# V-DETR/V-DETR

Measured on AMD Instinct MI355X. Metric: scenes/sec (train fwd+bwd) 40k-pt ScanNet, higher is better.
Workload: dtype f32

## Files before the change

include/vdetr_hip.h:

```cpp
#ifndef VDETR_HIP_H
#define VDETR_HIP_H

#include <stddef.h>
#include <stdint.h>

#ifdef __cplusplus
extern "C" {
#endif

#define VDETR_OK 0
#define VDETR_ERR_ARG 1
#define VDETR_ERR_LAUNCH 2
#define VDETR_ERR_WORKSPACE 3

typedef void* vdetr_stream_t;

int vdetr_abi_version(void);
const char* vdetr_last_error(void);
int vdetr_ab_switches(void);


size_t vdetr_fps_workspace_bytes(int b, int n);
int vdetr_furthest_point_sampling_f32(const float* xyz, int b, int n, int m, int32_t* idx,
                                      void* workspace, size_t workspace_bytes, vdetr_stream_t stream);

size_t vdetr_fps_varlen_workspace_bytes(const int32_t* counts, int b);
int vdetr_furthest_point_sampling_varlen_f32(const float* const* xyz, const int32_t* counts, int b, int m, int32_t* idx,
                                             void* workspace, size_t workspace_bytes, vdetr_stream_t stream);

int vdetr_gather_rows_f32(const float* const* rows, const int32_t* idx, float* out, int b, int c, int m, vdetr_stream_t stream);
int vdetr_gather_rows_grad_f32(const float* grad_out, const int32_t* idx, float* const* grad_rows, int b, int c, int m,
                               vdetr_stream_t stream);

int vdetr_gather_points_f32(const float* points, const int32_t* idx, float* out, int b, int c, int n,
                            int m, vdetr_stream_t stream);
int vdetr_gather_points_grad_f32(const float* grad_out, const int32_t* idx, float* grad_points, int b,
                                 int c, int n, int m, vdetr_stream_t stream);
int vdetr_gather_points_grad_set_f32(const float* grad_out, const int32_t* idx, float* grad_points, int b,
                                     int c, int n, int m, vdetr_stream_t stream);

int vdetr_ball_query_f32(const float* new_xyz, const float* xyz, int32_t* idx, int b, int n, int m,
                         float radius, int nsample, vdetr_stream_t stream);

int vdetr_group_points_f32(const float* points, const int32_t* idx, float* out, int b, int c, int n,
                           int npoints, int nsample, vdetr_stream_t stream);
int vdetr_group_points_grad_f32(const float* grad_out, const int32_t* idx, float* grad_points, int b,
                                int c, int n, int npoints, int nsample, vdetr_stream_t stream);
int vdetr_group_points_grad_set_f32(const float* grad_out, const int32_t* idx, float* grad_points, int b,
                                    int c, int n, int npoints, int nsample, vdetr_stream_t stream);

int vdetr_three_nn_f32(const float* unknown, const float* known, float* dist2, int32_t* idx, int b,
                       int n, int m, vdetr_stream_t stream);
int vdetr_three_interpolate_f32(const float* points, const int32_t* idx, const float* weight,
                                float* out, int b, int c, int m, int n, vdetr_stream_t stream);
int vdetr_three_interpolate_grad_f32(const float* grad_out, const int32_t* idx, const float* weight,
                                     float* grad_points, int b, int c, int n, int m,
                                     vdetr_stream_t stream);

#define VDETR_ATTN_SHARED_KV 0
#define VDETR_ATTN_PER_HEAD 1

#define VDETR_MASK_NONE 0
#define VDETR_MASK_BOOL 1
#define VDETR_MASK_FLOAT 2

typedef struct vdetr_attn_desc {
  int32_t kind;
  int32_t B, H, nQ, nK;
  float scale;
  const float* table;
  int32_t table_size;
  float log_scale;
  float inv_log_norm;
  const float* vertices;
  const float* xyz;
  const float* cos_sin;
  const void* mask;
  int32_t mask_kind;
  float dropout_p;
  uint64_t seed, offset;
  const uint64_t* rng_state;
  int32_t k_row_stride, v_row_stride;
  uint32_t* bwd_aux;
  int32_t table_grid;
  int32_t kv_waves;
  int32_t fwd_kernel;
  int32_t bwd_kernel;
  int32_t kv_halves;
  const void* kv_img;
  uint32_t* fwd_sched;
} vdetr_attn_desc;

size_t vdetr_attn_fwd_workspace_bytes(const vdetr_attn_desc* d);
size_t vdetr_attn_kv_image_bytes(int B, int nK);
int vdetr_attn_pack_kv_f32(const float* k, const float* v, int B, int nK, int k_row_stride, int v_row_stride, int nlayers,
                           int64_t layer_stride, void* img, vdetr_stream_t stream);
size_t vdetr_attn_kv_image_parts_bytes(int B, int nK, int parts);
int vdetr_attn_pack_kv_parts_f32(const float* k, const float* v, int B, int nK, int k_row_stride, int v_row_stride, int nlayers,
                                 int64_t layer_stride, int parts, void* img, vdetr_stream_t stream);

int vdetr_attn_fwd_f32(const vdetr_attn_desc* d, const float* q, const float* k, const float* v,
                       float* out, float* lse, float* scores, void* workspace, size_t workspace_bytes,
                       vdetr_stream_t stream);

typedef struct vdetr_attn_parts {
  const float* part_o;
  const float* part_lse;
  int32_t ksplit;
  int32_t reserved;
  int64_t rows;
} vdetr_attn_parts;
int vdetr_attn_fwd_parts_f32(const vdetr_attn_desc* d, const float* q, const float* k, const float* v,
                             float* out, float* lse, float* scores, void* workspace, size_t workspace_bytes,
                             vdetr_attn_parts* parts, vdetr_stream_t stream);

int vdetr_attn_fwd_bf16(const vdetr_attn_desc* d, const void* q, const void* k, const void* v, float* out, float* lse,
                        float* scores, void* workspace, size_t workspace_bytes, vdetr_stream_t stream);
size_t vdetr_attn_bwd_workspace_bytes(const vdetr_attn_desc* d);
int vdetr_attn_bwd_scores_f32(const vdetr_attn_desc* d, const float* scores, const float* dprob, const float* lse,
                              const float* delta, float* probs_out, float* ds_out, float* dtable, void* workspace,
                              size_t workspace_bytes, vdetr_stream_t stream);

size_t vdetr_attn_bwd_kv_workspace_bytes(const vdetr_attn_desc* d);
int vdetr_attn_bwd_kv_f32(const vdetr_attn_desc* d, const float* q, const float* v, const float* dout, const float* scores,
                          const float* lse, const float* delta, float* ds_out, float* dk, float* dv, void* workspace,
                          size_t workspace_bytes, vdetr_stream_t stream);
int vdetr_attn_bwd_kv_delta_f32(const vdetr_attn_desc* d, const float* q, const float* v, const float* dout, const float* out,
                                const float* scores, const float* lse, float* delta, float* ds_out, float* dk, float* dv,
                                void* workspace, size_t workspace_bytes, vdetr_stream_t stream);
typedef struct vdetr_attn_kv_prep {
  int32_t kind, B, H, nQ, nK, v_row_stride;
  const float* q;
  const float* v;
  const float* vertices;
  const float* cos_sin;
  void* workspace;
  float *dk, *dv;
  uint32_t* bwd_aux;
} vdetr_attn_kv_prep;
int vdetr_attn_bwd_kv_prep_f32(const vdetr_attn_kv_prep* items, int n, vdetr_stream_t stream);
int vdetr_attn_bwd_kv_packed_f32(const vdetr_attn_desc* d, const float* q, const float* v, const float* dout, const float* scores,
                                 const float* lse, const float* delta, float* ds_out, float* dk, float* dv, void* workspace,
                                 size_t workspace_bytes, vdetr_stream_t stream);
typedef struct vdetr_rb_attn_emit {
  void* workspace;
  float* delta;
  const float* out;
  uint32_t* bwd_aux;
  int32_t per_head, nQ;
} vdetr_rb_attn_emit;
int vdetr_attn_bwd_dq_f32(const vdetr_attn_desc* d, const float* ds, const float* k, float* dq, vdetr_stream_t stream);
int vdetr_attn_bwd_table_f32(const vdetr_attn_desc* d, const float* ds, float* dtable, void* workspace,
                             size_t workspace_bytes, vdetr_stream_t stream);
int vdetr_attn_bwd_table_kernel_names(const vdetr_attn_desc* d, const char** box_kernel, const char** general_kernel);

int vdetr_attn_delta_f32(const vdetr_attn_desc* d, const float* dout, const float* out, const float* v, float* delta,
                         vdetr_stream_t stream);

int vdetr_attn_dropout_mask_u8(const vdetr_attn_desc* d, uint8_t* keep, vdetr_stream_t stream);

int vdetr_rpe_bias_f32(const vdetr_attn_desc* d, float* rpe, vdetr_stream_t stream);

#define VDETR_CLS_SOFTMAX 0
#define VDETR_CLS_SIGMOID 1

typedef struct vdetr_box_decode_desc {
  int32_t B, N;
  int32_t A;
  int32_t C1;
  int32_t num_angle_bin;
  int32_t cls_kind;
  const float *center, *size;
  const float *angle_cls, *angle_res;
  const float* cls;
  const float *pre_center_norm, *pre_size_norm;
  const float *dims_min, *dims_max;
  float *center_reg, *size_reg, *center_unnorm, *center_norm, *size_unnorm, *size_norm, *pre_center_unnorm, *pre_size_unnorm;
  float* angle_residual;
  float *angle_cont, *angle_prob;
  int32_t* angle_class;
  float* corners;
  float* corners_aa;
  float* cls_prob;
  float* objectness;
  int32_t in_batch_stride;
  float *cls_logits_t, *angle_logits_t, *angle_res_norm_t;
  float *corners_lidar, *center_size;
} vdetr_box_decode_desc;

typedef struct vdetr_box_decode_grads {
  const float *center_reg, *size_reg, *center_unnorm, *center_norm, *size_unnorm, *size_norm;
  const float* angle_residual;
  const float *angle_cont, *angle_prob;
  const float *corners, *corners_aa;
  float *d_center, *d_size;
  float *d_angle_cls, *d_angle_res;
  const float *cls_logits_t, *angle_logits_t, *angle_res_norm_t;
  float* d_cls;
  int32_t out_batch_stride, slab_rows;
} vdetr_box_decode_grads;

int vdetr_box_decode_fwd_f32(const vdetr_box_decode_desc* d, vdetr_stream_t stream);
int vdetr_box_decode_bwd_f32(const vdetr_box_decode_desc* d, const vdetr_box_decode_grads* g, vdetr_stream_t stream);
int vdetr_anchor_boxes_f32(const float* logits, const float* xyz, const float* dims_min, const float* dims_max, const float* anchors,
                           int B, int N, int ncls, float* size_unnorm, float* center_norm, float* size_norm, float* corners,
                           vdetr_stream_t stream);
int vdetr_gather_proposals_f32(const long long* topk, int B, int N, int nq, int corners_are_camera, const float* corners,
                               const float* center, const float* size, const float* angle, const float* center_norm,
                               const float* size_norm, float* o_corners_lidar, float* o_center, float* o_size, float* o_angle,
                               float* o_center_norm, float* o_size_norm, float* o_query_ref, vdetr_stream_t stream);
int vdetr_box_decode_bwd_batch_f32(const vdetr_box_decode_desc* d, const vdetr_box_decode_grads* g, int n, vdetr_stream_t stream);

typedef struct vdetr_addln_desc {
  int32_t rows, C;
  float eps;
  float dropout_p;
  uint64_t seed, offset;
  const uint64_t* rng_state;
  const float* x;
  const float* r;
  const float *gamma, *beta;
  const float *gamma2, *beta2;
  float* y;
  float *out, *out2;
  float *mean, *rstd;
} vdetr_addln_desc;

typedef struct vdetr_addln_grads {
  const float *d_out, *d_out2;
  const float* d_y;
  float* d_x;
  float* d_r;
  float *d_gamma, *d_beta, *d_gamma2, *d_beta2;
  float* partials;
} vdetr_addln_grads;

int vdetr_add_ln_fwd_f32(const vdetr_addln_desc* d, vdetr_stream_t stream);
size_t vdetr_add_ln_bwd_workspace_bytes(const vdetr_addln_desc* d);
int vdetr_add_ln_bwd_f32(const vdetr_addln_desc* d, const vdetr_addln_grads* g, vdetr_stream_t stream);
typedef struct vdetr_addln_reduce {
  const float* partials;
  int32_t nparts, C;
  float *d_gamma, *d_beta, *d_gamma2, *d_beta2;
} vdetr_addln_reduce;
int vdetr_add_ln_param_reduce_batch_f32(const vdetr_addln_reduce* items, int n, vdetr_stream_t stream);

typedef struct vdetr_rb_linear {
  const float* w;
  const float* b;
  const float* wt;
} vdetr_rb_linear;
typedef struct vdetr_rb_norm {
  const float *gamma, *beta;
  float eps;
} vdetr_rb_norm;
typedef struct vdetr_rb_drop {
  float p;
  uint64_t seed;
} vdetr_rb_drop;

typedef struct vdetr_rb_qkv_desc {
  int32_t rows, B;
  const float* t;
  const float* pos;
  const float* w;
  const float* b;
  const float* wt;
  float* x;
  float* out;
} vdetr_rb_qkv_desc;
int vdetr_rb_qkv_f32(const vdetr_rb_qkv_desc* d, vdetr_stream_t stream);
int vdetr_rb_transpose_f32(const float* const* src, float* dst, int n, vdetr_stream_t stream);

typedef struct vdetr_rb_projq_desc {
  int32_t rows, B;
  const uint64_t* rng_state;
  const float* a;
  const float* tgt;
  const float* pos;
  vdetr_rb_linear proj, q;
  vdetr_rb_drop drop1;
  vdetr_rb_norm norm2;
  float *y, *mean_y, *rstd_y, *t2;
  float* xq;
  float* qout;
} vdetr_rb_projq_desc;
int vdetr_rb_proj_q_f32(const vdetr_rb_projq_desc* d, vdetr_stream_t stream);

typedef struct vdetr_rb_ffn_desc {
  int32_t rows, B;
  const uint64_t* rng_state;
  const float* a;
  const float* tgt;
  vdetr_rb_linear proj, lin1, lin2;
  vdetr_rb_drop drop2, drop_act, drop3;
  vdetr_rb_norm norm3, post1, post2;
  float *y, *mean_y, *rstd_y, *t2;
  float* h;
  float *z, *mean_z, *rstd_z, *o1, *o2;
} vdetr_rb_ffn_desc;
int vdetr_rb_ffn_f32(const vdetr_rb_ffn_desc* d, vdetr_stream_t stream);
int vdetr_rb_ffn_parts_f32(const vdetr_rb_ffn_desc* d, const vdetr_attn_parts* parts, float* attn_out, float* attn_lse,
                           vdetr_stream_t stream);

typedef struct vdetr_rb_qkv_grads {
  const float *dq, *dk, *dv;
  float *dq_rows, *dk_rows, *dv_rows;
  float* d_x;
  const float* d_x_add;
  float* d_t;
} vdetr_rb_qkv_grads;
int vdetr_rb_qkv_bwd_f32(const vdetr_rb_qkv_desc* d, const vdetr_rb_qkv_grads* g, vdetr_stream_t stream);

typedef struct vdetr_rb_projq_grads {
  const float* d_y;
  const float* d_qout;
  float* d_tgt;
  float* d_a;
  float* d_t2;
  float* dq_rows;
  float* d_proj;
  float* part_n2;
} vdetr_rb_projq_grads;
int vdetr_rb_proj_q_bwd_f32(const vdetr_rb_projq_desc* d, const vdetr_rb_projq_grads* g, vdetr_stream_t stream);

typedef struct vdetr_rb_ffn_grads {
  const float *d_z, *d_o1, *d_o2;
  float* d_tgt;
  float* d_a;
  float *d_lin2, *d_lin1, *d_proj;
  float *part_post, *part_n3;
} vdetr_rb_ffn_grads;
int vdetr_rb_ffn_bwd_f32(const vdetr_rb_ffn_desc* d, const vdetr_rb_ffn_grads* g, vdetr_stream_t stream);
int vdetr_rb_ffn0_f32(const vdetr_rb_ffn_desc* d, vdetr_stream_t stream);
int vdetr_rb_ffn0_bwd_f32(const vdetr_rb_ffn_desc* d, const vdetr_rb_ffn_grads* g, vdetr_stream_t stream);
int vdetr_rb_ffn_bwd_emit_f32(const vdetr_rb_ffn_desc* d, const vdetr_rb_ffn_grads* g, const vdetr_rb_attn_emit* e, vdetr_stream_t stream);
int vdetr_rb_proj_q_bwd_emit_f32(const vdetr_rb_projq_desc* d, const vdetr_rb_projq_grads* g, const vdetr_rb_attn_emit* e,
                                 vdetr_stream_t stream);

typedef struct vdetr_bnact_desc {
  int32_t B, C, N;
  int32_t training;
  int32_t relu;
  float eps, momentum;
  float dropout_p;
  uint64_t seed, offset;
  const uint64_t* rng_state;
  const float* x;
  const float *gamma, *beta;
  float *running_mean, *running_var;
  float* y;
  float *save_mean, *save_invstd;
  const float* pre_bias;
  int64_t* counters[8];
  int32_t ncounters;
  int32_t stats_given;
} vdetr_bnact_desc;

typedef struct vdetr_bnact_grads {
  const float* dy;
  float* dx;
  float *d_gamma, *d_beta;
  const float *sum_dy_xhat, *sum_dy, *inv_count;
} vdetr_bnact_grads;

int vdetr_relu_dropout_fwd_f32(const float* x, float* y, long n, float dropout_p, uint64_t seed, uint64_t offset,
                               const uint64_t* rng_state, vdetr_stream_t stream);
int vdetr_relu_dropout_bwd_f32(const float* y, const float* dy, float* dx, long n, float dropout_p, vdetr_stream_t stream);
int vdetr_bn_act_fwd_f32(const vdetr_bnact_desc* d, vdetr_stream_t stream);
int vdetr_bn_stats_f32(const vdetr_bnact_desc* d, float* mean, float* m2, vdetr_stream_t stream);
int vdetr_bn_act_bwd_f32(const vdetr_bnact_desc* d, const vdetr_bnact_grads* g, vdetr_stream_t stream);
int vdetr_bn_act_bwd_batch_f32(const vdetr_bnact_desc* descs, const vdetr_bnact_grads* grads, int n, vdetr_stream_t stream);

typedef struct vdetr_pack_entry {
  const void* src;
  uint64_t dst_offset;
  uint64_t numel;
} vdetr_pack_entry;
int vdetr_colsum_f32(const float* x, float* out, int rows, int cols, long row_stride, vdetr_stream_t stream);
size_t vdetr_colsum_workspace_bytes(int n, int rows, int cols);
int vdetr_colsum_batched_f32(const float* x, float* out, int n, int rows, int cols, long row_stride, long item_stride,
                             void* workspace, size_t workspace_bytes, vdetr_stream_t stream);
int vdetr_colsum_ptrs_f32(const float* const* items, float* out, int n, int rows, int cols, long row_stride, void* workspace,
                          size_t workspace_bytes, vdetr_stream_t stream);
int vdetr_pack_chunk_floats(void);
int vdetr_pack_f32(const vdetr_pack_entry* entries, const uint32_t* block_entry, const uint32_t* block_chunk, int nblocks,
                   float* dst, vdetr_stream_t stream);
int vdetr_pack_sumsq_f32(const vdetr_pack_entry* entries, const uint32_t* block_entry, const uint32_t* block_chunk, int nblocks,
                         float* dst, float* sumsq, vdetr_stream_t stream);

int vdetr_cpb_tables_f32(const float* coords, const float* w1, const float* b1, const float* w2, int n, int P, int hidden, int H,
                         float* hid_out, float* tables, vdetr_stream_t stream);

typedef struct vdetr_adamw_desc {
  float* param;
  const float* grad;
  float* exp_avg;
  float* exp_avg_sq;
  int64_t n;
  float* step;
  uint32_t* ticket;
  const float* sumsq;
  int32_t nsumsq;
  float max_norm;
  float norm_eps;
  float* norm_out;
  double lr, beta1, beta2, eps, weight_decay;
} vdetr_adamw_desc;
int vdetr_adamw_clip_f32(const vdetr_adamw_desc* d, vdetr_stream_t stream);
int vdetr_sumsq_blocks(long n);
int vdetr_sumsq_f32(const float* g, long n, float* partial, int npartial, vdetr_stream_t stream);

int vdetr_morton_sort_max(void);
int vdetr_morton_order_f32(const float* xyz, int B, int n, int* codes, long long* order, vdetr_stream_t stream);
int vdetr_topk_order_f32(const float* values, int B, int n, int nq, long long* order, vdetr_stream_t stream);

#define VDETR_GT_CORNERS 0
#define VDETR_GT_CENTER 24
#define VDETR_GT_SIZE 27
#define VDETR_GT_ANGLE 30
#define VDETR_GT_LABEL 31
#define VDETR_GT_ANGLE_CLS 32
#define VDETR_GT_ANGLE_RES 33
#define VDETR_GT_PRESENT 34
#define VDETR_GT_FLOATS 36

int vdetr_gt_prepare_f32(const float* gt, int B, int G, int repeat, float* gt_rep, int64_t* nactual, int64_t* nactual_rep,
                         float* sums, vdetr_stream_t stream);

typedef struct vdetr_match_desc {
  int32_t B, P, G;
  int32_t C, A;
  int32_t cls_kind;
  int32_t label_override;
  float w_cls, w_objectness, w_center, w_giou, w_size, w_angle_cls, w_angle_reg;
  const float* cls;
  const float* objectness;
  const float *center_reg, *size_reg, *pre_center, *pre_size;
  const float* corners;
  const float *angle_logits, *angle_res_norm;
  const float* gt;
  const int64_t* nactual;
  float* cost_t;
  float* giou_t;
  const float* rotated;
} vdetr_match_desc;
int vdetr_match_cost_f32(const vdetr_match_desc* d, vdetr_stream_t stream);
int vdetr_match_cost_batch_f32(const vdetr_match_desc* descs, int n, vdetr_stream_t stream);

#define VDETR_LSA_MAX_PROBLEMS 16
typedef struct vdetr_lsa_problem {
  const float* cost_t;
  const int64_t* nactual;
  int64_t* inds;
  float* mask;
  int32_t B, P, G;
  int32_t row_repeat;
} vdetr_lsa_problem;
typedef struct vdetr_lsa_batch {
  int32_t nproblems;
  int32_t reserved;
  vdetr_lsa_problem p[VDETR_LSA_MAX_PROBLEMS];
} vdetr_lsa_batch;
int vdetr_lsa_f64(const vdetr_lsa_batch* batch, int32_t* status, vdetr_stream_t stream);

int vdetr_point_labels_f32(const float* seed_xyz, const float* gt, const int64_t* nactual, int B, int N, int G, int C,
                           int64_t* labels, float* matched_count, vdetr_stream_t stream);

typedef struct vdetr_setloss_desc {
  int32_t B, P, G, C, A;
  int32_t label_override;
  float focal_alpha;
  float w_cls, w_angle_cls, w_angle_reg, w_center, w_size, w_giou;
  int32_t cls_kind;
  float w_no_object;
  const float* cls_logits;
  const float *center_reg, *size_reg, *pre_center, *pre_size;
  const float* corners;
  const float *angle_logits, *angle_res_norm;
  const float* gt;
  const int64_t* nactual;
  const int64_t* inds;
  const float* mask;
  const int64_t* labels;
  const float* num_boxes;
  float* losses;
  unsigned long long* card_ws;
  float *d_cls_logits, *d_center_reg, *d_size_reg, *d_corners, *d_angle_logits, *d_angle_res_norm;
  const float* rotated;
  const float* ce_rows_matched;
} vdetr_setloss_desc;
int vdetr_set_loss_f32(const vdetr_setloss_desc* d, vdetr_stream_t stream);
int vdetr_set_loss_batch_f32(const vdetr_setloss_desc* descs, int n, vdetr_stream_t stream);

#define VDETR_IOU_GIOU 0
#define VDETR_IOU_DIOU 1
#define VDETR_IOU_IOU 2
typedef struct vdetr_iou_ext {
  int32_t iou_kind;
  int32_t reserved;
  const float *center, *size;
  const float* angle;
  float *d_center, *d_size;
  float* d_angle;
} vdetr_iou_ext;
int vdetr_match_cost_ext_batch_f32(const vdetr_match_desc* descs, const vdetr_iou_ext* exts, int n, vdetr_stream_t stream);
int vdetr_set_loss_ext_batch_f32(const vdetr_setloss_desc* descs, const vdetr_iou_ext* exts, int n, vdetr_stream_t stream);

size_t vdetr_nms3d_workspace_bytes(int B, int K);
int vdetr_nms3d_f32(const float* corners, const float* score, const int32_t* cls, const uint8_t* valid, const int64_t* order,
                    int B, int K, double iou_threshold, int old_type, uint8_t* keep, void* workspace, size_t workspace_bytes,
                    vdetr_stream_t stream);

size_t vdetr_nms3d_rot_workspace_bytes(int B, int K);
int vdetr_nms3d_rot_f32(const float* corners, const float* score, const int32_t* cls, const uint8_t* valid, const int64_t* order,
                        int B, int K, double iou_threshold, int old_type, uint8_t* keep, void* workspace,
                        size_t workspace_bytes, vdetr_stream_t stream);

int vdetr_box_point_count_f32(const float* points, const float* boxes, int B, int N, int K, int32_t* counts,
                              vdetr_stream_t stream);

int vdetr_box3d_iou_max_f64(const float* pred_corners, const int32_t* pred_img, const int32_t* pred_cls, int P,
                            const float* gt_corners, const int32_t* gt_cls, const int32_t* img_gt_begin, double* ovmax,
                            int32_t* jmax, vdetr_stream_t stream);

int vdetr_box3d_iou_pairs_f64(const float* corners_a, int Na, const float* corners_b, int Nb, double* out,
                              vdetr_stream_t stream);

int vdetr_sp_kernel_map_i32(const int64_t* in_keys, int nin, const int64_t* out_keys, int nout, const int32_t* offsets, int K,
                            int32_t* nbr, vdetr_stream_t stream);
int vdetr_sp_inverse_map_i32(const int32_t* nbr, int K, int nout, int nin, int32_t* inv, vdetr_stream_t stream);
int vdetr_sp_gather_cols_f32(const float* in, const int32_t* nbr, int K, int nout, int C, float* col, vdetr_stream_t stream);
int vdetr_sp_gather_sum_f32(const float* dcol, const int32_t* inv, int K, int nin, int C, int offset_major_rows, float* din,
                            vdetr_stream_t stream);

int vdetr_sp_pairs_gemm_f32(const float* x, const int32_t* arow, const float* w, const int32_t* tiles, int ntiles, int cin,
                            int cout, int transposed, float* y, vdetr_stream_t stream);
int vdetr_sp_pairs_wgrad_f32(const float* x, const float* dy, const int32_t* pin, const int32_t* pout, const int32_t* chunks,
                             int nchunks, int cin, int cout, float* partials, vdetr_stream_t stream);
int vdetr_sp_wgrad_reduce_f32(const float* partials, const int32_t* seg, int K, long elems, float* dw, vdetr_stream_t stream);
int vdetr_sp_pair_plan_workspace_ints(int K, int nout);
int vdetr_sp_pair_plan_i32(const int32_t* nbr, int K, int nout, int nin, int32_t* pin, int32_t* pout, int32_t* slot,
                           int32_t* islot, int32_t* counts, int32_t* workspace, vdetr_stream_t stream);

typedef struct vdetr_spbn_desc {
  int32_t N, C, act, training;
  float eps, momentum;
  const float *x, *gamma, *beta, *residual;
  float *running_mean, *running_var;
  int64_t* num_batches_tracked;
  float *y, *save_mean, *save_invstd;
  void* workspace;
} vdetr_spbn_desc;
size_t vdetr_sp_bn_workspace_bytes(int N, int C);
int vdetr_sp_bn_act_fwd_f32(const vdetr_spbn_desc* d, vdetr_stream_t stream);
int vdetr_sp_bn_act_bwd_f32(const vdetr_spbn_desc* d, const float* dy, float* dx, float* dresidual, float* dgamma, float* dbeta,
                            vdetr_stream_t stream);

int vdetr_pos_embed_fourier_f32(const float* xyz, int b, int n, const float* range_min, const float* range_max,
                                const float* gauss_b, int ldb, int d_out, float* out, vdetr_stream_t stream);
int vdetr_pos_embed_sine_f32(const float* xyz, int b, int n, const float* range_min, const float* range_max,
                             int num_channels, float temperature, float scale, float* out, vdetr_stream_t stream);

typedef struct vdetr_heads_desc {
  int32_t B, N;
  int32_t G, rows;
  const float* x;
  const float* w1t;
  const float* w2t;
  const float* w3;
  const float* b3;
  const float *gamma1, *beta1, *gamma2, *beta2;
  float *running_mean1, *running_var1, *running_mean2, *running_var2;
  int64_t* counters1[8];
  int64_t* counters2[8];
  float eps, momentum;
  float p1, p2;
  uint64_t salt1, salt2;
  const uint64_t* rng_state;
  float *pre1, *h1, *pre2, *h2;
  float *save_mean1, *save_invstd1, *save_mean2, *save_invstd2;
  float* y;
  void* workspace;
} vdetr_heads_desc;
size_t vdetr_heads_workspace_bytes(int B, int N, int G);
int vdetr_heads_fwd_f32(const vdetr_heads_desc* d, vdetr_stream_t stream);

typedef struct vdetr_heads_infer_desc {
  int32_t B, N;
  int32_t G, rows;
  int32_t tile;
  float eps;
  const float* x;
  const float* w1t;
  const float* w2t;
  const float* w3;
  const float* b3;
  const float *mean1, *var1, *gamma1, *beta1;
  const float *mean2, *var2, *gamma2, *beta2;
  float* y;
} vdetr_heads_infer_desc;
int vdetr_heads_infer_f32(const vdetr_heads_infer_desc* d, vdetr_stream_t stream);

typedef struct vdetr_posmlp_desc {
  int32_t B, N, cin;
  const float* x;
  const float* w1;
  const float* b1;
  const float *gamma, *beta;
  float *running_mean, *running_var;
  int64_t* counter;
  float eps, momentum;
  const float* w2t;
  const float* b2;
  float *hpre, *hact;
  float *save_mean, *save_invstd;
  float* out;
} vdetr_posmlp_desc;
int vdetr_pos_mlp_fwd_f32(const vdetr_posmlp_desc* d, vdetr_stream_t stream);
int vdetr_rb_qkv_pos_f32(const vdetr_rb_qkv_desc* d, const vdetr_posmlp_desc* m, vdetr_stream_t stream);
int vdetr_pos_mlp_infer_f32(const vdetr_posmlp_desc* d, vdetr_stream_t stream);
int vdetr_rb_qkv_pos_infer_f32(const vdetr_rb_qkv_desc* d, const vdetr_posmlp_desc* m, vdetr_stream_t stream);

int vdetr_selftest_lds_atomics(int mode, int iters, float* sink, vdetr_stream_t stream);

int vdetr_probe_timestamp(uint64_t* slot, vdetr_stream_t stream);

int vdetr_selftest_mfma_f32(const float* a, const float* b, float* c, vdetr_stream_t stream);

#ifdef __cplusplus
}
#endif
#endif
```

v-detr_amd/_lib.py:

```python
import ctypes
import os

import torch

_HERE = os.path.dirname(os.path.abspath(__file__))
LIB_PATH = os.path.join(_HERE, "lib", "libvdetr_hip.so")

c_int, c_float, c_void_p, c_size_t = ctypes.c_int, ctypes.c_float, ctypes.c_void_p, ctypes.c_size_t

VDETR_ATTN_SHARED_KV, VDETR_ATTN_PER_HEAD = 0, 1
VDETR_MASK_NONE, VDETR_MASK_BOOL, VDETR_MASK_FLOAT = 0, 1, 2


class AttnDesc(ctypes.Structure):

    _fields_ = [
        ("kind", ctypes.c_int32), ("B", ctypes.c_int32), ("H", ctypes.c_int32), ("nQ", ctypes.c_int32),
        ("nK", ctypes.c_int32), ("scale", c_float),
        ("table", c_void_p), ("table_size", ctypes.c_int32), ("log_scale", c_float), ("inv_log_norm", c_float),
        ("vertices", c_void_p), ("xyz", c_void_p), ("cos_sin", c_void_p),
        ("mask", c_void_p), ("mask_kind", ctypes.c_int32),
        ("dropout_p", c_float), ("seed", ctypes.c_uint64), ("offset", ctypes.c_uint64),
        ("rng_state", c_void_p),
        ("k_row_stride", ctypes.c_int32), ("v_row_stride", ctypes.c_int32),
        ("bwd_aux", c_void_p),
        ("table_grid", ctypes.c_int32), ("kv_waves", ctypes.c_int32), ("fwd_kernel", ctypes.c_int32), ("bwd_kernel", ctypes.c_int32), ("kv_halves", ctypes.c_int32), ("kv_img", c_void_p),
        ("fwd_sched", c_void_p),
    ]


VDETR_CLS_SOFTMAX, VDETR_CLS_SIGMOID = 0, 1

_BOX_IN = ("center", "size", "angle_cls", "angle_res", "cls", "pre_center_norm", "pre_size_norm", "dims_min", "dims_max")
_BOX_OUT = ("center_reg", "size_reg", "center_unnorm", "center_norm", "size_unnorm", "size_norm", "pre_center_unnorm",
            "pre_size_unnorm", "angle_residual", "angle_cont", "angle_prob", "angle_class", "corners", "corners_aa",
            "cls_prob", "objectness")


class BoxDecodeDesc(ctypes.Structure):

    _fields_ = ([(n, ctypes.c_int32) for n in ("B", "N", "A", "C1", "num_angle_bin", "cls_kind")] +
                [(n, c_void_p) for n in _BOX_IN + _BOX_OUT] + [("in_batch_stride", ctypes.c_int32)] +
                [(n, c_void_p) for n in ("cls_logits_t", "angle_logits_t", "angle_res_norm_t", "corners_lidar", "center_size")])


_BOX_GRAD_IN = ("center_reg", "size_reg", "center_unnorm", "center_norm", "size_unnorm", "size_norm", "angle_residual",
                "angle_cont", "angle_prob", "corners", "corners_aa")
_BOX_GRAD_OUT = ("d_center", "d_size", "d_angle_cls", "d_angle_res")


class BoxDecodeGrads(ctypes.Structure):

    _fields_ = ([(n, c_void_p) for n in _BOX_GRAD_IN + _BOX_GRAD_OUT] +
                [(n, c_void_p) for n in ("cls_logits_t", "angle_logits_t", "angle_res_norm_t", "d_cls")] +
                [("out_batch_stride", ctypes.c_int32), ("slab_rows", ctypes.c_int32)])


class AddLnDesc(ctypes.Structure):

    _fields_ = [("rows", ctypes.c_int32), ("C", ctypes.c_int32), ("eps", c_float), ("dropout_p", c_float),
                ("seed", ctypes.c_uint64), ("offset", ctypes.c_uint64), ("rng_state", c_void_p)] + [
        (n, c_void_p) for n in ("x", "r", "gamma", "beta", "gamma2", "beta2", "y", "out", "out2", "mean", "rstd")]


class AddLnGrads(ctypes.Structure):

    _fields_ = [(n, c_void_p) for n in ("d_out", "d_out2", "d_y", "d_x", "d_r", "d_gamma", "d_beta", "d_gamma2", "d_beta2",
                                        "partials")]


class AddLnReduce(ctypes.Structure):

    _fields_ = [("partials", c_void_p), ("nparts", ctypes.c_int32), ("C", ctypes.c_int32), ("d_gamma", c_void_p), ("d_beta", c_void_p),
                ("d_gamma2", c_void_p), ("d_beta2", c_void_p)]


class RbLinear(ctypes.Structure):

    _fields_ = [("w", c_void_p), ("b", c_void_p), ("wt", c_void_p)]


class RbNorm(ctypes.Structure):

    _fields_ = [("gamma", c_void_p), ("beta", c_void_p), ("eps", c_float)]


class RbDrop(ctypes.Structure):

    _fields_ = [("p", c_float), ("seed", ctypes.c_uint64)]


class RbQkvDesc(ctypes.Structure):

    _fields_ = [("rows", ctypes.c_int32), ("B", ctypes.c_int32)] + [(n, c_void_p) for n in ("t", "pos", "w", "b", "wt", "x", "out")]


class RbProjQDesc(ctypes.Structure):

    _fields_ = ([("rows", ctypes.c_int32), ("B", ctypes.c_int32)] + [(n, c_void_p) for n in ("rng_state", "a", "tgt", "pos")] +
                [("proj", RbLinear), ("q", RbLinear), ("drop1", RbDrop), ("norm2", RbNorm)] +
                [(n, c_void_p) for n in ("y", "mean_y", "rstd_y", "t2", "xq", "qout")])


class RbFfnDesc(ctypes.Structure):

    _fields_ = ([("rows", ctypes.c_int32), ("B", ctypes.c_int32)] + [(n, c_void_p) for n in ("rng_state", "a", "tgt")] +
                [("proj", RbLinear), ("lin1", RbLinear), ("lin2", RbLinear), ("drop2", RbDrop), ("drop_act", RbDrop), ("drop3", RbDrop),
                 ("norm3", RbNorm), ("post1", RbNorm), ("post2", RbNorm)] +
                [(n, c_void_p) for n in ("y", "mean_y", "rstd_y", "t2", "h", "z", "mean_z", "rstd_z", "o1", "o2")])


class RbQkvGrads(ctypes.Structure):

    _fields_ = [(n, c_void_p) for n in ("dq", "dk", "dv", "dq_rows", "dk_rows", "dv_rows", "d_x", "d_x_add", "d_t")]


class RbProjQGrads(ctypes.Structure):

    _fields_ = [(n, c_void_p) for n in ("d_y", "d_qout", "d_tgt", "d_a", "d_t2", "dq_rows", "d_proj", "part_n2")]


class RbFfnGrads(ctypes.Structure):

    _fields_ = [(n, c_void_p) for n in ("d_z", "d_o1", "d_o2", "d_tgt", "d_a", "d_lin2", "d_lin1", "d_proj", "part_post", "part_n3")]


class BnActDesc(ctypes.Structure):

    _fields_ = [(n, ctypes.c_int32) for n in ("B", "C", "N", "training", "relu")] + [
        ("eps", c_float), ("momentum", c_float), ("dropout_p", c_float), ("seed", ctypes.c_uint64),
        ("offset", ctypes.c_uint64), ("rng_state", c_void_p)] + [
        (n, c_void_p) for n in ("x", "gamma", "beta", "running_mean", "running_var", "y", "save_mean", "save_invstd",
                                "pre_bias")] + [("counters", c_void_p * 8), ("ncounters", ctypes.c_int32),
                                                ("stats_given", ctypes.c_int32)]


class HeadsDesc(ctypes.Structure):

    _fields_ = [(n, ctypes.c_int32) for n in ("B", "N", "G", "rows")] + [
        (n, c_void_p) for n in ("x", "w1t", "w2t", "w3", "b3", "gamma1", "beta1", "gamma2", "beta2", "running_mean1", "running_var1",
                                "running_mean2", "running_var2")] + [
        ("counters1", c_void_p * 8), ("counters2", c_void_p * 8), ("eps", c_float), ("momentum", c_float), ("p1", c_float),
        ("p2", c_float), ("salt1", ctypes.c_uint64), ("salt2", ctypes.c_uint64), ("rng_state", c_void_p)] + [
        (n, c_void_p) for n in ("pre1", "h1", "pre2", "h2", "save_mean1", "save_invstd1", "save_mean2", "save_invstd2", "y",
                                "workspace")]


class HeadsInferDesc(ctypes.Structure):

    _fields_ = [(n, ctypes.c_int32) for n in ("B", "N", "G", "rows", "tile")] + [("eps", c_float)] + [
        (n, c_void_p) for n in ("x", "w1t", "w2t", "w3", "b3", "mean1", "var1", "gamma1", "beta1", "mean2", "var2", "gamma2", "beta2",
                                "y")]


class AttnParts(ctypes.Structure):

    _fields_ = [("part_o", c_void_p), ("part_lse", c_void_p), ("ksplit", ctypes.c_int32), ("reserved", ctypes.c_int32),
                ("rows", ctypes.c_int64)]


class AttnKvPrep(ctypes.Structure):

    _fields_ = [(n, ctypes.c_int32) for n in ("kind", "B", "H", "nQ", "nK", "v_row_stride")] + [
        (n, c_void_p) for n in ("q", "v", "vertices", "cos_sin", "workspace", "dk", "dv", "bwd_aux")]


class RbAttnEmit(ctypes.Structure):

    _fields_ = [(n, c_void_p) for n in ("workspace", "delta", "out", "bwd_aux")] + [("per_head", ctypes.c_int32), ("nQ", ctypes.c_int32)]


class AdamWDesc(ctypes.Structure):

    _fields_ = [(n, c_void_p) for n in ("param", "grad", "exp_avg", "exp_avg_sq")] + [("n", ctypes.c_int64)] + [
        (n, c_void_p) for n in ("step", "ticket", "sumsq")] + [("nsumsq", ctypes.c_int32), ("max_norm", c_float), ("norm_eps", c_float),
                                                                ("norm_out", c_void_p)] + [
        (n, ctypes.c_double) for n in ("lr", "beta1", "beta2", "eps", "weight_decay")]


class PosMlpDesc(ctypes.Structure):

    _fields_ = [(n, ctypes.c_int32) for n in ("B", "N", "cin")] + [
        (n, c_void_p) for n in ("x", "w1", "b1", "gamma", "beta", "running_mean", "running_var", "counter")] + [
        ("eps", c_float), ("momentum", c_float)] + [
        (n, c_void_p) for n in ("w2t", "b2", "hpre", "hact", "save_mean", "save_invstd", "out")]


class BnActGrads(ctypes.Structure):

    _fields_ = [(n, c_void_p) for n in ("dy", "dx", "d_gamma", "d_beta", "sum_dy_xhat", "sum_dy", "inv_count")]


VDETR_GT_CORNERS, VDETR_GT_CENTER, VDETR_GT_SIZE, VDETR_GT_ANGLE, VDETR_GT_LABEL = 0, 24, 27, 30, 31
VDETR_GT_ANGLE_CLS, VDETR_GT_ANGLE_RES, VDETR_GT_PRESENT, VDETR_GT_FLOATS = 32, 33, 34, 36
VDETR_LSA_MAX_PROBLEMS = 16

_MATCH_W = ("w_cls", "w_objectness", "w_center", "w_giou", "w_size", "w_angle_cls", "w_angle_reg")
_MATCH_PTR = ("cls", "objectness", "center_reg", "size_reg", "pre_center", "pre_size", "corners", "angle_logits",
              "angle_res_norm", "gt", "nactual", "cost_t", "giou_t", "rotated")


class MatchDesc(ctypes.Structure):

    _fields_ = ([(n, ctypes.c_int32) for n in ("B", "P", "G", "C", "A", "cls_kind", "label_override")] +
                [(n, c_float) for n in _MATCH_W] + [(n, c_void_p) for n in _MATCH_PTR])


class LsaProblem(ctypes.Structure):

    _fields_ = [(n, c_void_p) for n in ("cost_t", "nactual", "inds", "mask")] + [
        (n, ctypes.c_int32) for n in ("B", "P", "G", "row_repeat")]


class LsaBatch(ctypes.Structure):

    _fields_ = [("nproblems", ctypes.c_int32), ("reserved", ctypes.c_int32), ("p", LsaProblem * VDETR_LSA_MAX_PROBLEMS)]


_LOSS_W = ("w_cls", "w_angle_cls", "w_angle_reg", "w_center", "w_size", "w_giou")
_LOSS_PTR = ("cls_logits", "center_reg", "size_reg", "pre_center", "pre_size", "corners", "angle_logits", "angle_res_norm",
             "gt", "nactual", "inds", "mask", "labels", "num_boxes", "losses", "card_ws", "d_cls_logits", "d_center_reg", "d_size_reg",
             "d_corners", "d_angle_logits", "d_angle_res_norm", "rotated", "ce_rows_matched")


class SetLossDesc(ctypes.Structure):

    _fields_ = ([(n, ctypes.c_int32) for n in ("B", "P", "G", "C", "A", "label_override")] + [("focal_alpha", c_float)] +
                [(n, c_float) for n in _LOSS_W] + [("cls_kind", ctypes.c_int32), ("w_no_object", c_float)] +
                [(n, c_void_p) for n in _LOSS_PTR])


VDETR_IOU_GIOU, VDETR_IOU_DIOU, VDETR_IOU_IOU = 0, 1, 2
IOU_KINDS = {"giou": VDETR_IOU_GIOU, "diou": VDETR_IOU_DIOU, "iou": VDETR_IOU_IOU}


class IouExt(ctypes.Structure):

    _fields_ = [("iou_kind", ctypes.c_int32), ("reserved", ctypes.c_int32)] + [
        (n, c_void_p) for n in ("center", "size", "angle", "d_center", "d_size", "d_angle")]


class SpBnDesc(ctypes.Structure):

    _fields_ = ([(n, ctypes.c_int32) for n in ("N", "C", "act", "training")] + [("eps", c_float), ("momentum", c_float)] +
                [(n, c_void_p) for n in ("x", "gamma", "beta", "residual", "running_mean", "running_var", "num_batches_tracked",
                                         "y", "save_mean", "save_invstd", "workspace")])


_SIGNATURES = {
    "vdetr_abi_version": (c_int, []),
    "vdetr_ab_switches": (c_int, []),
    "vdetr_last_error": (ctypes.c_char_p, []),
    "vdetr_fps_workspace_bytes": (c_size_t, [c_int, c_int]),
    "vdetr_furthest_point_sampling_f32": (c_int, [c_void_p, c_int, c_int, c_int, c_void_p, c_void_p, c_size_t, c_void_p]),
    "vdetr_fps_varlen_workspace_bytes": (c_size_t, [c_void_p, c_int]),
    "vdetr_furthest_point_sampling_varlen_f32": (c_int, [c_void_p, c_void_p, c_int, c_int, c_void_p, c_void_p, c_size_t, c_void_p]),
    "vdetr_pos_embed_fourier_f32": (c_int, [c_void_p, c_int, c_int, c_void_p, c_void_p, c_void_p, c_int, c_int, c_void_p, c_void_p]),
    "vdetr_pos_embed_sine_f32": (c_int, [c_void_p, c_int, c_int, c_void_p, c_void_p, c_int, c_float, c_float, c_void_p, c_void_p]),
    "vdetr_gather_rows_f32": (c_int, [c_void_p, c_void_p, c_void_p, c_int, c_int, c_int, c_void_p]),
    "vdetr_gather_rows_grad_f32": (c_int, [c_void_p, c_void_p, c_void_p, c_int, c_int, c_int, c_void_p]),
    "vdetr_gather_points_f32": (c_int, [c_void_p, c_void_p, c_void_p, c_int, c_int, c_int, c_int, c_void_p]),
    "vdetr_gather_points_grad_f32": (c_int, [c_void_p, c_void_p, c_void_p, c_int, c_int, c_int, c_int, c_void_p]),
    "vdetr_gather_points_grad_set_f32": (c_int, [c_void_p, c_void_p, c_void_p, c_int, c_int, c_int, c_int, c_void_p]),
    "vdetr_group_points_grad_set_f32": (c_int, [c_void_p, c_void_p, c_void_p, c_int, c_int, c_int, c_int, c_int, c_void_p]),
    "vdetr_ball_query_f32": (c_int, [c_void_p, c_void_p, c_void_p, c_int, c_int, c_int, c_float, c_int, c_void_p]),
    "vdetr_group_points_f32": (c_int, [c_void_p, c_void_p, c_void_p, c_int, c_int, c_int, c_int, c_int, c_void_p]),
    "vdetr_group_points_grad_f32": (c_int, [c_void_p, c_void_p, c_void_p, c_int, c_int, c_int, c_int, c_int, c_void_p]),
    "vdetr_three_nn_f32": (c_int, [c_void_p, c_void_p, c_void_p, c_void_p, c_int, c_int, c_int, c_void_p]),
    "vdetr_three_interpolate_f32": (c_int, [c_void_p, c_void_p, c_void_p, c_void_p, c_int, c_int, c_int, c_int, c_void_p]),
    "vdetr_three_interpolate_grad_f32": (c_int, [c_void_p, c_void_p, c_void_p, c_void_p, c_int, c_int, c_int, c_int, c_void_p]),
    "vdetr_attn_fwd_workspace_bytes": (c_size_t, [ctypes.POINTER(AttnDesc)]),
    "vdetr_attn_kv_image_bytes": (c_size_t, [c_int, c_int]),
    "vdetr_attn_pack_kv_f32": (c_int, [c_void_p, c_void_p, c_int, c_int, c_int, c_int, c_int, ctypes.c_int64, c_void_p, c_void_p]),
    "vdetr_attn_kv_image_parts_bytes": (c_size_t, [c_int, c_int, c_int]),
    "vdetr_attn_pack_kv_parts_f32": (c_int, [c_void_p, c_void_p, c_int, c_int, c_int, c_int, c_int, ctypes.c_int64, c_int, c_void_p, c_void_p]),
    "vdetr_attn_fwd_f32": (c_int, [ctypes.POINTER(AttnDesc), c_void_p, c_void_p, c_void_p, c_void_p, c_void_p, c_void_p, c_void_p, c_size_t, c_void_p]),
    "vdetr_attn_fwd_bf16": (c_int, [ctypes.POINTER(AttnDesc), c_void_p, c_void_p, c_void_p, c_void_p, c_void_p, c_void_p, c_void_p, c_size_t, c_void_p]),
    "vdetr_attn_fwd_parts_f32": (c_int, [ctypes.POINTER(AttnDesc), c_void_p, c_void_p, c_void_p, c_void_p, c_void_p, c_void_p, c_void_p, c_size_t,
                                         ctypes.POINTER(AttnParts), c_void_p]),
    "vdetr_attn_bwd_workspace_bytes": (c_size_t, [ctypes.POINTER(AttnDesc)]),
    "vdetr_attn_bwd_scores_f32": (c_int, [ctypes.POINTER(AttnDesc), c_void_p, c_void_p, c_void_p, c_void_p, c_void_p, c_void_p, c_void_p, c_void_p, c_size_t, c_void_p]),
    "vdetr_attn_bwd_kv_workspace_bytes": (c_size_t, [ctypes.POINTER(AttnDesc)]),
    "vdetr_attn_bwd_kv_f32": (c_int, [ctypes.POINTER(AttnDesc)] + [c_void_p] * 10 + [c_size_t, c_void_p]),
    "vdetr_attn_bwd_kv_delta_f32": (c_int, [ctypes.POINTER(AttnDesc)] + [c_void_p] * 11 + [c_size_t, c_void_p]),
    "vdetr_attn_bwd_dq_f32": (c_int, [ctypes.POINTER(AttnDesc), c_void_p, c_void_p, c_void_p, c_void_p]),
    "vdetr_attn_bwd_table_f32": (c_int, [ctypes.POINTER(AttnDesc), c_void_p, c_void_p, c_void_p, c_size_t, c_void_p]),
    "vdetr_attn_bwd_table_kernel_names": (c_int, [ctypes.POINTER(AttnDesc), ctypes.POINTER(ctypes.c_char_p), ctypes.POINTER(ctypes.c_char_p)]),
    "vdetr_attn_delta_f32": (c_int, [ctypes.POINTER(AttnDesc), c_void_p, c_void_p, c_void_p, c_void_p, c_void_p]),
    "vdetr_attn_dropout_mask_u8": (c_int, [ctypes.POINTER(AttnDesc), c_void_p, c_void_p]),
    "vdetr_rpe_bias_f32": (c_int, [ctypes.POINTER(AttnDesc), c_void_p, c_void_p]),
    "vdetr_box_decode_fwd_f32": (c_int, [ctypes.POINTER(BoxDecodeDesc), c_void_p]),
    "vdetr_box_decode_bwd_f32": (c_int, [ctypes.POINTER(BoxDecodeDesc), ctypes.POINTER(BoxDecodeGrads), c_void_p]),
    "vdetr_box_decode_bwd_batch_f32": (c_int, [ctypes.POINTER(BoxDecodeDesc), ctypes.POINTER(BoxDecodeGrads), c_int, c_void_p]),
    "vdetr_add_ln_fwd_f32": (c_int, [ctypes.POINTER(AddLnDesc), c_void_p]),
    "vdetr_add_ln_bwd_workspace_bytes": (c_size_t, [ctypes.POINTER(AddLnDesc)]),
    "vdetr_add_ln_bwd_f32": (c_int, [ctypes.POINTER(AddLnDesc), ctypes.POINTER(AddLnGrads), c_void_p]),
    "vdetr_add_ln_param_reduce_batch_f32": (c_int, [ctypes.POINTER(AddLnReduce), c_int, c_void_p]),
    "vdetr_relu_dropout_fwd_f32": (c_int, [c_void_p, c_void_p, ctypes.c_long, c_float, ctypes.c_uint64, ctypes.c_uint64, c_void_p,
                                           c_void_p]),
    "vdetr_relu_dropout_bwd_f32": (c_int, [c_void_p, c_void_p, c_void_p, ctypes.c_long, c_float, c_void_p]),
    "vdetr_bn_act_fwd_f32": (c_int, [ctypes.POINTER(BnActDesc), c_void_p]),
    "vdetr_bn_stats_f32": (c_int, [ctypes.POINTER(BnActDesc), c_void_p, c_void_p, c_void_p]),
    "vdetr_heads_workspace_bytes": (c_size_t, [c_int, c_int, c_int]),
    "vdetr_heads_fwd_f32": (c_int, [ctypes.POINTER(HeadsDesc), c_void_p]),
    "vdetr_pos_mlp_fwd_f32": (c_int, [ctypes.POINTER(PosMlpDesc), c_void_p]),
    "vdetr_heads_infer_f32": (c_int, [ctypes.POINTER(HeadsInferDesc), c_void_p]),
    "vdetr_pos_mlp_infer_f32": (c_int, [ctypes.POINTER(PosMlpDesc), c_void_p]),
    "vdetr_bn_act_bwd_f32": (c_int, [ctypes.POINTER(BnActDesc), ctypes.POINTER(BnActGrads), c_void_p]),
    "vdetr_bn_act_bwd_batch_f32": (c_int, [ctypes.POINTER(BnActDesc), ctypes.POINTER(BnActGrads), c_int, c_void_p]),
    "vdetr_colsum_f32": (c_int, [c_void_p, c_void_p, c_int, c_int, ctypes.c_long, c_void_p]),
    "vdetr_colsum_workspace_bytes": (c_size_t, [c_int, c_int, c_int]),
    "vdetr_colsum_batched_f32": (c_int, [c_void_p, c_void_p, c_int, c_int, c_int, ctypes.c_long, ctypes.c_long, c_void_p, c_size_t, c_void_p]),
    "vdetr_colsum_ptrs_f32": (c_int, [c_void_p, c_void_p, c_int, c_int, c_int, ctypes.c_long, c_void_p, c_size_t, c_void_p]),
    "vdetr_nms3d_workspace_bytes": (c_size_t, [c_int, c_int]),
    "vdetr_nms3d_f32": (c_int, [c_void_p, c_void_p, c_void_p, c_void_p, c_void_p, c_int, c_int, ctypes.c_double, c_int, c_void_p,
                        c_void_p, c_size_t, c_void_p]),
    "vdetr_nms3d_rot_workspace_bytes": (c_size_t, [c_int, c_int]),
    "vdetr_nms3d_rot_f32": (c_int, [c_void_p, c_void_p, c_void_p, c_void_p, c_void_p, c_int, c_int, ctypes.c_double, c_int, c_void_p,
                            c_void_p, c_size_t, c_void_p]),
    "vdetr_box_point_count_f32": (c_int, [c_void_p, c_void_p, c_int, c_int, c_int, c_void_p, c_void_p]),
    "vdetr_box3d_iou_max_f64": (c_int, [c_void_p, c_void_p, c_void_p, c_int, c_void_p, c_void_p, c_void_p, c_void_p, c_void_p,
                                c_void_p]),
    "vdetr_box3d_iou_pairs_f64": (c_int, [c_void_p, c_int, c_void_p, c_int, c_void_p, c_void_p]),
    "vdetr_morton_sort_max": (c_int, []),
    "vdetr_morton_order_f32": (c_int, [c_void_p, c_int, c_int, c_void_p, c_void_p, c_void_p]),
    "vdetr_pack_chunk_floats": (c_int, []),
    "vdetr_pack_f32": (c_int, [c_void_p, c_void_p, c_void_p, c_int, c_void_p, c_void_p]),
    "vdetr_pack_sumsq_f32": (c_int, [c_void_p, c_void_p, c_void_p, c_int, c_void_p, c_void_p, c_void_p]),
    "vdetr_adamw_clip_f32": (c_int, [ctypes.POINTER(AdamWDesc), c_void_p]),
    "vdetr_cpb_tables_f32": (c_int, [c_void_p] * 4 + [c_int] * 4 + [c_void_p] * 3),
    "vdetr_sumsq_blocks": (c_int, [ctypes.c_long]),
    "vdetr_sumsq_f32": (c_int, [c_void_p, ctypes.c_long, c_void_p, c_int, c_void_p]),
    "vdetr_gt_prepare_f32": (c_int, [c_void_p, c_int, c_int, c_int, c_void_p, c_void_p, c_void_p, c_void_p, c_void_p]),
    "vdetr_match_cost_f32": (c_int, [ctypes.POINTER(MatchDesc), c_void_p]),
    "vdetr_match_cost_batch_f32": (c_int, [ctypes.POINTER(MatchDesc), c_int, c_void_p]),
    "vdetr_lsa_f64": (c_int, [ctypes.POINTER(LsaBatch), c_void_p, c_void_p]),
    "vdetr_point_labels_f32": (c_int, [c_void_p, c_void_p, c_void_p, c_int, c_int, c_int, c_int, c_void_p, c_void_p, c_void_p]),
    "vdetr_set_loss_f32": (c_int, [ctypes.POINTER(SetLossDesc), c_void_p]),
    "vdetr_set_loss_batch_f32": (c_int, [ctypes.POINTER(SetLossDesc), c_int, c_void_p]),
    "vdetr_match_cost_ext_batch_f32": (c_int, [ctypes.POINTER(MatchDesc), ctypes.POINTER(IouExt), c_int, c_void_p]),
    "vdetr_set_loss_ext_batch_f32": (c_int, [ctypes.POINTER(SetLossDesc), ctypes.POINTER(IouExt), c_int, c_void_p]),
    "vdetr_sp_kernel_map_i32": (c_int, [c_void_p, c_int, c_void_p, c_int, c_void_p, c_int, c_void_p, c_void_p]),
    "vdetr_sp_inverse_map_i32": (c_int, [c_void_p, c_int, c_int, c_int, c_void_p, c_void_p]),
    "vdetr_sp_gather_cols_f32": (c_int, [c_void_p, c_void_p, c_int, c_int, c_int, c_void_p, c_void_p]),
    "vdetr_sp_gather_sum_f32": (c_int, [c_void_p, c_void_p, c_int, c_int, c_int, c_int, c_void_p, c_void_p]),
    "vdetr_sp_pairs_gemm_f32": (c_int, [c_void_p, c_void_p, c_void_p, c_void_p, c_int, c_int, c_int, c_int, c_void_p, c_void_p]),
    "vdetr_sp_pair_plan_workspace_ints": (c_int, [c_int, c_int]),
    "vdetr_sp_pair_plan_i32": (c_int, [c_void_p, c_int, c_int, c_int, c_void_p, c_void_p, c_void_p, c_void_p, c_void_p, c_void_p,
                               c_void_p]),
    "vdetr_sp_wgrad_reduce_f32": (c_int, [c_void_p, c_void_p, c_int, ctypes.c_long, c_void_p, c_void_p]),
    "vdetr_sp_pairs_wgrad_f32": (c_int, [c_void_p, c_void_p, c_void_p, c_void_p, c_void_p, c_int, c_int, c_int, c_void_p, c_void_p]),
    "vdetr_sp_bn_workspace_bytes": (c_size_t, [c_int, c_int]),
    "vdetr_sp_bn_act_fwd_f32": (c_int, [ctypes.POINTER(SpBnDesc), c_void_p]),
    "vdetr_sp_bn_act_bwd_f32": (c_int, [ctypes.POINTER(SpBnDesc), c_void_p, c_void_p, c_void_p, c_void_p, c_void_p, c_void_p]),
    "vdetr_rb_transpose_f32": (c_int, [c_void_p, c_void_p, c_int, c_void_p]),
    "vdetr_rb_qkv_f32": (c_int, [ctypes.POINTER(RbQkvDesc), c_void_p]),
    "vdetr_rb_proj_q_f32": (c_int, [ctypes.POINTER(RbProjQDesc), c_void_p]),
    "vdetr_rb_qkv_pos_f32": (c_int, [ctypes.POINTER(RbQkvDesc), ctypes.POINTER(PosMlpDesc), c_void_p]),
    "vdetr_rb_qkv_pos_infer_f32": (c_int, [ctypes.POINTER(RbQkvDesc), ctypes.POINTER(PosMlpDesc), c_void_p]),
    "vdetr_rb_ffn_f32": (c_int, [ctypes.POINTER(RbFfnDesc), c_void_p]),
    "vdetr_rb_ffn_parts_f32": (c_int, [ctypes.POINTER(RbFfnDesc), ctypes.POINTER(AttnParts), c_void_p, c_void_p, c_void_p]),
    "vdetr_rb_qkv_bwd_f32": (c_int, [ctypes.POINTER(RbQkvDesc), ctypes.POINTER(RbQkvGrads), c_void_p]),
    "vdetr_rb_proj_q_bwd_f32": (c_int, [ctypes.POINTER(RbProjQDesc), ctypes.POINTER(RbProjQGrads), c_void_p]),
    "vdetr_rb_ffn_bwd_f32": (c_int, [ctypes.POINTER(RbFfnDesc), ctypes.POINTER(RbFfnGrads), c_void_p]),
    "vdetr_rb_ffn0_f32": (c_int, [ctypes.POINTER(RbFfnDesc), c_void_p]),
    "vdetr_rb_ffn0_bwd_f32": (c_int, [ctypes.POINTER(RbFfnDesc), ctypes.POINTER(RbFfnGrads), c_void_p]),
    "vdetr_rb_ffn_bwd_emit_f32": (c_int, [ctypes.POINTER(RbFfnDesc), ctypes.POINTER(RbFfnGrads), ctypes.POINTER(RbAttnEmit), c_void_p]),
    "vdetr_rb_proj_q_bwd_emit_f32": (c_int, [ctypes.POINTER(RbProjQDesc), ctypes.POINTER(RbProjQGrads), ctypes.POINTER(RbAttnEmit), c_void_p]),
    "vdetr_attn_bwd_kv_prep_f32": (c_int, [ctypes.POINTER(AttnKvPrep), c_int, c_void_p]),
    "vdetr_attn_bwd_kv_packed_f32": (c_int, [ctypes.POINTER(AttnDesc)] + [c_void_p] * 10 + [c_size_t, c_void_p]),
    "vdetr_probe_timestamp": (c_int, [c_void_p, c_void_p]),
    "vdetr_topk_order_f32": (c_int, [c_void_p, c_int, c_int, c_int, c_void_p, c_void_p]),
    "vdetr_anchor_boxes_f32": (c_int, [c_void_p] * 5 + [c_int] * 3 + [c_void_p] * 5),
    "vdetr_gather_proposals_f32": (c_int, [c_void_p, c_int, c_int, c_int, c_int] + [c_void_p] * 14),
    "vdetr_selftest_lds_atomics": (c_int, [c_int, c_int, c_void_p, c_void_p]),
    "vdetr_selftest_mfma_f32": (c_int, [c_void_p, c_void_p, c_void_p, c_void_p]),
}

_lib = None


def exported_symbols():
    return sorted(_SIGNATURES)


def lib():
    global _lib
    if _lib is None:
        if not os.path.exists(LIB_PATH):
            raise RuntimeError(
                f"{LIB_PATH} is missing: build it with `python -c 'import __graft_entry__ as g; g.build()'` "
                "(hipcc --offload-arch=gfx950).  vdetr_amd has no CPU fallback.")
        handle = ctypes.CDLL(LIB_PATH)
        for name, (restype, argtypes) in _SIGNATURES.items():
            fn = getattr(handle, name)
            fn.restype = restype
            fn.argtypes = argtypes
        _lib = handle
    return _lib


def check(status, op):
    if status != 0:
        msg = lib().vdetr_last_error().decode(errors="replace")
        raise RuntimeError(f"vdetr_hip {op} failed (status {status}): {msg}")


def stream_ptr():
    return c_void_p(torch.cuda.current_stream().cuda_stream)


def ptr(t):
    return c_void_p(t.data_ptr()) if t is not None else c_void_p(0)


def require_gpu(t, name):
    if not t.is_cuda:
        raise RuntimeError(f"{name}: CPU not supported (tensor is on {t.device})")


def require_contiguous(t, name):
    if not t.is_contiguous():
        raise RuntimeError(f"{name} must be a contiguous tensor")


def require_float(t, name):
    if t.dtype != torch.float32:
        raise RuntimeError(f"{name} must be a float tensor")


def require_int(t, name):
    if t.dtype != torch.int32:
        raise RuntimeError(f"{name} must be an int tensor")


def workspace(nbytes, device):
    return torch.empty(max(int(nbytes), 1), dtype=torch.uint8, device=device)


_rocblas = {"lib": None, "handles": {}}
ROCBLAS_OP_N, ROCBLAS_OP_T = 111, 112


def rocblas():
    if _rocblas["lib"] is None:
        path = os.path.join(os.path.dirname(torch.__file__), "lib", "librocblas.so")
        rb = ctypes.CDLL(path if os.path.exists(path) else "librocblas.so")
        rb.rocblas_create_handle.argtypes = [ctypes.POINTER(c_void_p)]
        rb.rocblas_set_stream.argtypes = [c_void_p, c_void_p]
        rb.rocblas_sgemm_batched.argtypes = [c_void_p, c_int, c_int, c_int, c_int, c_int, c_void_p, c_void_p, c_int, c_void_p, c_int,
                                             c_void_p, c_void_p, c_int, c_int]
        _rocblas["lib"] = rb
    return _rocblas["lib"]


def sgemm_batched_ptrs(op_a, op_b, m, n, k, a_ptrs, lda, b_ptrs, ldb, c_ptrs, ldc, batch, device, alpha=1.0, beta=0.0):
    rb = rocblas()
    key = device.index if device.index is not None else torch.cuda.current_device()
    h = _rocblas["handles"].get(key)
    if h is None:
        if torch.cuda.is_current_stream_capturing():
            raise RuntimeError("rocBLAS handle: create it before a stream capture (run one step eagerly first)")
        h = c_void_p()
        with torch.cuda.device(key):
            if rb.rocblas_create_handle(ctypes.byref(h)) != 0:
                raise RuntimeError("rocblas_create_handle failed")
        _rocblas["handles"][key] = h
    if rb.rocblas_set_stream(h, c_void_p(torch.cuda.current_stream(device).cuda_stream)) != 0:
        raise RuntimeError("rocblas_set_stream failed")
    al, be = c_float(alpha), c_float(beta)
    addr = lambda p: c_void_p(p.data_ptr() if torch.is_tensor(p) else int(p))
    rc = rb.rocblas_sgemm_batched(h, op_a, op_b, m, n, k, ctypes.byref(al), addr(a_ptrs), lda, addr(b_ptrs), ldb, ctypes.byref(be),
                                  addr(c_ptrs), ldc, batch)
    if rc != 0:
        raise RuntimeError(f"rocblas_sgemm_batched failed (status {rc})")


_ptr_tables = {}


def upload_ptrs(ptrs, device):
    n = len(ptrs)
    key = device.index if device.index is not None else torch.cuda.current_device()
    T = _ptr_tables.get(key)
    if T is None:
        if torch.cuda.is_current_stream_capturing():
            raise RuntimeError("pointer tables: allocate before a stream capture (run one step eagerly first)")
        T = _ptr_tables[key] = {"ring": [torch.empty(1024, dtype=torch.int64).pin_memory() for _ in range(4)], "events": [None] * 4, "tick": 0,
                                "spare": [torch.empty(1024, dtype=torch.int64).pin_memory() for _ in range(48)], "kept": []}
    if n > 1024:
        raise RuntimeError(f"pointer table of {n} entries (max 1024)")
    dev = torch.empty(n, dtype=torch.int64, device=device)
    if torch.cuda.is_current_stream_capturing():
        if not T["spare"]:
            raise RuntimeError("pointer tables: more than 48 captured uploads in this process")
        host = T["spare"].pop()
        T["kept"].append(host)
        host[:n] = torch.tensor(ptrs, dtype=torch.int64)
        dev.copy_(host[:n], non_blocking=True)
        return dev
    slot = T["tick"] % 4
    T["tick"] += 1
    if T["events"][slot] is not None:
        T["events"][slot].synchronize()
    host = T["ring"][slot]
    host[:n] = torch.tensor(ptrs, dtype=torch.int64)
    dev.copy_(host[:n], non_blocking=True)
    ev = torch.cuda.Event()
    ev.record(torch.cuda.current_stream(device))
    T["events"][slot] = ev
    return dev
```

v-detr_amd/attention.py:

```python
import contextlib
import ctypes
import os
import weakref

import torch
from torch.autograd import Function

from . import _lib as L

HEAD_DIM = 64


class RPEConfig:

    def __init__(self, table_size=10, log_scale=512.0, max_value=4.0):
        self.table_size = int(table_size)
        self.log_scale = float(log_scale)
        self.max_value = float(max_value)

    @property
    def inv_log_norm(self):
        return 1.0 / (3.0 * self.max_value)


def new_rng_state(device, seed=None):
    if seed is None:
        seed = torch.initial_seed()
    return torch.tensor([seed & 0x7FFFFFFFFFFFFFFF, 0], dtype=torch.int64, device=device)


FWD_KERNEL = int(os.environ.get("VDETR_FWD_KERNEL", "0"))
BWD_KERNEL = int(os.environ.get("VDETR_BWD_KERNEL", "0"))
TABLE_GRID = 0
FUSED_KV_BWD = os.environ.get("VDETR_BWD_FUSED", "1") != "0"
SELF_FWD_BODY = os.environ.get("VDETR_SELF_FWD", "") == "body"


_ASYNC_ENV = os.environ.get("VDETR_BWD_ASYNC_TABLE", "auto")
ASYNC_TABLE_GRAD = _ASYNC_ENV != "0"
ASYNC_MIN_PAIRS = 1 << 21
ASYNC_TABLE_GRID = int(os.environ.get("VDETR_BWD_ASYNC_GRID", "190"))


_step_side = {}


def side_branch_in_use(device):
    return bool(_step_side.get(_dev_key(device)))


class SideResults:
    pending = []

    @classmethod
    def flush(cls):
        from .helpers import DeferredParamGrads
        items, cls.pending = cls.pending, []
        late, side_late[:] = list(side_late), []
        for fn, alive in late:
            with torch.no_grad():
                items.append((None, fn(), alive))
        for dev, pairs, _alive in items:
            side = _side_streams.get(_dev_key(dev)) if dev is not None else None
            if side is not None:
                torch.cuda.current_stream(dev).wait_stream(side)
            roots, grads = [], []
            with torch.no_grad():
                for p, g in pairs:
                    if p is not None and p.requires_grad:
                        DeferredParamGrads._deliver(p, g, roots, grads)
            if roots:
                torch.autograd.backward(roots, grads)


_tick = {}
side_late = []


def flush_layer_params_on_side(ref, rows):
    from .helpers import DeferredParamGrads, DeferredPosEmbedGrads
    if not (ref.is_cuda and DeferredParamGrads.enabled and side_branch_in_use(ref.device)):
        return
    dev = ref.device
    key = _dev_key(dev)
    cur = torch.cuda.current_stream(dev)
    fork = torch.cuda.Event()
    fork.record(cur)
    if key not in _tick:
        _tick[key] = torch.zeros(4, device=dev)
    _tick[key].add_(0.0)
    side = _side_stream(dev)
    side.wait_event(fork)
    pairs, keep = [], []
    late, side_late[:] = list(side_late), []
    from .runtime import ts_mark
    ts_mark("main: all layers' backward done")
    with torch.cuda.stream(side):
        ts_mark("side: parked gradients start")
        DeferredParamGrads.flush(select=lambda it: it[2].shape[0] == rows, collect=pairs, keepalive=keep)
        DeferredPosEmbedGrads.flush(collect=pairs, keepalive=keep)
        from .add_ln import DeferredLnGrads
        DeferredLnGrads.flush(collect=pairs, keepalive=keep)
        for fn, alive in late:
            pairs += fn()
            keep.append(alive)
        ts_mark("side: parked gradients end")
    if pairs:
        SideResults.pending.append((dev, pairs, keep))


def set_async_table_grad(mode):
    global _ASYNC_ENV, ASYNC_TABLE_GRAD
    prev, _ASYNC_ENV = _ASYNC_ENV, str(mode)
    ASYNC_TABLE_GRAD = _ASYNC_ENV != "0"
    return prev


def _async_wanted(B, nQ, nK):
    return ASYNC_TABLE_GRAD and (_ASYNC_ENV == "1" or B * nQ * nK >= ASYNC_MIN_PAIRS)


_side_streams = {}
_side_keep = []


def _dev_key(device):
    device = torch.device(device)
    if device.type != "cuda":
        return (device.type, 0)
    return (device.type, device.index if device.index is not None else torch.cuda.current_device())


def _side_stream(device):
    key = _dev_key(device)
    if key not in _side_streams:
        _side_streams[key] = torch.cuda.Stream(device=device)
    return _side_streams[key]


class _JoinTableGrad(Function):
    @staticmethod
    def forward(ctx, t):
        ctx.dev = t.device
        return t.view_as(t)

    @staticmethod
    def backward(ctx, g):
        side = _side_streams.get(_dev_key(ctx.dev))
        if side is not None and _side_keep:
            torch.cuda.current_stream(ctx.dev).wait_stream(side)
        _side_keep.clear()
        return g


class _ParkTableGrad(Function):

    @staticmethod
    def forward(ctx, anchor, table, slot):
        ctx.slot = slot
        return table.view_as(table)

    @staticmethod
    def backward(ctx, g):
        ctx.slot[1] = g
        return None, None, None


class DeferredTableGrads:
    pending = []
    _anchor = {}
    _begun = []
    buffers = {}
    _outputs = {}
    _buffer_keys = {}

    @classmethod
    def park(cls, tables, mlp=None):
        key = _dev_key(tables.device)
        if key not in cls._anchor:
            cls._anchor[key] = torch.zeros(1, device=tables.device, requires_grad=True)
        alive = []
        for item in cls.pending:
            _tables, slots, _acc, _mlp = item
            outs = cls._outputs.get(id(slots), ())
            if all(g is None for _, g in slots) and all(r() is None for r in outs):
                cls._outputs.pop(id(slots), None)
                for key_ in cls._buffer_keys.pop(id(slots), ()):
                    cls.buffers.pop(key_, None)
                continue
            alive.append(item)
        cls.pending = alive
        if sum(1 for _, slots, _, _ in alive if any(g is not None for _, g in slots)) > 32:
            raise RuntimeError("runtime.defer_weight_grads() is on but runtime.flush_weight_grads() has not been called for 32 "
                               "backward passes (parked RPE-table gradients pile up)")
        cut = tables.detach()
        slots = [[i, None] for i in range(tables.shape[0])]
        acc = None
        if tables.is_cuda and tables.dtype == torch.float32:
            acc = _take_zeros(tables, tuple(tables.shape), tables.dtype)
            for i in range(tables.shape[0]):
                cls.buffers[cut[i].data_ptr()] = acc[i]
            cls._buffer_keys[id(slots)] = [cut[i].data_ptr() for i in range(tables.shape[0])]
        cls.pending.append((tables, slots, acc, mlp))
        outs = [_ParkTableGrad.apply(cls._anchor[key], cut[i], slots[i]) for i in range(tables.shape[0])]
        cls._outputs[id(slots)] = [weakref.ref(o) for o in outs]
        return outs

    @classmethod
    def begin_flush(cls):
        keep = []
        for item in cls.pending:
            tables, slots, acc, mlp = item
            if mlp is None or all(g is None for _, g in slots):
                keep.append(item)
                continue
            dev = tables.device
            side = _side_streams.get(_dev_key(dev)) if (tables.is_cuda and _side_keep) else None
            cur = torch.cuda.current_stream(dev) if tables.is_cuda else None
            if acc is None or not all(g is None or g.data_ptr() == acc[i].data_ptr() for i, g in slots):
                if side is not None and _side_keep:
                    cur.wait_stream(side)
                acc = torch.stack([g if g is not None else torch.zeros_like(tables[i]) for i, g in slots])
                if side is not None:
                    side.wait_stream(cur)
            c1, w1, b1, w2, hid = mlp
            n8 = hid.shape[0]
            with (torch.cuda.stream(side) if side is not None else contextlib.nullcontext()), torch.no_grad():
                dT = acc.reshape(n8, hid.shape[1], -1)
                dW2 = torch.bmm(dT.transpose(1, 2), hid)
                dhid = torch.ops.aten.threshold_backward(torch.bmm(dT, w2.detach()), hid, 0.0)
                dW1b = torch.bmm(dhid.transpose(1, 2), c1.unsqueeze(0).expand(n8, -1, -1))
                if side is not None:
                    from .runtime import ts_mark
                    ts_mark("side: table MLPs' backward end")
            cls._begun.append((dev if side is not None else None, ((w1, dW1b[..., :3]), (b1, dW1b[..., 3]), (w2, dW2)),
                               (acc, dT, dhid, hid)))
        cls.pending = keep

    @classmethod
    def flush(cls):
        from .helpers import DeferredParamGrads
        SideResults.flush()
        begun, cls._begun = cls._begun, []
        for dev, pairs, _alive in begun:
            side = _side_streams.get(_dev_key(dev)) if dev is not None else None
            if side is not None:
                torch.cuda.current_stream(dev).wait_stream(side)
            _side_keep.clear()
            roots, grads = [], []
            with torch.no_grad():
                for p, g in pairs:
                    if p.requires_grad:
                        DeferredParamGrads._deliver(p, g, roots, grads)
            if roots:
                torch.autograd.backward(roots, grads)
        items, cls.pending = cls.pending, []
        cls.buffers.clear()
        cls._outputs.clear()
        cls._buffer_keys.clear()
        for tables, slots, acc, _mlp in items:
            if all(g is None for _, g in slots):
                continue
            if not tables.requires_grad:
                raise RuntimeError("tables parked with their MLP's operands can only be flushed through begin_flush()")
            dev = tables.device
            side = _side_streams.get(_dev_key(dev))
            if side is not None and _side_keep:
                torch.cuda.current_stream(dev).wait_stream(side)
            _side_keep.clear()
            if acc is not None and all(g is None or g.data_ptr() == acc[i].data_ptr() for i, g in slots):
                g = acc
            else:
                g = torch.stack([g if g is not None else torch.zeros_like(tables[i]) for i, g in slots])
            torch.autograd.backward([tables], [g])


def table_grads_parkable(ref):
    from .helpers import DeferredParamGrads
    return bool(ASYNC_TABLE_GRAD and DeferredParamGrads.enabled and ref.is_cuda and ref.requires_grad and torch.is_grad_enabled())


def park_table_grads(tables, mlp=None):
    if mlp is not None or table_grads_parkable(tables):
        _side_stream(tables.device)
        return DeferredTableGrads.park(tables, mlp)
    return [join_table_grad(t) for t in tables.unbind(0)]


def join_table_grad(table):
    if ASYNC_TABLE_GRAD and table is not None and table.is_cuda and table.requires_grad and torch.is_grad_enabled():
        _side_stream(table.device)
        return _JoinTableGrad.apply(table)
    return table


def _table_accumulator(table):
    buf = DeferredTableGrads.buffers.pop(table.data_ptr(), None)
    if buf is not None and buf.shape == table.shape:
        return buf
    return _take_zeros(table, tuple(table.shape), table.dtype)


def _launch_table_async(lib, d, q, ds, table, aux, vertices, xyz, mask, fork=None, dtable=None, also=()):
    if dtable is None:
        dtable = _take_zeros(table, tuple(table.shape), table.dtype)
    nbytes = lib.vdetr_attn_bwd_workspace_bytes(ctypes.byref(d))
    side = _side_stream(q.device)
    if fork is not None:
        side.wait_event(fork)
    else:
        side.wait_stream(torch.cuda.current_stream(q.device))
    from .runtime import ts_mark
    with torch.cuda.stream(side):
        ws2 = L.workspace(nbytes, q.device)
        keep_grid = d.table_grid
        d.table_grid = side_table_grid(q.device)
        ts_mark("side: table kernel start")
        try:
            L.check(lib.vdetr_attn_bwd_table_f32(ctypes.byref(d), L.ptr(ds), L.ptr(dtable), L.ptr(ws2), nbytes, L.stream_ptr()),
                    "attn_bwd_table")
        finally:
            d.table_grid = keep_grid
        ts_mark("side: table kernel end")
    _side_keep.append((ds, dtable, ws2, aux, table, vertices, xyz, mask) + tuple(also))
    return dtable


def side_table_grid(device):
    cus = torch.cuda.get_device_properties(device).multi_processor_count
    if not 2 <= ASYNC_TABLE_GRID < 256:
        return 0
    return max(2, (ASYNC_TABLE_GRID * cus // 256) & ~1)


_master = {}
_current = {}


def begin_step(device):
    device = torch.device(device)
    key = (device.type, device.index if device.index is not None else torch.cuda.current_device())
    if key not in _master:
        _master[key] = new_rng_state(device)
    snap = _master[key].clone()
    _master[key][1] += 1
    _current[key] = snap
    _step_side[key] = False
    _no_pending("begin_step")
    _kv_recs.pop(key, None)
    _kv_by_out.clear()
    _zero_pool[key] = None
    return snap


_zero_pool = {}
_ZERO_POOL_FLOATS = 1 << 19


def _take_zeros(like, shape, dtype):
    numel = 1
    for d in shape:
        numel *= int(d)
    key = (like.device.type, like.device.index if like.device.index is not None else torch.cuda.current_device())
    if key in _zero_pool and numel * 4 <= _ZERO_POOL_FLOATS:
        pool = _zero_pool[key]
        if pool is None:
            pool = _zero_pool[key] = [torch.zeros(_ZERO_POOL_FLOATS, dtype=torch.float32, device=like.device), 0]
        buf, used = pool
        n4 = (numel + 3) // 4 * 4
        if used + n4 <= buf.numel():
            pool[1] = used + n4
            return buf[used:used + numel].view(dtype).view(shape)
    return torch.zeros(shape, dtype=dtype, device=like.device)


def current_rng(device):
    device = torch.device(device)
    key = (device.type, device.index if device.index is not None else torch.cuda.current_device())
    return _current.get(key)


def reset_rng(seed=None):
    _master.clear()
    _current.clear()
    _zero_pool.clear()


def _desc(kind, B, H, nQ, nK, scale, table, rpe, vertices, xyz, cos_sin, mask, dropout_p, rng_state, salt=0,
          k_stride=0, v_stride=0):
    d = L.AttnDesc()
    d.k_row_stride, d.v_row_stride = int(k_stride), int(v_stride)
    d.kind, d.B, d.H, d.nQ, d.nK, d.scale = kind, B, H, nQ, nK, float(scale)
    if table is not None:
        d.table = table.data_ptr()
        d.table_size, d.log_scale, d.inv_log_norm = rpe.table_size, rpe.log_scale, rpe.inv_log_norm
        d.vertices, d.xyz = vertices.data_ptr(), xyz.data_ptr()
        d.cos_sin = cos_sin.data_ptr() if cos_sin is not None else None
    if mask is not None:
        d.mask = mask.data_ptr()
        d.mask_kind = L.VDETR_MASK_BOOL if mask.dtype == torch.uint8 else L.VDETR_MASK_FLOAT
    d.dropout_p = float(dropout_p)
    d.seed = int(salt) & 0xFFFFFFFFFFFFFFFF
    if rng_state is not None:
        d.rng_state = rng_state.data_ptr()
    d.fwd_kernel = FWD_KERNEL
    d.bwd_kernel = BWD_KERNEL
    d.table_grid = TABLE_GRID
    return d


def _prep_mask(mask, B, nQ, nK):
    if mask is None:
        return None
    if mask.dtype == torch.bool:
        mask = mask.to(torch.uint8)
    elif mask.dtype != torch.float32:
        mask = mask.float()
    return mask.expand(B, nQ, nK).contiguous()


def _check_inputs(**tensors):
    for name, t in tensors.items():
        if t is None:
            continue
        L.require_gpu(t, name)
        L.require_contiguous(t, name)
        L.require_float(t, name)


_pending_parts = {}
DEFER_COMBINE = os.environ.get("VDETR_DEFER_COMBINE", "1") != "0"


def take_pending_parts(out):
    return _pending_parts.pop(out.data_ptr(), None) if _pending_parts else None


def _no_pending(where):
    if _pending_parts:
        _pending_parts.clear()
        raise RuntimeError(f"{where}: an attention forward left its key-split merge to a consumer that never ran "
                           "(fused_attention(defer_combine=True) must be followed by rowblock.ffn on its output)")


KV_PREPACK = os.environ.get("VDETR_KV_PREPACK", "1") != "0"
_kv_recs = {}
_kv_by_out = {}


class _KvRec:
    __slots__ = ("q", "v", "vertices", "cos_sin", "kind", "dims", "want_aux", "ws", "nbytes", "dkv", "delta", "aux", "prepared", "emitted")


def _kv_register(out, q, v, table, vertices, cos_sin, kind, B, H, nQ, nK):
    shared = kind == L.VDETR_ATTN_SHARED_KV
    if not (KV_PREPACK and FUSED_KV_BWD and B == 1 and H == 4 and nQ % 32 == 0 and q.dtype == torch.float32 and v.dtype == torch.float32
            and (shared or table is None) and v.stride(1) % 4 == 0 and v.data_ptr() % 16 == 0 and 4 * nQ * nK * 4 < (1 << 31)):
        return None
    r = _KvRec()
    r.q, r.v, r.vertices, r.cos_sin, r.kind, r.dims = q, v, (vertices if table is not None else None), cos_sin, kind, (B, H, nQ, nK)
    r.want_aux = bool(table is not None and table.requires_grad)
    r.prepared, r.emitted = False, None
    r.ws = r.dkv = r.delta = r.aux = None
    lst = _kv_recs.setdefault(_dev_key(q.device), [])
    if len(lst) >= 64:
        del lst[:]
        _kv_by_out.clear()
    lst.append(r)
    _kv_by_out[out.data_ptr()] = r
    return r


def kv_record_of(out):
    return _kv_by_out.pop(out.data_ptr(), None) if _kv_by_out else None


def kv_prepare(rec):
    if rec.prepared:
        return
    dev = rec.q.device
    lib = L.lib()
    todo = [r for r in _kv_recs.get(_dev_key(dev), []) if not r.prepared]
    if rec not in todo:
        todo.append(rec)
    for i in range(0, len(todo), 16):
        chunk = todo[i:i + 16]
        items = (L.AttnKvPrep * len(chunk))()
        for it, r in zip(items, chunk):
            B, H, nQ, nK = r.dims
            shared = r.kind == L.VDETR_ATTN_SHARED_KV
            dd = L.AttnDesc()
            dd.kind, dd.B, dd.H, dd.nQ, dd.nK = r.kind, B, H, nQ, nK
            r.nbytes = lib.vdetr_attn_bwd_kv_workspace_bytes(ctypes.byref(dd))
            r.ws = L.workspace(r.nbytes, dev)
            assert r.ws.data_ptr() % 256 == 0
            r.dkv = torch.empty((2, B, nK, 64 if shared else H * 64), dtype=torch.float32, device=dev)
            r.delta = torch.empty((B, nQ, H) if shared else (B, H, nQ), dtype=torch.float32, device=dev)
            r.aux = _take_zeros(r.q, (8,), torch.int32) if r.want_aux else None
            it.kind, it.B, it.H, it.nQ, it.nK, it.v_row_stride = r.kind, B, H, nQ, nK, r.v.stride(1)
            it.q, it.v = r.q.data_ptr(), r.v.data_ptr()
            it.vertices = r.vertices.data_ptr() if (r.vertices is not None and r.aux is not None) else None
            it.cos_sin = r.cos_sin.data_ptr() if (r.cos_sin is not None and it.vertices) else None
            it.workspace, it.dk, it.dv = r.ws.data_ptr(), r.dkv[0].data_ptr(), r.dkv[1].data_ptr()
            it.bwd_aux = r.aux.data_ptr() if r.aux is not None else None
        L.check(lib.vdetr_attn_bwd_kv_prep_f32(items, len(chunk), L.stream_ptr()), "attn_bwd_kv_prep")
        for r in chunk:
            r.prepared = True


class _FusedAttention(Function):
    @staticmethod
    def forward(ctx, q, k, v, table, vertices, xyz, cos_sin, mask, kind, H, scale, rpe, dropout_p, rng_state,
                need_grad, salt, table_async=False, kv_img=None, boxes=False, operand_bf16=False, defer_combine=False):
        B, nQ, C = q.shape
        nK = k.shape[1]
        assert C == H * HEAD_DIM, f"embed dim {C} != {H} heads x {HEAD_DIM}"
        bf16 = q.dtype == torch.bfloat16
        if bf16:
            if kind != L.VDETR_ATTN_SHARED_KV or k.dtype != torch.bfloat16 or v.dtype != torch.bfloat16:
                raise RuntimeError("fused_attention: the bf16 path takes bf16 q, k AND v of a shared-KV attention")
            _check_inputs(table=table, vertices=vertices, xyz=xyz, cos_sin=cos_sin)
            L.require_gpu(q, "q")
            L.require_contiguous(q, "q")
        else:
            _check_inputs(q=q, table=table, vertices=vertices, xyz=xyz, cos_sin=cos_sin)
        for name, t in (("k", k), ("v", v)):
            L.require_gpu(t, name)
            if not bf16:
                L.require_float(t, name)
        ks, vs = k.stride(1), v.stride(1)
        lib = L.lib()
        use_drop = dropout_p > 0.0
        rng = rng_state if use_drop else None
        d = _desc(kind, B, H, nQ, nK, scale, table, rpe, vertices, xyz, cos_sin, mask, dropout_p if use_drop else 0.0, rng,
                  salt, ks, vs)
        out = torch.empty(q.shape, dtype=torch.float32, device=q.device)
        rows = (B, nQ, H) if kind == L.VDETR_ATTN_SHARED_KV else (B, H, nQ)
        lse = torch.empty(rows, dtype=torch.float32, device=q.device)
        scores = torch.empty(rows + (nK,), dtype=torch.float32, device=q.device) if need_grad else None
        if kind == L.VDETR_ATTN_PER_HEAD and SELF_FWD_BODY:
            d.fwd_kernel = 4
        if operand_bf16 and not bf16 and FWD_KERNEL == 0:
            d.fwd_kernel = 3
        if kv_img is not None and not bf16 and FWD_KERNEL == 0:
            if not isinstance(kv_img, KVImage):
                raise TypeError("fused_attention: kv_img must be an item of pack_kv_images()")
            want = 1 if operand_bf16 else 3
            if (kv_img.parts, kv_img.B, kv_img.nK) != (want, B, nK) or kv_img.data.device != q.device:
                raise RuntimeError(f"fused_attention: kv_img was packed for parts={kv_img.parts}, B={kv_img.B}, nK={kv_img.nK} on "
                                   f"{kv_img.data.device}; this call needs parts={want}, B={B}, nK={nK} on {q.device}")
            d.kv_img = kv_img.data.data_ptr()
        sched = None
        if table is not None:
            sched = _take_zeros(q, (4,), torch.int32)
            d.fwd_sched = sched.data_ptr()
        nbytes = lib.vdetr_attn_fwd_workspace_bytes(ctypes.byref(d))
        ws = L.workspace(nbytes, q.device) if nbytes else None
        if defer_combine and DEFER_COMBINE and not bf16 and kind == L.VDETR_ATTN_SHARED_KV and H == 4:
            _no_pending("fused_attention")
            parts = L.AttnParts()
            L.check(lib.vdetr_attn_fwd_parts_f32(ctypes.byref(d), L.ptr(q), L.ptr(k), L.ptr(v), L.ptr(out), L.ptr(lse), L.ptr(scores),
                                                 L.ptr(ws), nbytes, ctypes.byref(parts), L.stream_ptr()), "attn_fwd_parts")
            if 2 <= parts.ksplit <= 16:
                _pending_parts[out.data_ptr()] = (parts, ws, lse, out)
            elif parts.ksplit != 1:
                raise RuntimeError(f"fused_attention: {parts.ksplit} key chunks left unmerged and no consumer takes that many")
        else:
            fwd = lib.vdetr_attn_fwd_bf16 if bf16 else lib.vdetr_attn_fwd_f32
            L.check(fwd(ctypes.byref(d), L.ptr(q), L.ptr(k), L.ptr(v), L.ptr(out), L.ptr(lse),
                        L.ptr(scores), L.ptr(ws), nbytes, L.stream_ptr()), "attn_fwd")
        if need_grad:
            ctx.save_for_backward(q, k, v, table, vertices, xyz, cos_sin, mask, out, lse, scores, rng)
            ctx.cfg = (kind, H, scale, rpe, dropout_p if use_drop else 0.0, salt)
            ctx.kv_rec = None if (bf16 or mask is not None) else _kv_register(out, q, v, table, vertices, cos_sin, kind, B, H, nQ, nK)
            ctx.table_async = bool(table_async)
            ctx.boxes = bool(boxes)
            if table_async and table is not None and table.requires_grad and _async_wanted(q.shape[0], q.shape[1], k.shape[1]):
                _step_side[_dev_key(q.device)] = True
        if _kv_by_out and getattr(ctx, "kv_rec", None) is None:
            _kv_by_out.pop(out.data_ptr(), None)
        return out

    @staticmethod
    def backward(ctx, dout):
        q, k, v, table, vertices, xyz, cos_sin, mask, out, lse, scores, rng = ctx.saved_tensors
        kind, H, scale, rpe, dropout_p, salt = ctx.cfg
        in_dtype = q.dtype
        if in_dtype == torch.bfloat16:
            q, k, v = q.float(), k.float().contiguous(), v.float().contiguous()
        B, nQ, C = q.shape
        nK = k.shape[1]
        lib = L.lib()
        dout = dout.contiguous()
        shared = kind == L.VDETR_ATTN_SHARED_KV
        want_table = table is not None and ctx.needs_input_grad[3]
        d = _desc(kind, B, H, nQ, nK, scale, table, rpe, vertices, xyz, cos_sin, mask, dropout_p, rng, salt, 0, v.stride(1))
        if getattr(ctx, "boxes", False) and BWD_KERNEL == 0 and cos_sin is None:
            d.bwd_kernel = 2
        if want_table:
            aux = _take_zeros(q, (8,), torch.int32)
            d.bwd_aux = aux.data_ptr()
        delta = torch.empty((B, nQ, H) if shared else (B, H, nQ), dtype=torch.float32, device=q.device)
        rows_kv, nprob_kv = (4 * nQ, B) if shared else (nQ, B * H)
        fused = (FUSED_KV_BWD and ((shared and H == 4) or (not shared and not want_table))
                 and rows_kv * nK * 4 < (1 << 31) and nprob_kv <= 65535 and v.stride(1) % 4 == 0
                 and all(t.data_ptr() % 16 == 0 for t in (v, lse)))
        if not fused:
            L.check(lib.vdetr_attn_delta_f32(ctypes.byref(d), L.ptr(dout), L.ptr(out), L.ptr(v), L.ptr(delta), L.stream_ptr()),
                    "attn_delta")
        if fused:
            ds = torch.empty_like(scores)
            dkv = torch.empty((2, B, nK, k.shape[2]), dtype=torch.float32, device=q.device)
            run_async = want_table and ctx.table_async and _async_wanted(B, nQ, nK)
            d.kv_waves = 4 if (run_async or _side_keep) and ASYNC_TABLE_GRID >= 256 else 8
            d.kv_halves = 1 if (_side_keep and not shared) else 2
            rec = getattr(ctx, "kv_rec", None)
            if (rec is not None and rec.prepared and rec.emitted == dout.data_ptr() and (rec.aux is not None) == bool(want_table)
                    and in_dtype == torch.float32):
                delta, dkv, aux = rec.delta, rec.dkv, rec.aux
                d.bwd_aux = aux.data_ptr() if aux is not None else None
                L.check(lib.vdetr_attn_bwd_kv_packed_f32(ctypes.byref(d), L.ptr(q), L.ptr(v), L.ptr(dout), L.ptr(scores), L.ptr(lse),
                                                         L.ptr(delta), L.ptr(ds), L.ptr(dkv[0]), L.ptr(dkv[1]), L.ptr(rec.ws), rec.nbytes,
                                                         L.stream_ptr()), "attn_bwd_kv_packed")
            else:
                nbytes = lib.vdetr_attn_bwd_kv_workspace_bytes(ctypes.byref(d))
                ws = L.workspace(nbytes, q.device)
                L.check(lib.vdetr_attn_bwd_kv_delta_f32(ctypes.byref(d), L.ptr(q), L.ptr(v), L.ptr(dout), L.ptr(out), L.ptr(scores),
                                                        L.ptr(lse), L.ptr(delta), L.ptr(ds), L.ptr(dkv[0]), L.ptr(dkv[1]), L.ptr(ws),
                                                        nbytes, L.stream_ptr()), "attn_bwd_kv")
            from .runtime import ts_mark
            ts_mark("main: key-side pass done" if shared else "main: self-attention key-side pass done")
            dtable = fork = None
            if run_async:
                dtable = _table_accumulator(table)
                fork = torch.cuda.Event()
                fork.record(torch.cuda.current_stream(q.device))
            if shared:
                dq = q.new_empty((B, nQ * H, HEAD_DIM))
                torch.baddbmm(dq, ds.view(B, nQ * H, nK), k, beta=0.0, alpha=float(scale), out=dq)
                dq = dq.view(B, nQ, C)
            else:
                ds_r = ds.view(B * H, nQ, nK)
                k4 = k.reshape(B, nK, H, HEAD_DIM).permute(0, 2, 1, 3)
                if B == 1:
                    dq = q.new_empty((1, nQ, C))
                    dq_r = dq.view(nQ, H, HEAD_DIM).permute(1, 0, 2)
                    torch.baddbmm(dq_r, ds_r, k4[0], beta=0.0, alpha=float(scale), out=dq_r)
                else:
                    dq = torch.bmm(ds_r, k4.reshape(B * H, nK, HEAD_DIM)).mul_(float(scale))
                    dq = dq.view(B, H, nQ, HEAD_DIM).permute(0, 2, 1, 3).reshape(B, nQ, C)
            if want_table:
                if run_async:
                    dtable = _launch_table_async(lib, d, q, ds, table, aux, vertices, xyz, mask, fork, dtable, also=(cos_sin, rng))
                else:
                    dtable = _table_accumulator(table)
                    nbytes = lib.vdetr_attn_bwd_workspace_bytes(ctypes.byref(d))
                    ws = L.workspace(nbytes, q.device)
                    L.check(lib.vdetr_attn_bwd_table_f32(ctypes.byref(d), L.ptr(ds), L.ptr(dtable), L.ptr(ws), nbytes,
                                                         L.stream_ptr()), "attn_bwd_table")
            dk, dv = dkv[0], dkv[1]
            if in_dtype == torch.bfloat16:
                dq, dk, dv = dq.to(in_dtype), dk.to(in_dtype), dv.to(in_dtype)
            return (dq, dk, dv, dtable) + (None,) * 17
        if shared:
            do_r = dout.view(B, nQ * H, HEAD_DIM)
            dprob = torch.bmm(do_r, v.transpose(1, 2))
        else:
            def heads(t, n):
                t4 = t.reshape(B, n, H, HEAD_DIM).permute(0, 2, 1, 3)
                return t4[0] if B == 1 else t4.reshape(B * H, n, HEAD_DIM)
            do_r, v_r = heads(dout, nQ), heads(v, nK)
            dprob = torch.bmm(do_r, v_r.transpose(1, 2))
        dtable = _take_zeros(table, tuple(table.shape), table.dtype) if want_table else None
        nbytes = lib.vdetr_attn_bwd_workspace_bytes(ctypes.byref(d)) if want_table else 0
        ws = L.workspace(nbytes, q.device) if nbytes else None
        probs = torch.empty_like(scores) if want_table else scores
        dscore = torch.empty_like(dprob) if want_table else dprob
        L.check(lib.vdetr_attn_bwd_scores_f32(ctypes.byref(d), L.ptr(scores), L.ptr(dprob), L.ptr(lse), L.ptr(delta),
                                              L.ptr(probs), L.ptr(dscore), L.ptr(dtable), L.ptr(ws), nbytes,
                                              L.stream_ptr()), "attn_bwd_scores")
        scores, dprob = probs, dscore
        if shared:
            p_r = scores.view(B, nQ * H, nK)
            ds_r = dprob
            q_r = q.view(B, nQ * H, HEAD_DIM)
            dv = torch.bmm(p_r.transpose(1, 2), do_r)
            dk = torch.bmm(ds_r.transpose(1, 2), q_r)
            dq = torch.bmm(ds_r, k).view(B, nQ, C)
        else:
            p_r = scores.view(B * H, nQ, nK)
            ds_r = dprob
            q_r, k_r = heads(q, nQ), heads(k, nK)
            if B == 1:
                dv, dk, dq = q.new_empty((1, nK, C)), q.new_empty((1, nK, C)), q.new_empty((1, nQ, C))
                torch.bmm(p_r.transpose(1, 2), do_r, out=dv.view(nK, H, HEAD_DIM).permute(1, 0, 2))
                torch.bmm(ds_r.transpose(1, 2), q_r, out=dk.view(nK, H, HEAD_DIM).permute(1, 0, 2))
                torch.bmm(ds_r, k_r, out=dq.view(nQ, H, HEAD_DIM).permute(1, 0, 2))
            else:
                dv = torch.bmm(p_r.transpose(1, 2), do_r).view(B, H, nK, HEAD_DIM).permute(0, 2, 1, 3).reshape(B, nK, C)
                dk = torch.bmm(ds_r.transpose(1, 2), q_r).view(B, H, nK, HEAD_DIM).permute(0, 2, 1, 3).reshape(B, nK, C)
                dq = torch.bmm(ds_r, k_r).view(B, H, nQ, HEAD_DIM).permute(0, 2, 1, 3).reshape(B, nQ, C)
        if in_dtype == torch.bfloat16:
            dq, dk, dv = dq.to(in_dtype), dk.to(in_dtype), dv.to(in_dtype)
        return (dq, dk, dv, dtable) + (None,) * 17


def _kv_layout(t, B, nK):
    mult = 8 if t.dtype == torch.bfloat16 else 4
    ok = (t.dim() == 3 and t.stride(2) == 1 and t.stride(1) % mult == 0 and t.stride(1) >= t.shape[2] and
          t.data_ptr() % 16 == 0 and (B == 1 or t.stride(0) == nK * t.stride(1)))
    return t if ok else t.contiguous()


def fused_attention(q, k, v, *, num_heads, scale, shared_kv, table=None, rpe=None, vertices=None, xyz=None,
                    cos_sin=None, attn_mask=None, dropout_p=0.0, rng_state=None, salt=0, table_grad_async=False, kv_img=None,
                    vertices_are_boxes=False, operand_bf16=False, defer_combine=False):
    B, nQ, _ = q.shape
    nK = k.shape[1]
    kind = L.VDETR_ATTN_SHARED_KV if shared_kv else L.VDETR_ATTN_PER_HEAD
    if dropout_p > 0.0 and rng_state is None:
        rng_state = current_rng(q.device)
        if rng_state is None:
            rng_state = begin_step(q.device)
    mask = _prep_mask(attn_mask, B, nQ, nK)
    need_grad = torch.is_grad_enabled() and any(
        t is not None and t.requires_grad for t in (q, k, v, table))
    if table is not None:
        table = table.contiguous()
        vertices = vertices.detach().contiguous()
        xyz = xyz.detach().contiguous()
        if cos_sin is not None:
            cos_sin = cos_sin.detach().contiguous()
    k, v = _kv_layout(k, B, nK), _kv_layout(v, B, nK)
    return _FusedAttention.apply(q.contiguous(), k, v, table, vertices, xyz, cos_sin, mask,
                                 kind, num_heads, float(scale), rpe, float(dropout_p), rng_state, need_grad, int(salt),
                                 bool(table_grad_async), kv_img, bool(vertices_are_boxes), bool(operand_bf16), bool(defer_combine))


class KVImage:
    __slots__ = ("data", "parts", "B", "nK")

    def __init__(self, data, parts, B, nK):
        self.data, self.parts, self.B, self.nK = data, int(parts), int(B), int(nK)


def pack_kv_images(kv, n, parts=3):
    if (FWD_KERNEL != 0 or not kv.is_cuda or kv.dtype != torch.float32 or not kv.is_contiguous() or kv.shape[2] != n * 2 * HEAD_DIM
            or kv.data_ptr() % 16):
        return None
    B, nK = kv.shape[0], kv.shape[1]
    lib = L.lib()
    nbytes = lib.vdetr_attn_kv_image_parts_bytes(B, nK, parts)
    img = torch.empty((n, nbytes), dtype=torch.uint8, device=kv.device)
    L.check(lib.vdetr_attn_pack_kv_parts_f32(kv.data_ptr(), kv.data_ptr() + 4 * HEAD_DIM, B, nK, kv.shape[2], kv.shape[2], n, 2 * HEAD_DIM,
                                             parts, img.data_ptr(), L.stream_ptr()), "attn_pack_kv")
    return [KVImage(img[i], parts, B, nK) for i in range(n)]


def attention_probabilities(q, k, *, num_heads, scale, shared_kv, table=None, rpe=None, vertices=None, xyz=None,
                            cos_sin=None, attn_mask=None, dropout_p=0.0, rng_state=None, salt=0):
    B, nQ, C = q.shape
    nK = k.shape[1]
    kind = L.VDETR_ATTN_SHARED_KV if shared_kv else L.VDETR_ATTN_PER_HEAD
    mask = _prep_mask(attn_mask, B, nQ, nK)
    lib = L.lib()
    with torch.no_grad():
        q, k = q.detach().contiguous(), k.detach().contiguous()
        if table is not None:
            table, vertices, xyz = table.detach().contiguous(), vertices.detach().contiguous(), xyz.detach().contiguous()
            cos_sin = cos_sin.detach().contiguous() if cos_sin is not None else None
        d = _desc(kind, B, num_heads, nQ, nK, scale, table, rpe, vertices, xyz, cos_sin, mask, dropout_p, rng_state, salt)
        out = torch.empty_like(q)
        rows = (B, nQ, num_heads) if shared_kv else (B, num_heads, nQ)
        lse = torch.empty(rows, dtype=torch.float32, device=q.device)
        scores = torch.empty(rows + (nK,), dtype=torch.float32, device=q.device)
        nbytes = lib.vdetr_attn_fwd_workspace_bytes(ctypes.byref(d))
        ws = L.workspace(nbytes, q.device) if nbytes else None
        L.check(lib.vdetr_attn_fwd_f32(ctypes.byref(d), L.ptr(q), L.ptr(k), L.ptr(k), L.ptr(out), L.ptr(lse),
                                       L.ptr(scores), L.ptr(ws), nbytes, L.stream_ptr()), "attn_fwd")
        L.check(lib.vdetr_attn_bwd_scores_f32(ctypes.byref(d), L.ptr(scores), None, L.ptr(lse), None, L.ptr(scores),
                                              None, None, None, 0, L.stream_ptr()), "attn_probs")
    return scores.permute(0, 2, 1, 3) if shared_kv else scores


def rpe_bias(table, vertices, xyz, rpe, cos_sin=None):
    _check_inputs(table=table, vertices=vertices, xyz=xyz, cos_sin=cos_sin)
    B, nQ = vertices.shape[:2]
    nK = xyz.shape[1]
    H = table.shape[-1]
    d = _desc(L.VDETR_ATTN_SHARED_KV, B, H, nQ, nK, 1.0, table, rpe, vertices, xyz, cos_sin, None, 0.0, None)
    out = torch.empty((B, nQ, H, nK), dtype=torch.float32, device=table.device)
    L.check(L.lib().vdetr_rpe_bias_f32(ctypes.byref(d), L.ptr(out), L.stream_ptr()), "rpe_bias")
    return out.permute(0, 2, 1, 3)


def dropout_keep_mask(B, H, nQ, nK, shared_kv, dropout_p, rng_state, salt=0):
    kind = L.VDETR_ATTN_SHARED_KV if shared_kv else L.VDETR_ATTN_PER_HEAD
    d = _desc(kind, B, H, nQ, nK, 1.0, None, None, None, None, None, None, dropout_p, rng_state, salt)
    rows = (B, nQ, H) if shared_kv else (B, H, nQ)
    keep = torch.empty(rows + (nK,), dtype=torch.uint8, device=rng_state.device)
    L.check(L.lib().vdetr_attn_dropout_mask_u8(ctypes.byref(d), L.ptr(keep), L.stream_ptr()), "dropout_mask")
    return keep.permute(0, 2, 1, 3) if shared_kv else keep
```

v-detr_amd/csrc/attn_bwd_kv.hip:

```cpp
#include "kv_pack.h"

#include <stdlib.h>

#include <atomic>

namespace vdetr {

int attn_fill_params(const vdetr_attn_desc* d, AttnParams* P, const char* op);

typedef float f32x16 __attribute__((ext_vector_type(16)));


struct KvParams {
  AttnParams A;
  const float* dout;
  float* dk;
  float* dv;
  uint4* pack;
  int R, NT;
};

struct KvProblem {
  const float* q;
  const float* dout;
  const float* v;
  float* dk;
  float* dv;
  size_t score_off;
  size_t row_off;
  int rstride, ostride, b, head;
};
template <bool PERHEAD>
__device__ __forceinline__ KvProblem kv_problem(const KvParams& K, int prob) {
  const AttnParams& P = K.A;
  KvProblem p;
  if (PERHEAD) {
    const int b = prob / P.H, hh = prob - b * P.H, C = P.H * kDh;
    p.b = b; p.head = hh;
    p.q = P.q + (size_t)b * P.nQ * C + hh * kDh;
    p.dout = K.dout + (size_t)b * P.nQ * C + hh * kDh;
    p.rstride = C;
    p.v = P.v + (size_t)b * P.nK * P.v_stride + hh * kDh;
    p.dk = K.dk + (size_t)b * P.nK * C + hh * kDh;
    p.dv = K.dv + (size_t)b * P.nK * C + hh * kDh;
    p.ostride = C;
  } else {
    p.b = prob; p.head = 0;
    p.q = P.q + (size_t)prob * K.R * kDh;
    p.dout = K.dout + (size_t)prob * K.R * kDh;
    p.rstride = kDh;
    p.v = P.v + (size_t)prob * P.nK * P.v_stride;
    p.dk = K.dk + (size_t)prob * P.nK * kDh;
    p.dv = K.dv + (size_t)prob * P.nK * kDh;
    p.ostride = kDh;
  }
  p.score_off = (size_t)prob * K.R * P.nK;
  p.row_off = (size_t)prob * K.R;
  return p;
}


__device__ __forceinline__ f32x16 kv_mfma(bf16x8 a, bf16x8 b, f32x16 c) {
  return __builtin_amdgcn_mfma_f32_32x32x16_bf16(a, b, c, 0, 0, 0);
}
__device__ __forceinline__ f32x16 kv_mfma3(bf16x8 ah, bf16x8 al, bf16x8 bh, bf16x8 bl, f32x16 c) {
  c = kv_mfma(al, bh, c);
  c = kv_mfma(ah, bl, c);
  return kv_mfma(ah, bh, c);
}

template <bool PERHEAD>
__global__ __launch_bounds__(256) void attn_bwd_kv_pack_kernel(KvParams K, DeltaArgs D, int ndelta) {
  if ((int)blockIdx.x < ndelta) {
    __shared__ float wmax[4];
    attn_delta_body(D, (int)blockIdx.x, wmax);
    return;
  }
  const AttnParams& P = K.A;
  const int R = K.R, NT = K.NT;
  const int nprob = PERHEAD ? P.B * P.H : P.B;
  const long gid = (long)((int)blockIdx.x - ndelta) * 256 + threadIdx.x, stride = (long)((int)gridDim.x - ndelta) * 256;
  const long nunits = (long)nprob * NT * 12 * kWave;
  for (long u = gid; u < nunits; u += stride) {
    const int lane = (int)(u & 63);
    long r = u >> 6;
    const int sub = (int)(r & 3);
    r >>= 2;
    const int kind = (int)(r % 3);
    const long bt = r / 3;
    const int prob = (int)(bt / NT), tile = (int)(bt - (long)prob * NT), r0 = tile * 32;
    const int l31 = lane & 31, g = lane >> 5;
    const KvProblem pb = kv_problem<PERHEAD>(K, prob);
    const float* src = kind == 2 ? pb.q : pb.dout;
    float x[8];
    if (kind == 0) {
      const int row = r0 + l31;
#pragma unroll
      for (int e = 0; e < 8; ++e) x[e] = row < R ? src[(size_t)row * pb.rstride + 16 * sub + 8 * g + e] : 0.f;
    } else {
      const int d = 32 * (sub >> 1) + l31, t = sub & 1;
#pragma unroll
      for (int e = 0; e < 8; ++e) {
        const int row = r0 + kv_row(8 * t + e, g);
        x[e] = row < R ? src[(size_t)row * pb.rstride + d] : 0.f;
      }
    }
    bf16x8 hi, lo;
    kv_split8(x, hi, lo);
    uint4* dst = K.pack + ((bt * 3 + kind) * 4 + sub) * kKvOperandUnits;
    dst[lane] = __builtin_bit_cast(uint4, hi);
    dst[kWave + lane] = __builtin_bit_cast(uint4, lo);
  }
  const long nz = (long)P.B * P.nK * (PERHEAD ? P.H : 1) * kDh / 4;
  f32x4* zk = reinterpret_cast<f32x4*>(K.dk);
  f32x4* zv = reinterpret_cast<f32x4*>(K.dv);
  for (long i = gid; i < nz; i += stride) {
    zk[i] = f32x4{0.f, 0.f, 0.f, 0.f};
    zv[i] = f32x4{0.f, 0.f, 0.f, 0.f};
  }
}

template <bool PERHEAD, int WAVES, int HALVES = 2>
__global__ __launch_bounds__(WAVES * kWave) void attn_bwd_kv_kernel(KvParams K) {
  constexpr int kKvWaves = WAVES, kKvThreads = WAVES * kWave, kKvSlots = HALVES * WAVES;
  AttnParams P = K.A;
  attn_load_rng(P);
  extern __shared__ __attribute__((aligned(16))) float smem[];
  const int tid = threadIdx.x, lane = tid & 63;
  const int w = __builtin_amdgcn_readfirstlane(tid >> 6);
  const int l31 = lane & 31, g = lane >> 5;
  const int kt = blockIdx.x / HALVES, hf = blockIdx.x % HALVES, prob = blockIdx.y;
  const KvProblem pb = kv_problem<PERHEAD>(K, prob);
  const int b = pb.b;
  const int R = K.R, NT = K.NT, nK = P.nK;
  const int key = kt * 32 + l31;
  const bool kvalid = key < nK;

  uint4* vstrip = reinterpret_cast<uint4*>(smem) + w * (8 * kWave) + lane;
  {
    const float* vrow = pb.v + (size_t)(kvalid ? key : 0) * P.v_stride + 8 * g;
#pragma unroll
    for (int s = 0; s < 4; ++s) {
      const f32x4 a = *reinterpret_cast<const f32x4*>(vrow + 16 * s), c = *reinterpret_cast<const f32x4*>(vrow + 16 * s + 4);
      float x[8] = {a[0], a[1], a[2], a[3], c[0], c[1], c[2], c[3]};
      if (!kvalid) {
#pragma unroll
        for (int e = 0; e < 8; ++e) x[e] = 0.f;
      }
      bf16x8 hi, lo;
      kv_split8(x, hi, lo);
      vstrip[(2 * s) * kWave] = __builtin_bit_cast(uint4, hi);
      vstrip[(2 * s + 1) * kWave] = __builtin_bit_cast(uint4, lo);
    }
  }
  f32x16 accV[2], accK[2];
#pragma unroll
  for (int i = 0; i < 16; ++i) { accV[0][i] = 0.f; accV[1][i] = 0.f; accK[0][i] = 0.f; accK[1][i] = 0.f; }

  using rsrc_t = __amdgpu_buffer_rsrc_t;
  const unsigned recs = (unsigned)((size_t)R * nK * 4);
  const rsrc_t rs = __builtin_amdgcn_make_buffer_rsrc(P.scores + pb.score_off, 0, (int)recs, 0x00020000);
  const rsrc_t rd = __builtin_amdgcn_make_buffer_rsrc(P.ds_out + pb.score_off, 0, (int)recs, 0x00020000);
  const int rowbytes = nK * 4;
  const unsigned lane_off = kvalid ? (unsigned)(4 * g * rowbytes + key * 4) : 0x80000000u;
  const float* lse_b = P.lse + pb.row_off;
  const float* delta_b = P.delta + pb.row_off;
  const bool has_mask = P.mask_kind == VDETR_MASK_BOOL;
  const unsigned char* mask_b = reinterpret_cast<const unsigned char*>(P.mask) + (size_t)b * P.nQ * nK + (kvalid ? key : 0);

  auto load_scores = [&](int tile, float (&sv)[16]) {
#pragma unroll
    for (int a = 0; a < 4; ++a) {
      const unsigned voff = lane_off + (unsigned)((tile * 32 + 8 * a) * rowbytes);
#pragma unroll
      for (int h = 0; h < 4; ++h)
        sv[4 * a + h] = __builtin_bit_cast(float, __builtin_amdgcn_raw_buffer_load_b32(rs, (int)(voff + (unsigned)(h * rowbytes)), 0, kStreamAux));
    }
  };
  const int first = hf * kKvWaves + w;
  float sv[16], sn[16];
  if (first < NT) load_scores(first, sn);

  for (int tile = first; tile < NT; tile += kKvSlots) {
    const int r0 = tile * 32;
#pragma unroll
    for (int i = 0; i < 16; ++i) sv[i] = sn[i];
    const uint4* pk = K.pack + ((size_t)prob * NT + tile) * kKvTileUnits + lane;
    auto operand = [&](int kind, int sub, int hl) { return pk[((kind * 4 + sub) * 2 + hl) * kWave]; };
    auto row_consts = [&](int t, float (&lv)[8], float (&dv)[8]) {
#pragma unroll
      for (int a2 = 0; a2 < 2; ++a2) {
        const int rb = r0 + 8 * (2 * t + a2) + 4 * g;
        if (PERHEAD) {
#pragma unroll
          for (int h = 0; h < 4; ++h) {
            const int row = min(rb + h, R - 1);
            lv[4 * a2 + h] = lse_b[row];
            dv[4 * a2 + h] = delta_b[row];
          }
        } else {
          const f32x4 l4 = *reinterpret_cast<const f32x4*>(lse_b + min(rb, R - 4));
          const f32x4 d4 = *reinterpret_cast<const f32x4*>(delta_b + min(rb, R - 4));
#pragma unroll
          for (int h = 0; h < 4; ++h) { lv[4 * a2 + h] = l4[h]; dv[4 * a2 + h] = d4[h]; }
        }
      }
    };
    uint4 opA[8], opB[8];
#pragma unroll
    for (int s = 0; s < 4; ++s) { opA[2 * s] = operand(0, s, 0); opA[2 * s + 1] = operand(0, s, 1); }
#pragma unroll
    for (int mt = 0; mt < 2; ++mt) {
      opB[2 * mt] = operand(1, 2 * mt, 0); opB[2 * mt + 1] = operand(1, 2 * mt, 1);
      opB[4 + 2 * mt] = operand(2, 2 * mt, 0); opB[4 + 2 * mt + 1] = operand(2, 2 * mt, 1);
    }
    float lv0[8], dv0[8];
    row_consts(0, lv0, dv0);
    __builtin_amdgcn_sched_barrier(0);
    f32x16 dp;
#pragma unroll
    for (int i = 0; i < 16; ++i) dp[i] = 0.f;
#pragma unroll
    for (int s = 0; s < 4; ++s) {
      const bf16x8 vh = __builtin_bit_cast(bf16x8, vstrip[(2 * s) * kWave]), vl = __builtin_bit_cast(bf16x8, vstrip[(2 * s + 1) * kWave]);
      dp = kv_mfma3(__builtin_bit_cast(bf16x8, opA[2 * s]), __builtin_bit_cast(bf16x8, opA[2 * s + 1]), vh, vl, dp);
    }
    __builtin_amdgcn_sched_barrier(0);
#pragma unroll
    for (int mt = 0; mt < 2; ++mt) {
      opA[2 * mt] = operand(1, 2 * mt + 1, 0); opA[2 * mt + 1] = operand(1, 2 * mt + 1, 1);
      opA[4 + 2 * mt] = operand(2, 2 * mt + 1, 0); opA[4 + 2 * mt + 1] = operand(2, 2 * mt + 1, 1);
    }
    float lv1[8], dv1[8];
    row_consts(1, lv1, dv1);
    if (tile + kKvSlots < NT) load_scores(tile + kKvSlots, sn);
    __builtin_amdgcn_sched_barrier(0);
#pragma unroll
    for (int t = 0; t < 2; ++t) {
      float xp[8], xs[8];
#pragma unroll
      for (int a2 = 0; a2 < 2; ++a2) {
        const int a = 2 * t + a2;
        const int rb = r0 + 8 * a + 4 * g;
        const unsigned voff = lane_off + (unsigned)((r0 + 8 * a) * rowbytes);
        uint4 rnd = make_uint4(0xFFFFu, 0xFFFFu, 0xFFFFu, 0xFFFFu);
        bool masked = false;
        if (!PERHEAD) {
          const int qi = min(rb, R - 4) >> 2;
          if (P.drop_thresh) rnd = attn_rand4(P, b, qi, key, 0);
          if (has_mask) masked = mask_b[(size_t)qi * nK] != 0;
        }
#pragma unroll
        for (int h = 0; h < 4; ++h) {
          const int v = 4 * a + h, e = 4 * a2 + h;
          const bool ok = rb + h < R && kvalid;
          int pick = h;
          if (PERHEAD) {
            const int qi = min(rb + h, R - 1);
            if (P.drop_thresh) rnd = attn_rand4(P, b, qi, key, pb.head >> 2);
            if (has_mask) masked = mask_b[(size_t)qi * nK] != 0;
            pick = pb.head & 3;
          }
          const bool keep = pick4(rnd, pick) >= P.drop_thresh;
          const ScoreGrad gr = score_grad(sv[v], t ? lv1[e] : lv0[e], keep, P.drop_scale, true, dp[v], t ? dv1[e] : dv0[e], masked);
          xp[e] = ok ? gr.p_drop : 0.f;
          xs[e] = ok ? gr.ds : 0.f;
          __builtin_amdgcn_raw_buffer_store_b32(__float_as_int(gr.ds), rd, (int)(voff + (unsigned)(h * rowbytes)), 0, kStreamAux);
        }
      }
      bf16x8 ph, pl, sh, sl;
      kv_split8(xp, ph, pl);
      kv_split8(xs, sh, sl);
      const uint4* op = t ? opA : opB;
#pragma unroll
      for (int mt = 0; mt < 2; ++mt) {
        accV[mt] = kv_mfma3(__builtin_bit_cast(bf16x8, op[2 * mt]), __builtin_bit_cast(bf16x8, op[2 * mt + 1]), ph, pl, accV[mt]);
        accK[mt] = kv_mfma3(__builtin_bit_cast(bf16x8, op[4 + 2 * mt]), __builtin_bit_cast(bf16x8, op[4 + 2 * mt + 1]), sh, sl, accK[mt]);
      }
      __builtin_amdgcn_sched_barrier(0);
    }
  }
  __syncthreads();

  auto put = [&](int slot) {
    float* dst = smem + (size_t)slot * 64 * kWave + lane;
#pragma unroll
    for (int i = 0; i < 16; ++i) {
      dst[i * kWave] = accV[0][i]; dst[(16 + i) * kWave] = accV[1][i];
      dst[(32 + i) * kWave] = accK[0][i]; dst[(48 + i) * kWave] = accK[1][i];
    }
  };
  auto add = [&](int slot) {
    const float* src = smem + (size_t)slot * 64 * kWave + lane;
#pragma unroll
    for (int i = 0; i < 16; ++i) {
      accV[0][i] += src[i * kWave]; accV[1][i] += src[(16 + i) * kWave];
      accK[0][i] += src[(32 + i) * kWave]; accK[1][i] += src[(48 + i) * kWave];
    }
  };
#pragma unroll
  for (int half = kKvWaves / 2; half >= 1; half >>= 1) {
    if (w >= half && w < 2 * half) put(w - half);
    __syncthreads();
    if (w < half) add(w);
    __syncthreads();
  }
  constexpr int kFinStride = kDh + 1;
  if (w == 0) {
#pragma unroll
    for (int mt = 0; mt < 2; ++mt)
#pragma unroll
      for (int i = 0; i < 16; ++i) {
        const int d = 32 * mt + kv_row(i, g);
        smem[l31 * kFinStride + d] = accV[mt][i];
        smem[(32 + l31) * kFinStride + d] = accK[mt][i] * P.scale;
      }
  }
  __syncthreads();
  for (int idx = tid; idx < 2 * 32 * kDh; idx += kKvThreads) {
    const int which = idx >> 11, kl = (idx >> 6) & 31, d = idx & 63;
    const int kg = kt * 32 + kl;
    if (kg < nK) unsafeAtomicAdd((which ? pb.dk : pb.dv) + (size_t)kg * pb.ostride + d, smem[(which * 32 + kl) * kFinStride + d]);
  }
}

constexpr int kPrepMax = 16;
struct PrepItem {
  const float* q; const float* v; const float* vertices; const float* cos_sin;
  uint4* pack; float* dk; float* dv; unsigned* aux;
  int B, H, nQ, nK, v_stride, perhead;
};
struct PrepBatch { PrepItem it[kPrepMax]; };

__global__ __launch_bounds__(256) void attn_bwd_kv_prep_kernel(PrepBatch Bt) {
  const PrepItem& I = Bt.it[blockIdx.y];
  const int lane = threadIdx.x & 63, wv = threadIdx.x >> 6;
  const int nvb = I.aux ? (int)(((long)I.B * I.nK + 4 * kDeltaKeys - 1) / (4 * kDeltaKeys)) : 0;
  const int nqb = (I.aux && I.vertices) ? (int)(((long)I.B * I.nQ + 3) / 4) : 0;
  int blk = blockIdx.x;
  if (blk < nvb) {
    __shared__ float wmax[4];
    float n2max = 0.f;
    const int key0 = (blk * 4 + wv) * kDeltaKeys;
#pragma unroll 4
    for (int i = 0; i < kDeltaKeys; ++i) {
      const int key = key0 + i;
      const float x = key < I.B * I.nK ? I.v[(size_t)key * I.v_stride + lane] : 0.f;
      n2max = fmaxf(n2max, wave_allsum_f32(x * x));
    }
    if (lane == 0) wmax[wv] = n2max;
    __syncthreads();
    if (threadIdx.x == 0) atomicMax(I.aux + 1, __float_as_uint(fmaxf(fmaxf(wmax[0], wmax[1]), fmaxf(wmax[2], wmax[3]))));
    return;
  }
  blk -= nvb;
  if (blk < nqb) {
    const int row = blk * 4 + wv;
    if (row >= I.B * I.nQ) return;
    if (row == 0 && lane == 0) I.aux[5] = 1u;
    const float* vp = I.vertices + (size_t)row * 24;
    const int i = lane & 7;
    bool ok;
    if (!I.cos_sin) {
      ok = vp[i * 3] == vp[rpe_box_xi(i) ? 6 : 0] && vp[i * 3 + 1] == vp[rpe_box_yi(i) ? 4 : 1] && vp[i * 3 + 2] == vp[rpe_box_zi(i) ? 14 : 2];
    } else {
      float ex = vp[i * 3] - vp[0], ey = vp[i * 3 + 1] - vp[1];
      const float ez = vp[i * 3 + 2] - vp[2];
      rpe_rotate(ex, ey, I.cos_sin[(size_t)row * 2], I.cos_sin[(size_t)row * 2 + 1]);
      const float EX = readlane_f32(ex, 3), EY = readlane_f32(ey, 1), EZ = readlane_f32(ez, 4);
      const float tol = 1e-5f * (1.f + fabsf(vp[0]) + fabsf(vp[1]) + fabsf(vp[2]));
      ok = fabsf(ex - (rpe_box_xi(i) ? EX : 0.f)) <= tol && fabsf(ey - (rpe_box_yi(i) ? EY : 0.f)) <= tol &&
           fabsf(ez - (rpe_box_zi(i) ? EZ : 0.f)) <= tol;
    }
    if (!__all(ok) && lane == 0) atomicAdd(I.aux + 4, 1u);
    return;
  }
  blk -= nqb;
  const int nwork = (int)gridDim.x - nvb - nqb;
  if (nwork <= 0) return;
  const int C = I.H * kDh;
  const int R = I.perhead ? I.nQ : I.H * I.nQ, NT = (R + 31) / 32, nprob = I.perhead ? I.B * I.H : I.B;
  const long gid = (long)blk * 256 + threadIdx.x, stride = (long)nwork * 256;
  const long nunits = (long)nprob * NT * 4 * kWave;
  for (long u = gid; u < nunits; u += stride) {
    const int ln = (int)(u & 63), sub = (int)((u >> 6) & 3);
    const long bt = u >> 8;
    const int prob = (int)(bt / NT), tile = (int)(bt - (long)prob * NT), r0 = tile * 32;
    const int l31 = ln & 31, g = ln >> 5, d = 32 * (sub >> 1) + l31, t = sub & 1;
    const float* src;
    int rstride;
    if (I.perhead) {
      const int b = prob / I.H, hh = prob - b * I.H;
      src = I.q + (size_t)b * I.nQ * C + hh * kDh;
      rstride = C;
    } else {
      src = I.q + (size_t)prob * R * kDh;
      rstride = kDh;
    }
    float x[8];
#pragma unroll
    for (int e = 0; e < 8; ++e) {
      const int row = r0 + kv_row(8 * t + e, g);
      x[e] = row < R ? src[(size_t)row * rstride + d] : 0.f;
    }
    kv_store_unit(I.pack, bt, 2, sub, ln, x);
  }
  const long nz = (long)I.B * I.nK * (I.perhead ? I.H : 1) * kDh / 4;
  f32x4* zk = reinterpret_cast<f32x4*>(I.dk);
  f32x4* zv = reinterpret_cast<f32x4*>(I.dv);
  for (long i = gid; i < nz; i += stride) {
    zk[i] = f32x4{0.f, 0.f, 0.f, 0.f};
    zv[i] = f32x4{0.f, 0.f, 0.f, 0.f};
  }
}

}

using namespace vdetr;

static bool kv_supported(const vdetr_attn_desc* d) {
  return d && ((d->kind == VDETR_ATTN_SHARED_KV && d->H == 4) || d->kind == VDETR_ATTN_PER_HEAD);
}
static size_t kv_rows(const vdetr_attn_desc* d) { return d->kind == VDETR_ATTN_PER_HEAD ? (size_t)d->nQ : (size_t)d->nQ * 4; }
static size_t kv_problems(const vdetr_attn_desc* d) { return d->kind == VDETR_ATTN_PER_HEAD ? (size_t)d->B * d->H : (size_t)d->B; }

extern "C" size_t vdetr_attn_bwd_kv_workspace_bytes(const vdetr_attn_desc* d) {
  if (!kv_supported(d) || d->B <= 0 || d->nQ <= 0 || d->H <= 0) return 0;
  const size_t nt = (kv_rows(d) + 31) / 32;
  return kv_problems(d) * nt * kKvTileUnits * sizeof(uint4) + 256;
}

template <bool PERHEAD, int WAVES, int HALVES = 2>
static int kv_launch(const KvParams& K, int nkt, int nprob, long pack_work, const DeltaArgs& D, int ndelta, bool packed, hipStream_t st) {
  const unsigned pack_blocks = (unsigned)((pack_work + 255) / 256 < 2048 ? (pack_work + 255) / 256 : 2048);
  if (!packed) {
    hipLaunchKernelGGL(attn_bwd_kv_pack_kernel<PERHEAD>, dim3(pack_blocks + (unsigned)ndelta), dim3(256), 0, st, K, D, ndelta);
    if (int e = check_launch("attn_bwd_kv_pack")) return e;
  }
  const size_t strips = (size_t)WAVES * 8 * kWave * sizeof(uint4), tree = (size_t)(WAVES / 2) * 64 * kWave * sizeof(float);
  const size_t fin = (size_t)2 * 32 * (kDh + 1) * sizeof(float);
  const size_t lds = strips > tree ? (strips > fin ? strips : fin) : (tree > fin ? tree : fin);
  if (int e = set_lds(attn_bwd_kv_kernel<PERHEAD, WAVES, HALVES>, lds, "attn_bwd_kv")) return e;
  hipLaunchKernelGGL((attn_bwd_kv_kernel<PERHEAD, WAVES, HALVES>), dim3(HALVES * nkt, nprob), dim3(WAVES * kWave), lds, st, K);
  return check_launch("attn_bwd_kv");
}

static int kv_run(const vdetr_attn_desc* d, const float* q, const float* v, const float* dout, const float* out,
                  const float* scores, const float* lse, float* delta, float* ds_out, float* dk, float* dv, void* workspace,
                  size_t workspace_bytes, vdetr_stream_t stream, bool packed = false) {
  KvParams K;
  if (int e = attn_fill_params(d, &K.A, "attn_bwd_kv")) return e;
  VDETR_REQUIRE(kv_supported(d), "attn_bwd_kv: built for shared K/V with 4 heads and for per-head K/V (kind %d, H %d)", d->kind, d->H);
  VDETR_REQUIRE(q && v && dout && scores && lse && delta && ds_out && dk && dv, "attn_bwd_kv: null pointer");
  VDETR_REQUIRE(K.A.v_stride % 4 == 0 && (((uintptr_t)v | (uintptr_t)lse | (uintptr_t)delta | (uintptr_t)dk | (uintptr_t)dv) & 15) == 0,
                "attn_bwd_kv: v rows, lse, delta, dk and dv must be 16-B aligned");
  const size_t rows = kv_rows(d), nprob = kv_problems(d);
  VDETR_REQUIRE(rows * d->nK * 4 < ((size_t)1 << 31), "attn_bwd_kv: a score matrix (%zu x %d) must stay below 2 GB", rows, d->nK);
  VDETR_REQUIRE(nprob <= 65535, "attn_bwd_kv: %zu score matrices > 65535", nprob);
  const size_t need = vdetr_attn_bwd_kv_workspace_bytes(d);
  if (!workspace || workspace_bytes < need) {
    set_error("attn_bwd_kv: workspace %zu B < required %zu B", workspace_bytes, need);
    return VDETR_ERR_WORKSPACE;
  }
  K.A.q = q; K.A.v = v;
  K.A.scores = const_cast<float*>(scores); K.A.lse = const_cast<float*>(lse); K.A.delta = delta; K.A.ds_out = ds_out;
  K.dout = dout; K.dk = dk; K.dv = dv;
  K.pack = reinterpret_cast<uint4*>(((uintptr_t)workspace + 255) & ~(uintptr_t)255);
  K.R = (int)rows;
  K.NT = (K.R + 31) / 32;
  const long units = (long)nprob * K.NT * 12 * kWave;
  const long zero4 = (long)d->B * d->nK * (d->kind == VDETR_ATTN_PER_HEAD ? d->H : 1) * kDh / 4;
  const long work = units > zero4 ? units : zero4;
  const int nkt = (d->nK + 31) / 32;
  VDETR_REQUIRE(d->kv_waves == 0 || d->kv_waves == 4 || d->kv_waves == 8, "attn_bwd_kv: kv_waves %d (0, 4 or 8)", d->kv_waves);
  VDETR_REQUIRE(d->kv_halves == 0 || d->kv_halves == 1 || d->kv_halves == 2, "attn_bwd_kv: kv_halves %d (0, 1 or 2)", d->kv_halves);
  const bool four = d->kv_waves == 4;
  const bool one = d->kv_halves == 1 && !four;
  hipStream_t st = (hipStream_t)stream;
  DeltaArgs D{};
  int ndelta = 0;
  if (out) {
    VDETR_REQUIRE(!d->bwd_aux || d->kind == VDETR_ATTN_SHARED_KV, "attn_bwd_kv: bwd_aux needs the shared-KV kind");
    attn_delta_args(d, dout, out, v, delta, &D);
    ndelta = D.qblocks + D.vblocks;
  }
  if (d->kind == VDETR_ATTN_PER_HEAD) {
    if (one) return kv_launch<true, 8, 1>(K, nkt, (int)nprob, work, D, ndelta, packed, st);
    return four ? kv_launch<true, 4>(K, nkt, (int)nprob, work, D, ndelta, packed, st) : kv_launch<true, 8>(K, nkt, (int)nprob, work, D, ndelta, packed, st);
  }
  if (one) return kv_launch<false, 8, 1>(K, nkt, (int)nprob, work, D, ndelta, packed, st);
  return four ? kv_launch<false, 4>(K, nkt, (int)nprob, work, D, ndelta, packed, st) : kv_launch<false, 8>(K, nkt, (int)nprob, work, D, ndelta, packed, st);
}

extern "C" int vdetr_attn_bwd_kv_f32(const vdetr_attn_desc* d, const float* q, const float* v, const float* dout,
                                     const float* scores, const float* lse, const float* delta, float* ds_out, float* dk,
                                     float* dv, void* workspace, size_t workspace_bytes, vdetr_stream_t stream) {
  return kv_run(d, q, v, dout, nullptr, scores, lse, const_cast<float*>(delta), ds_out, dk, dv, workspace, workspace_bytes, stream);
}

extern "C" int vdetr_attn_bwd_kv_delta_f32(const vdetr_attn_desc* d, const float* q, const float* v, const float* dout,
                                           const float* out, const float* scores, const float* lse, float* delta, float* ds_out,
                                           float* dk, float* dv, void* workspace, size_t workspace_bytes, vdetr_stream_t stream) {
  VDETR_REQUIRE(out, "attn_bwd_kv_delta: null pointer (out)");
  return kv_run(d, q, v, dout, out, scores, lse, delta, ds_out, dk, dv, workspace, workspace_bytes, stream);
}

extern "C" int vdetr_attn_bwd_kv_packed_f32(const vdetr_attn_desc* d, const float* q, const float* v, const float* dout, const float* scores,
                                            const float* lse, const float* delta, float* ds_out, float* dk, float* dv, void* workspace,
                                            size_t workspace_bytes, vdetr_stream_t stream) {
  VDETR_REQUIRE(workspace && (((uintptr_t)workspace) & 255) == 0, "attn_bwd_kv_packed: the workspace (the operand images) must be 256-B aligned");
  return kv_run(d, q, v, dout, nullptr, scores, lse, const_cast<float*>(delta), ds_out, dk, dv, workspace, workspace_bytes, stream, true);
}

extern "C" int vdetr_attn_bwd_kv_prep_f32(const vdetr_attn_kv_prep* items, int n, vdetr_stream_t stream) {
  VDETR_REQUIRE(items && n >= 1 && n <= kPrepMax, "attn_bwd_kv_prep: %d items (1..%d)", n, kPrepMax);
  PrepBatch Bt;
  long blocks = 1;
  for (int i = 0; i < n; ++i) {
    const vdetr_attn_kv_prep& s = items[i];
    VDETR_REQUIRE(s.q && s.v && s.workspace && s.dk && s.dv, "attn_bwd_kv_prep: null pointer in item %d", i);
    VDETR_REQUIRE(s.kind == VDETR_ATTN_SHARED_KV || s.kind == VDETR_ATTN_PER_HEAD, "attn_bwd_kv_prep: kind %d", s.kind);
    VDETR_REQUIRE(s.B > 0 && s.nQ > 0 && s.nK > 0 && s.H == 4, "attn_bwd_kv_prep: item %d: B=%d nQ=%d nK=%d H=%d (4 heads)", i, s.B, s.nQ, s.nK, s.H);
    VDETR_REQUIRE((((uintptr_t)s.workspace) & 255) == 0 && (((uintptr_t)s.dk | (uintptr_t)s.dv) & 15) == 0, "attn_bwd_kv_prep: item %d: alignment", i);
    VDETR_REQUIRE(s.kind == VDETR_ATTN_SHARED_KV || !s.bwd_aux, "attn_bwd_kv_prep: bwd_aux needs the shared-KV kind");
    PrepItem& I = Bt.it[i];
    I.q = s.q; I.v = s.v; I.vertices = s.vertices; I.cos_sin = s.vertices ? s.cos_sin : nullptr;
    I.pack = reinterpret_cast<uint4*>(s.workspace); I.dk = s.dk; I.dv = s.dv; I.aux = s.bwd_aux;
    I.B = s.B; I.H = s.H; I.nQ = s.nQ; I.nK = s.nK;
    I.perhead = s.kind == VDETR_ATTN_PER_HEAD ? 1 : 0;
    I.v_stride = s.v_row_stride ? s.v_row_stride : (I.perhead ? s.H * 64 : 64);
    const long nvb = s.bwd_aux ? ((long)s.B * s.nK + 4 * kDeltaKeys - 1) / (4 * kDeltaKeys) : 0;
    const long nqb = (s.bwd_aux && s.vertices) ? ((long)s.B * s.nQ + 3) / 4 : 0;
    const long R = I.perhead ? s.nQ : (long)s.H * s.nQ, NT = (R + 31) / 32, nprob = I.perhead ? (long)s.B * s.H : s.B;
    const long units = nprob * NT * 4 * kWave, zero4 = (long)s.B * s.nK * (I.perhead ? s.H : 1) * kDh / 4;
    long work = ((units > zero4 ? units : zero4) + 255) / 256;
    work = work < 1 ? 1 : (work > 512 ? 512 : work);
    blocks = blocks > nvb + nqb + work ? blocks : nvb + nqb + work;
  }
  for (int i = n; i < kPrepMax; ++i) Bt.it[i] = Bt.it[0];
  hipLaunchKernelGGL(attn_bwd_kv_prep_kernel, dim3((unsigned)blocks, n), dim3(256), 0, (hipStream_t)stream, Bt);
  return check_launch("attn_bwd_kv_prep");
}
```

v-detr_amd/csrc/kv_pack.h:

```cpp
#pragma once
#include "attn_common.h"

namespace vdetr {

typedef __bf16 bf16x8 __attribute__((ext_vector_type(8)));

constexpr int kKvOperandUnits = 2 * kWave;
constexpr int kKvTileUnits = 3 * 4 * kKvOperandUnits;

__device__ __forceinline__ constexpr int kv_row(int v, int g) { return (v & 3) + 8 * (v >> 2) + 4 * g; }

__device__ __forceinline__ void kv_split8(const float (&x)[8], bf16x8& hi, bf16x8& lo) {
#pragma unroll
  for (int e = 0; e < 8; ++e) {
    const __bf16 h = (__bf16)x[e];
    hi[e] = h;
    lo[e] = (__bf16)(x[e] - (float)h);
  }
}

__device__ __forceinline__ void kv_store_unit(uint4* pack, long tile, int kind, int sub, int lane, const float (&x)[8]) {
  bf16x8 hi, lo;
  kv_split8(x, hi, lo);
  uint4* dst = pack + ((tile * 3 + kind) * 4 + sub) * kKvOperandUnits;
  dst[lane] = __builtin_bit_cast(uint4, hi);
  dst[kWave + lane] = __builtin_bit_cast(uint4, lo);
}

struct KvEmit {
  uint4* pack;
  float* delta;
  const float* out;
  unsigned* aux;
  int per_head, nQ;
};
__device__ __forceinline__ void kv_emit_rows16(const KvEmit& E, const float* xs, int stride, int q0, int tid, float* wmax) {
  const int NT = E.per_head ? E.nQ / 32 : E.nQ / 8;
  {
    const int pair = tid >> 2, quarter = tid & 3, ql = pair >> 2, h = pair & 3;
    const float* orow = E.out + ((size_t)(q0 + ql) * 4 + h) * kDh + 16 * quarter;
    const float* drow = xs + ql * stride + h * kDh + 16 * quarter;
    float s = 0.f, n2 = 0.f;
#pragma unroll
    for (int i = 0; i < 4; ++i) {
      const f32x4 o = *reinterpret_cast<const f32x4*>(orow + 4 * i);
      const f32x4 g = *reinterpret_cast<const f32x4*>(drow + 4 * i);
#pragma unroll
      for (int e = 0; e < 4; ++e) { s = fmaf(g[e], o[e], s); n2 = fmaf(g[e], g[e], n2); }
    }
    s += dpp_f32<kDppQuadXor1>(s); s += dpp_f32<kDppQuadXor2>(s);
    n2 += dpp_f32<kDppQuadXor1>(n2); n2 += dpp_f32<kDppQuadXor2>(n2);
    if (quarter == 0) E.delta[E.per_head ? (size_t)h * E.nQ + q0 + ql : (size_t)(q0 + ql) * 4 + h] = s;
    if (E.aux) {
      for (int m = 32; m >= 1; m >>= 1) n2 = fmaxf(n2, __shfl_xor(n2, m, 64));
      if ((tid & 63) == 0) wmax[tid >> 6] = n2;
    }
  }
#pragma unroll
  for (int u = 0; u < 4; ++u) {
    const int id = tid + 256 * u;
    float x[8];
    if (!E.per_head) {
      const int tl = id >> 9, unit = (id >> 6) & 7, lane = id & 63, kind = unit >> 2, sub = unit & 3, l31 = lane & 31, g = lane >> 5;
      if (kind == 0) {
        const float* src = xs + (tl * 8 + (l31 >> 2)) * stride + (l31 & 3) * kDh + 16 * sub + 8 * g;
        const f32x4 a = *reinterpret_cast<const f32x4*>(src), b = *reinterpret_cast<const f32x4*>(src + 4);
#pragma unroll
        for (int e = 0; e < 4; ++e) { x[e] = a[e]; x[4 + e] = b[e]; }
      } else {
        const int d = 32 * (sub >> 1) + l31, t = sub & 1;
#pragma unroll
        for (int e = 0; e < 8; ++e) {
          const int row = kv_row(8 * t + e, g);
          x[e] = xs[(tl * 8 + (row >> 2)) * stride + (row & 3) * kDh + d];
        }
      }
      kv_store_unit(E.pack, (long)(q0 >> 3) + tl, kind, sub, lane, x);
    } else {
      const int head = id >> 8, rem = id & 255, half = (q0 >> 4) & 1;
      const long tile = (long)head * NT + (q0 >> 5);
      if (rem < 128) {
        const int sub = rem >> 5, j = rem & 31, rl = j & 15, g = j >> 4, lane = 16 * half + rl + 32 * g;
        const float* src = xs + rl * stride + head * kDh + 16 * sub + 8 * g;
        const f32x4 a = *reinterpret_cast<const f32x4*>(src), b = *reinterpret_cast<const f32x4*>(src + 4);
#pragma unroll
        for (int e = 0; e < 4; ++e) { x[e] = a[e]; x[4 + e] = b[e]; }
        kv_store_unit(E.pack, tile, 0, sub, lane, x);
      } else {
        const int mt = (rem - 128) >> 6, lane = rem & 63, l31 = lane & 31, g = lane >> 5, d = 32 * mt + l31;
#pragma unroll
        for (int e = 0; e < 8; ++e) x[e] = xs[(kv_row(8 * half + e, g) - 16 * half) * stride + head * kDh + d];
        kv_store_unit(E.pack, tile, 1, 2 * mt + half, lane, x);
      }
    }
  }
  if (E.aux) {
    __syncthreads();
    if (tid == 0) atomicMax(E.aux, __float_as_uint(fmaxf(fmaxf(wmax[0], wmax[1]), fmaxf(wmax[2], wmax[3]))));
  }
}

}
```

Before: 158.9.

## Fuse self-attention backward dQ, dK, dV into one launch with prepacked K/V images

Adds a dedicated self-attention backward path for per-head, 4-head, unmasked, table-free attention. Key-owner blocks compute dK/dV while row-owner blocks compute dQ inside a single kernel launch, using bf16 hi/lo split images of K and V packed ahead of time alongside the existing dout/q prepack. This removes the materialised ds matrix and the separate dQ launch, at the cost of recomputing score gradients in both block types and extra workspace for the images. It also extends the prep struct and the Python bindings.

```diff
diff --git a/include/vdetr_hip.h b/include/vdetr_hip.h
--- a/include/vdetr_hip.h
+++ b/include/vdetr_hip.h
@@ -137,11 +137,17 @@
   void* workspace;
   float *dk, *dv;
   uint32_t* bwd_aux;
+  const float* k;
+  int32_t k_row_stride, reserved;
 } vdetr_attn_kv_prep;
 int vdetr_attn_bwd_kv_prep_f32(const vdetr_attn_kv_prep* items, int n, vdetr_stream_t stream);
 int vdetr_attn_bwd_kv_packed_f32(const vdetr_attn_desc* d, const float* q, const float* v, const float* dout, const float* scores,
                                  const float* lse, const float* delta, float* ds_out, float* dk, float* dv, void* workspace,
                                  size_t workspace_bytes, vdetr_stream_t stream);
+size_t vdetr_attn_bwd_self_workspace_bytes(const vdetr_attn_desc* d);
+int vdetr_attn_bwd_self_f32(const vdetr_attn_desc* d, const float* q, const float* k, const float* v, const float* dout,
+                            const float* out, const float* scores, const float* lse, float* delta, float* dq, float* dk, float* dv,
+                            void* workspace, size_t workspace_bytes, vdetr_stream_t stream);
 typedef struct vdetr_rb_attn_emit {
   void* workspace;
   float* delta;
diff --git a/v-detr_amd/_lib.py b/v-detr_amd/_lib.py
--- a/v-detr_amd/_lib.py
+++ b/v-detr_amd/_lib.py
@@ -162,7 +162,8 @@
 class AttnKvPrep(ctypes.Structure):
 
     _fields_ = [(n, ctypes.c_int32) for n in ("kind", "B", "H", "nQ", "nK", "v_row_stride")] + [
-        (n, c_void_p) for n in ("q", "v", "vertices", "cos_sin", "workspace", "dk", "dv", "bwd_aux")]
+        (n, c_void_p) for n in ("q", "v", "vertices", "cos_sin", "workspace", "dk", "dv", "bwd_aux", "k")] + [
+        ("k_row_stride", ctypes.c_int32), ("reserved", ctypes.c_int32)]
 
 
 class RbAttnEmit(ctypes.Structure):
@@ -369,6 +370,8 @@
     "vdetr_rb_proj_q_bwd_emit_f32": (c_int, [ctypes.POINTER(RbProjQDesc), ctypes.POINTER(RbProjQGrads), ctypes.POINTER(RbAttnEmit), c_void_p]),
     "vdetr_attn_bwd_kv_prep_f32": (c_int, [ctypes.POINTER(AttnKvPrep), c_int, c_void_p]),
     "vdetr_attn_bwd_kv_packed_f32": (c_int, [ctypes.POINTER(AttnDesc)] + [c_void_p] * 10 + [c_size_t, c_void_p]),
+    "vdetr_attn_bwd_self_workspace_bytes": (c_size_t, [ctypes.POINTER(AttnDesc)]),
+    "vdetr_attn_bwd_self_f32": (c_int, [ctypes.POINTER(AttnDesc)] + [c_void_p] * 12 + [c_size_t, c_void_p]),
     "vdetr_probe_timestamp": (c_int, [c_void_p, c_void_p]),
     "vdetr_topk_order_f32": (c_int, [c_void_p, c_int, c_int, c_int, c_void_p, c_void_p]),
     "vdetr_anchor_boxes_f32": (c_int, [c_void_p] * 5 + [c_int] * 3 + [c_void_p] * 5),
diff --git a/v-detr_amd/attention.py b/v-detr_amd/attention.py
--- a/v-detr_amd/attention.py
+++ b/v-detr_amd/attention.py
@@ -444,15 +444,23 @@
 
 
 KV_PREPACK = os.environ.get("VDETR_KV_PREPACK", "1") != "0"
+SELF_BWD_ONE_LAUNCH = True
 _kv_recs = {}
 _kv_by_out = {}
 
 
 class _KvRec:
-    __slots__ = ("q", "v", "vertices", "cos_sin", "kind", "dims", "want_aux", "ws", "nbytes", "dkv", "delta", "aux", "prepared", "emitted")
-
-
-def _kv_register(out, q, v, table, vertices, cos_sin, kind, B, H, nQ, nK):
+    __slots__ = ("q", "v", "vertices", "cos_sin", "kind", "dims", "want_aux", "ws", "nbytes", "dkv", "delta", "aux", "prepared", "emitted",
+                 "k", "self_img")
+
+
+def _self_bwd_ok(q, k, v, kind, B, H, nQ, nK):
+    return (kind == L.VDETR_ATTN_PER_HEAD and H == 4 and nQ % 32 == 0 and nK % 32 == 0 and q.dtype == torch.float32
+            and k.dtype == torch.float32 and v.dtype == torch.float32 and k.stride(2) == 1 and k.stride(1) % 4 == 0
+            and (B == 1 or k.stride(0) == nK * k.stride(1)) and k.data_ptr() % 16 == 0 and v.data_ptr() % 16 == 0)
+
+
+def _kv_register(out, q, v, table, vertices, cos_sin, kind, B, H, nQ, nK, k=None):
     shared = kind == L.VDETR_ATTN_SHARED_KV
     if not (KV_PREPACK and FUSED_KV_BWD and B == 1 and H == 4 and nQ % 32 == 0 and q.dtype == torch.float32 and v.dtype == torch.float32
             and (shared or table is None) and v.stride(1) % 4 == 0 and v.data_ptr() % 16 == 0 and 4 * nQ * nK * 4 < (1 << 31)):
@@ -461,6 +469,8 @@
     r.q, r.v, r.vertices, r.cos_sin, r.kind, r.dims = q, v, (vertices if table is not None else None), cos_sin, kind, (B, H, nQ, nK)
     r.want_aux = bool(table is not None and table.requires_grad)
     r.prepared, r.emitted = False, None
+    r.k = k if (k is not None and table is None and _self_bwd_ok(q, k, v, kind, B, H, nQ, nK)) else None
+    r.self_img = False
     r.ws = r.dkv = r.delta = r.aux = None
     lst = _kv_recs.setdefault(_dev_key(q.device), [])
     if len(lst) >= 64:
@@ -491,7 +501,8 @@
             shared = r.kind == L.VDETR_ATTN_SHARED_KV
             dd = L.AttnDesc()
             dd.kind, dd.B, dd.H, dd.nQ, dd.nK = r.kind, B, H, nQ, nK
-            r.nbytes = lib.vdetr_attn_bwd_kv_workspace_bytes(ctypes.byref(dd))
+            r.self_img = bool(SELF_BWD_ONE_LAUNCH and r.k is not None)
+            r.nbytes = (lib.vdetr_attn_bwd_self_workspace_bytes if r.self_img else lib.vdetr_attn_bwd_kv_workspace_bytes)(ctypes.byref(dd))
             r.ws = L.workspace(r.nbytes, dev)
             assert r.ws.data_ptr() % 256 == 0
             r.dkv = torch.empty((2, B, nK, 64 if shared else H * 64), dtype=torch.float32, device=dev)
@@ -503,6 +514,7 @@
             it.cos_sin = r.cos_sin.data_ptr() if (r.cos_sin is not None and it.vertices) else None
             it.workspace, it.dk, it.dv = r.ws.data_ptr(), r.dkv[0].data_ptr(), r.dkv[1].data_ptr()
             it.bwd_aux = r.aux.data_ptr() if r.aux is not None else None
+            it.k, it.k_row_stride = (r.k.data_ptr(), r.k.stride(1)) if r.self_img else (None, 0)
         L.check(lib.vdetr_attn_bwd_kv_prep_f32(items, len(chunk), L.stream_ptr()), "attn_bwd_kv_prep")
         for r in chunk:
             r.prepared = True
@@ -572,7 +584,7 @@
         if need_grad:
             ctx.save_for_backward(q, k, v, table, vertices, xyz, cos_sin, mask, out, lse, scores, rng)
             ctx.cfg = (kind, H, scale, rpe, dropout_p if use_drop else 0.0, salt)
-            ctx.kv_rec = None if (bf16 or mask is not None) else _kv_register(out, q, v, table, vertices, cos_sin, kind, B, H, nQ, nK)
+            ctx.kv_rec = None if (bf16 or mask is not None) else _kv_register(out, q, v, table, vertices, cos_sin, kind, B, H, nQ, nK, k)
             ctx.table_async = bool(table_async)
             ctx.boxes = bool(boxes)
             if table_async and table is not None and table.requires_grad and _async_wanted(q.shape[0], q.shape[1], k.shape[1]):
@@ -608,6 +620,26 @@
         if not fused:
             L.check(lib.vdetr_attn_delta_f32(ctypes.byref(d), L.ptr(dout), L.ptr(out), L.ptr(v), L.ptr(delta), L.stream_ptr()),
                     "attn_delta")
+        if (fused and SELF_BWD_ONE_LAUNCH and not shared and table is None and mask is None and in_dtype == torch.float32
+                and _self_bwd_ok(q, k, v, kind, B, H, nQ, nK) and scores.data_ptr() % 16 == 0):
+            d.k_row_stride = k.stride(1)
+            dq = q.new_empty((B, nQ, C))
+            rec = getattr(ctx, "kv_rec", None)
+            if rec is not None and rec.prepared and rec.self_img and rec.emitted == dout.data_ptr() and rec.aux is None:
+                dkv = rec.dkv
+                L.check(lib.vdetr_attn_bwd_self_f32(ctypes.byref(d), L.ptr(q), L.ptr(k), L.ptr(v), L.ptr(dout), None, L.ptr(scores),
+                                                    L.ptr(lse), L.ptr(rec.delta), L.ptr(dq), L.ptr(dkv[0]), L.ptr(dkv[1]), L.ptr(rec.ws),
+                                                    rec.nbytes, L.stream_ptr()), "attn_bwd_self")
+            else:
+                dkv = torch.empty((2, B, nK, C), dtype=torch.float32, device=q.device)
+                nbytes = lib.vdetr_attn_bwd_self_workspace_bytes(ctypes.byref(d))
+                ws = L.workspace(nbytes, q.device)
+                L.check(lib.vdetr_attn_bwd_self_f32(ctypes.byref(d), L.ptr(q), L.ptr(k), L.ptr(v), L.ptr(dout), L.ptr(out), L.ptr(scores),
+                                                    L.ptr(lse), L.ptr(delta), L.ptr(dq), L.ptr(dkv[0]), L.ptr(dkv[1]), L.ptr(ws), nbytes,
+                                                    L.stream_ptr()), "attn_bwd_self")
+            from .runtime import ts_mark
+            ts_mark("main: self-attention key-side pass done")
+            return (dq, dkv[0], dkv[1], None) + (None,) * 17
         if fused:
             ds = torch.empty_like(scores)
             dkv = torch.empty((2, B, nK, k.shape[2]), dtype=torch.float32, device=q.device)
diff --git a/v-detr_amd/csrc/attn_bwd_kv.hip b/v-detr_amd/csrc/attn_bwd_kv.hip
--- a/v-detr_amd/csrc/attn_bwd_kv.hip
+++ b/v-detr_amd/csrc/attn_bwd_kv.hip
@@ -1,4 +1,4 @@
-#include "kv_pack.h"
+#include "attn_bwd_kv_body.h"
 
 #include <stdlib.h>
 
@@ -7,67 +7,6 @@
 namespace vdetr {
 
 int attn_fill_params(const vdetr_attn_desc* d, AttnParams* P, const char* op);
-
-typedef float f32x16 __attribute__((ext_vector_type(16)));
-
-
-struct KvParams {
-  AttnParams A;
-  const float* dout;
-  float* dk;
-  float* dv;
-  uint4* pack;
-  int R, NT;
-};
-
-struct KvProblem {
-  const float* q;
-  const float* dout;
-  const float* v;
-  float* dk;
-  float* dv;
-  size_t score_off;
-  size_t row_off;
-  int rstride, ostride, b, head;
-};
-template <bool PERHEAD>
-__device__ __forceinline__ KvProblem kv_problem(const KvParams& K, int prob) {
-  const AttnParams& P = K.A;
-  KvProblem p;
-  if (PERHEAD) {
-    const int b = prob / P.H, hh = prob - b * P.H, C = P.H * kDh;
-    p.b = b; p.head = hh;
-    p.q = P.q + (size_t)b * P.nQ * C + hh * kDh;
-    p.dout = K.dout + (size_t)b * P.nQ * C + hh * kDh;
-    p.rstride = C;
-    p.v = P.v + (size_t)b * P.nK * P.v_stride + hh * kDh;
-    p.dk = K.dk + (size_t)b * P.nK * C + hh * kDh;
-    p.dv = K.dv + (size_t)b * P.nK * C + hh * kDh;
-    p.ostride = C;
-  } else {
-    p.b = prob; p.head = 0;
-    p.q = P.q + (size_t)prob * K.R * kDh;
-    p.dout = K.dout + (size_t)prob * K.R * kDh;
-    p.rstride = kDh;
-    p.v = P.v + (size_t)prob * P.nK * P.v_stride;
-    p.dk = K.dk + (size_t)prob * P.nK * kDh;
-    p.dv = K.dv + (size_t)prob * P.nK * kDh;
-    p.ostride = kDh;
-  }
-  p.score_off = (size_t)prob * K.R * P.nK;
-  p.row_off = (size_t)prob * K.R;
-  return p;
-}
-
-
-__device__ __forceinline__ f32x16 kv_mfma(bf16x8 a, bf16x8 b, f32x16 c) {
-  return __builtin_amdgcn_mfma_f32_32x32x16_bf16(a, b, c, 0, 0, 0);
-}
-__device__ __forceinline__ f32x16 kv_mfma3(bf16x8 ah, bf16x8 al, bf16x8 bh, bf16x8 bl, f32x16 c) {
-  c = kv_mfma(al, bh, c);
-  c = kv_mfma(ah, bl, c);
-  return kv_mfma(ah, bh, c);
-}
 
 template <bool PERHEAD>
 __global__ __launch_bounds__(256) void attn_bwd_kv_pack_kernel(KvParams K, DeltaArgs D, int ndelta) {
@@ -76,252 +15,13 @@
     attn_delta_body(D, (int)blockIdx.x, wmax);
     return;
   }
-  const AttnParams& P = K.A;
-  const int R = K.R, NT = K.NT;
-  const int nprob = PERHEAD ? P.B * P.H : P.B;
-  const long gid = (long)((int)blockIdx.x - ndelta) * 256 + threadIdx.x, stride = (long)((int)gridDim.x - ndelta) * 256;
-  const long nunits = (long)nprob * NT * 12 * kWave;
-  for (long u = gid; u < nunits; u += stride) {
-    const int lane = (int)(u & 63);
-    long r = u >> 6;
-    const int sub = (int)(r & 3);
-    r >>= 2;
-    const int kind = (int)(r % 3);
-    const long bt = r / 3;
-    const int prob = (int)(bt / NT), tile = (int)(bt - (long)prob * NT), r0 = tile * 32;
-    const int l31 = lane & 31, g = lane >> 5;
-    const KvProblem pb = kv_problem<PERHEAD>(K, prob);
-    const float* src = kind == 2 ? pb.q : pb.dout;
-    float x[8];
-    if (kind == 0) {
-      const int row = r0 + l31;
-#pragma unroll
-      for (int e = 0; e < 8; ++e) x[e] = row < R ? src[(size_t)row * pb.rstride + 16 * sub + 8 * g + e] : 0.f;
-    } else {
-      const int d = 32 * (sub >> 1) + l31, t = sub & 1;
-#pragma unroll
-      for (int e = 0; e < 8; ++e) {
-        const int row = r0 + kv_row(8 * t + e, g);
-        x[e] = row < R ? src[(size_t)row * pb.rstride + d] : 0.f;
-      }
-    }
-    bf16x8 hi, lo;
-    kv_split8(x, hi, lo);
-    uint4* dst = K.pack + ((bt * 3 + kind) * 4 + sub) * kKvOperandUnits;
-    dst[lane] = __builtin_bit_cast(uint4, hi);
-    dst[kWave + lane] = __builtin_bit_cast(uint4, lo);
-  }
-  const long nz = (long)P.B * P.nK * (PERHEAD ? P.H : 1) * kDh / 4;
-  f32x4* zk = reinterpret_cast<f32x4*>(K.dk);
-  f32x4* zv = reinterpret_cast<f32x4*>(K.dv);
-  for (long i = gid; i < nz; i += stride) {
-    zk[i] = f32x4{0.f, 0.f, 0.f, 0.f};
-    zv[i] = f32x4{0.f, 0.f, 0.f, 0.f};
-  }
+  kv_pack_body<PERHEAD>(K, (long)((int)blockIdx.x - ndelta) * 256 + threadIdx.x, (long)((int)gridDim.x - ndelta) * 256);
 }
 
 template <bool PERHEAD, int WAVES, int HALVES = 2>
 __global__ __launch_bounds__(WAVES * kWave) void attn_bwd_kv_kernel(KvParams K) {
-  constexpr int kKvWaves = WAVES, kKvThreads = WAVES * kWave, kKvSlots = HALVES * WAVES;
-  AttnParams P = K.A;
-  attn_load_rng(P);
   extern __shared__ __attribute__((aligned(16))) float smem[];
-  const int tid = threadIdx.x, lane = tid & 63;
-  const int w = __builtin_amdgcn_readfirstlane(tid >> 6);
-  const int l31 = lane & 31, g = lane >> 5;
-  const int kt = blockIdx.x / HALVES, hf = blockIdx.x % HALVES, prob = blockIdx.y;
-  const KvProblem pb = kv_problem<PERHEAD>(K, prob);
-  const int b = pb.b;
-  const int R = K.R, NT = K.NT, nK = P.nK;
-  const int key = kt * 32 + l31;
-  const bool kvalid = key < nK;
-
-  uint4* vstrip = reinterpret_cast<uint4*>(smem) + w * (8 * kWave) + lane;
-  {
-    const float* vrow = pb.v + (size_t)(kvalid ? key : 0) * P.v_stride + 8 * g;
-#pragma unroll
-    for (int s = 0; s < 4; ++s) {
-      const f32x4 a = *reinterpret_cast<const f32x4*>(vrow + 16 * s), c = *reinterpret_cast<const f32x4*>(vrow + 16 * s + 4);
-      float x[8] = {a[0], a[1], a[2], a[3], c[0], c[1], c[2], c[3]};
-      if (!kvalid) {
-#pragma unroll
-        for (int e = 0; e < 8; ++e) x[e] = 0.f;
-      }
-      bf16x8 hi, lo;
-      kv_split8(x, hi, lo);
-      vstrip[(2 * s) * kWave] = __builtin_bit_cast(uint4, hi);
-      vstrip[(2 * s + 1) * kWave] = __builtin_bit_cast(uint4, lo);
-    }
-  }
-  f32x16 accV[2], accK[2];
-#pragma unroll
-  for (int i = 0; i < 16; ++i) { accV[0][i] = 0.f; accV[1][i] = 0.f; accK[0][i] = 0.f; accK[1][i] = 0.f; }
-
-  using rsrc_t = __amdgpu_buffer_rsrc_t;
-  const unsigned recs = (unsigned)((size_t)R * nK * 4);
-  const rsrc_t rs = __builtin_amdgcn_make_buffer_rsrc(P.scores + pb.score_off, 0, (int)recs, 0x00020000);
-  const rsrc_t rd = __builtin_amdgcn_make_buffer_rsrc(P.ds_out + pb.score_off, 0, (int)recs, 0x00020000);
-  const int rowbytes = nK * 4;
-  const unsigned lane_off = kvalid ? (unsigned)(4 * g * rowbytes + key * 4) : 0x80000000u;
-  const float* lse_b = P.lse + pb.row_off;
-  const float* delta_b = P.delta + pb.row_off;
-  const bool has_mask = P.mask_kind == VDETR_MASK_BOOL;
-  const unsigned char* mask_b = reinterpret_cast<const unsigned char*>(P.mask) + (size_t)b * P.nQ * nK + (kvalid ? key : 0);
-
-  auto load_scores = [&](int tile, float (&sv)[16]) {
-#pragma unroll
-    for (int a = 0; a < 4; ++a) {
-      const unsigned voff = lane_off + (unsigned)((tile * 32 + 8 * a) * rowbytes);
-#pragma unroll
-      for (int h = 0; h < 4; ++h)
-        sv[4 * a + h] = __builtin_bit_cast(float, __builtin_amdgcn_raw_buffer_load_b32(rs, (int)(voff + (unsigned)(h * rowbytes)), 0, kStreamAux));
-    }
-  };
-  const int first = hf * kKvWaves + w;
-  float sv[16], sn[16];
-  if (first < NT) load_scores(first, sn);
-
-  for (int tile = first; tile < NT; tile += kKvSlots) {
-    const int r0 = tile * 32;
-#pragma unroll
-    for (int i = 0; i < 16; ++i) sv[i] = sn[i];
-    const uint4* pk = K.pack + ((size_t)prob * NT + tile) * kKvTileUnits + lane;
-    auto operand = [&](int kind, int sub, int hl) { return pk[((kind * 4 + sub) * 2 + hl) * kWave]; };
-    auto row_consts = [&](int t, float (&lv)[8], float (&dv)[8]) {
-#pragma unroll
-      for (int a2 = 0; a2 < 2; ++a2) {
-        const int rb = r0 + 8 * (2 * t + a2) + 4 * g;
-        if (PERHEAD) {
-#pragma unroll
-          for (int h = 0; h < 4; ++h) {
-            const int row = min(rb + h, R - 1);
-            lv[4 * a2 + h] = lse_b[row];
-            dv[4 * a2 + h] = delta_b[row];
-          }
-        } else {
-          const f32x4 l4 = *reinterpret_cast<const f32x4*>(lse_b + min(rb, R - 4));
-          const f32x4 d4 = *reinterpret_cast<const f32x4*>(delta_b + min(rb, R - 4));
-#pragma unroll
-          for (int h = 0; h < 4; ++h) { lv[4 * a2 + h] = l4[h]; dv[4 * a2 + h] = d4[h]; }
-        }
-      }
-    };
-    uint4 opA[8], opB[8];
-#pragma unroll
-    for (int s = 0; s < 4; ++s) { opA[2 * s] = operand(0, s, 0); opA[2 * s + 1] = operand(0, s, 1); }
-#pragma unroll
-    for (int mt = 0; mt < 2; ++mt) {
-      opB[2 * mt] = operand(1, 2 * mt, 0); opB[2 * mt + 1] = operand(1, 2 * mt, 1);
-      opB[4 + 2 * mt] = operand(2, 2 * mt, 0); opB[4 + 2 * mt + 1] = operand(2, 2 * mt, 1);
-    }
-    float lv0[8], dv0[8];
-    row_consts(0, lv0, dv0);
-    __builtin_amdgcn_sched_barrier(0);
-    f32x16 dp;
-#pragma unroll
-    for (int i = 0; i < 16; ++i) dp[i] = 0.f;
-#pragma unroll
-    for (int s = 0; s < 4; ++s) {
-      const bf16x8 vh = __builtin_bit_cast(bf16x8, vstrip[(2 * s) * kWave]), vl = __builtin_bit_cast(bf16x8, vstrip[(2 * s + 1) * kWave]);
-      dp = kv_mfma3(__builtin_bit_cast(bf16x8, opA[2 * s]), __builtin_bit_cast(bf16x8, opA[2 * s + 1]), vh, vl, dp);
-    }
-    __builtin_amdgcn_sched_barrier(0);
-#pragma unroll
-    for (int mt = 0; mt < 2; ++mt) {
-      opA[2 * mt] = operand(1, 2 * mt + 1, 0); opA[2 * mt + 1] = operand(1, 2 * mt + 1, 1);
-      opA[4 + 2 * mt] = operand(2, 2 * mt + 1, 0); opA[4 + 2 * mt + 1] = operand(2, 2 * mt + 1, 1);
-    }
-    float lv1[8], dv1[8];
-    row_consts(1, lv1, dv1);
-    if (tile + kKvSlots < NT) load_scores(tile + kKvSlots, sn);
-    __builtin_amdgcn_sched_barrier(0);
-#pragma unroll
-    for (int t = 0; t < 2; ++t) {
-      float xp[8], xs[8];
-#pragma unroll
-      for (int a2 = 0; a2 < 2; ++a2) {
-        const int a = 2 * t + a2;
-        const int rb = r0 + 8 * a + 4 * g;
-        const unsigned voff = lane_off + (unsigned)((r0 + 8 * a) * rowbytes);
-        uint4 rnd = make_uint4(0xFFFFu, 0xFFFFu, 0xFFFFu, 0xFFFFu);
-        bool masked = false;
-        if (!PERHEAD) {
-          const int qi = min(rb, R - 4) >> 2;
-          if (P.drop_thresh) rnd = attn_rand4(P, b, qi, key, 0);
-          if (has_mask) masked = mask_b[(size_t)qi * nK] != 0;
-        }
-#pragma unroll
-        for (int h = 0; h < 4; ++h) {
-          const int v = 4 * a + h, e = 4 * a2 + h;
-          const bool ok = rb + h < R && kvalid;
-          int pick = h;
-          if (PERHEAD) {
-            const int qi = min(rb + h, R - 1);
-            if (P.drop_thresh) rnd = attn_rand4(P, b, qi, key, pb.head >> 2);
-            if (has_mask) masked = mask_b[(size_t)qi * nK] != 0;
-            pick = pb.head & 3;
-          }
-          const bool keep = pick4(rnd, pick) >= P.drop_thresh;
-          const ScoreGrad gr = score_grad(sv[v], t ? lv1[e] : lv0[e], keep, P.drop_scale, true, dp[v], t ? dv1[e] : dv0[e], masked);
-          xp[e] = ok ? gr.p_drop : 0.f;
-          xs[e] = ok ? gr.ds : 0.f;
-          __builtin_amdgcn_raw_buffer_store_b32(__float_as_int(gr.ds), rd, (int)(voff + (unsigned)(h * rowbytes)), 0, kStreamAux);
-        }
-      }
-      bf16x8 ph, pl, sh, sl;
-      kv_split8(xp, ph, pl);
-      kv_split8(xs, sh, sl);
-      const uint4* op = t ? opA : opB;
-#pragma unroll
-      for (int mt = 0; mt < 2; ++mt) {
-        accV[mt] = kv_mfma3(__builtin_bit_cast(bf16x8, op[2 * mt]), __builtin_bit_cast(bf16x8, op[2 * mt + 1]), ph, pl, accV[mt]);
-        accK[mt] = kv_mfma3(__builtin_bit_cast(bf16x8, op[4 + 2 * mt]), __builtin_bit_cast(bf16x8, op[4 + 2 * mt + 1]), sh, sl, accK[mt]);
-      }
-      __builtin_amdgcn_sched_barrier(0);
-    }
-  }
-  __syncthreads();
-
-  auto put = [&](int slot) {
-    float* dst = smem + (size_t)slot * 64 * kWave + lane;
-#pragma unroll
-    for (int i = 0; i < 16; ++i) {
-      dst[i * kWave] = accV[0][i]; dst[(16 + i) * kWave] = accV[1][i];
-      dst[(32 + i) * kWave] = accK[0][i]; dst[(48 + i) * kWave] = accK[1][i];
-    }
-  };
-  auto add = [&](int slot) {
-    const float* src = smem + (size_t)slot * 64 * kWave + lane;
-#pragma unroll
-    for (int i = 0; i < 16; ++i) {
-      accV[0][i] += src[i * kWave]; accV[1][i] += src[(16 + i) * kWave];
-      accK[0][i] += src[(32 + i) * kWave]; accK[1][i] += src[(48 + i) * kWave];
-    }
-  };
-#pragma unroll
-  for (int half = kKvWaves / 2; half >= 1; half >>= 1) {
-    if (w >= half && w < 2 * half) put(w - half);
-    __syncthreads();
-    if (w < half) add(w);
-    __syncthreads();
-  }
-  constexpr int kFinStride = kDh + 1;
-  if (w == 0) {
-#pragma unroll
-    for (int mt = 0; mt < 2; ++mt)
-#pragma unroll
-      for (int i = 0; i < 16; ++i) {
-        const int d = 32 * mt + kv_row(i, g);
-        smem[l31 * kFinStride + d] = accV[mt][i];
-        smem[(32 + l31) * kFinStride + d] = accK[mt][i] * P.scale;
-      }
-  }
-  __syncthreads();
-  for (int idx = tid; idx < 2 * 32 * kDh; idx += kKvThreads) {
-    const int which = idx >> 11, kl = (idx >> 6) & 31, d = idx & 63;
-    const int kg = kt * 32 + kl;
-    if (kg < nK) unsafeAtomicAdd((which ? pb.dk : pb.dv) + (size_t)kg * pb.ostride + d, smem[(which * 32 + kl) * kFinStride + d]);
-  }
+  kv_key_owner_body<PERHEAD, WAVES, HALVES, false>(K, smem, blockIdx.x / HALVES, blockIdx.x % HALVES, blockIdx.y);
 }
 
 constexpr int kPrepMax = 16;
@@ -329,6 +29,7 @@
   const float* q; const float* v; const float* vertices; const float* cos_sin;
   uint4* pack; float* dk; float* dv; unsigned* aux;
   int B, H, nQ, nK, v_stride, perhead;
+  const float* k; uint4* self_img; int k_stride;
 };
 struct PrepBatch { PrepItem it[kPrepMax]; };
 
@@ -412,6 +113,7 @@
     zk[i] = f32x4{0.f, 0.f, 0.f, 0.f};
     zv[i] = f32x4{0.f, 0.f, 0.f, 0.f};
   }
+  if (I.self_img) kv_self_images(I.self_img, I.k, I.v, I.k_stride, I.v_stride, I.B, I.H, I.nK, gid, stride);
 }
 
 }
@@ -529,11 +231,20 @@
     I.B = s.B; I.H = s.H; I.nQ = s.nQ; I.nK = s.nK;
     I.perhead = s.kind == VDETR_ATTN_PER_HEAD ? 1 : 0;
     I.v_stride = s.v_row_stride ? s.v_row_stride : (I.perhead ? s.H * 64 : 64);
+    I.k = s.k; I.self_img = nullptr; I.k_stride = s.k_row_stride ? s.k_row_stride : s.H * 64;
+    if (s.k) {
+      VDETR_REQUIRE(I.perhead && s.nQ % 32 == 0 && s.nK % 32 == 0 && I.k_stride % 4 == 0 && (((uintptr_t)s.k | (uintptr_t)s.v) & 15) == 0,
+                    "attn_bwd_kv_prep: item %d: k is for the per-head kind with nQ, nK multiples of 32 and 16-B aligned k / v rows", i);
+      vdetr_attn_desc dd{};
+      dd.kind = s.kind; dd.B = s.B; dd.H = s.H; dd.nQ = s.nQ; dd.nK = s.nK;
+      I.self_img = reinterpret_cast<uint4*>(reinterpret_cast<char*>(s.workspace) + kv_self_image_offset(vdetr_attn_bwd_kv_workspace_bytes(&dd)));
+    }
     const long nvb = s.bwd_aux ? ((long)s.B * s.nK + 4 * kDeltaKeys - 1) / (4 * kDeltaKeys) : 0;
     const long nqb = (s.bwd_aux && s.vertices) ? ((long)s.B * s.nQ + 3) / 4 : 0;
     const long R = I.perhead ? s.nQ : (long)s.H * s.nQ, NT = (R + 31) / 32, nprob = I.perhead ? (long)s.B * s.H : s.B;
     const long units = nprob * NT * 4 * kWave, zero4 = (long)s.B * s.nK * (I.perhead ? s.H : 1) * kDh / 4;
-    long work = ((units > zero4 ? units : zero4) + 255) / 256;
+    const long self_units = s.k ? nprob * (s.nK / 32) * 8 * kWave : 0;
+    long work = ((units > zero4 ? (units > self_units ? units : self_units) : (zero4 > self_units ? zero4 : self_units)) + 255) / 256;
     work = work < 1 ? 1 : (work > 512 ? 512 : work);
     blocks = blocks > nvb + nqb + work ? blocks : nvb + nqb + work;
   }
diff --git a/v-detr_amd/csrc/attn_bwd_kv_body.h b/v-detr_amd/csrc/attn_bwd_kv_body.h
--- /dev/null
+++ b/v-detr_amd/csrc/attn_bwd_kv_body.h
@@ -0,0 +1,319 @@
+#pragma once
+#include "kv_pack.h"
+
+namespace vdetr {
+
+typedef float f32x16 __attribute__((ext_vector_type(16)));
+
+struct KvParams {
+  AttnParams A;
+  const float* dout;
+  float* dk;
+  float* dv;
+  uint4* pack;
+  int R, NT;
+};
+
+struct KvProblem {
+  const float* q;
+  const float* dout;
+  const float* v;
+  float* dk;
+  float* dv;
+  size_t score_off;
+  size_t row_off;
+  int rstride, ostride, b, head;
+};
+template <bool PERHEAD>
+__device__ __forceinline__ KvProblem kv_problem(const KvParams& K, int prob) {
+  const AttnParams& P = K.A;
+  KvProblem p;
+  if (PERHEAD) {
+    const int b = prob / P.H, hh = prob - b * P.H, C = P.H * kDh;
+    p.b = b; p.head = hh;
+    p.q = P.q + (size_t)b * P.nQ * C + hh * kDh;
+    p.dout = K.dout + (size_t)b * P.nQ * C + hh * kDh;
+    p.rstride = C;
+    p.v = P.v + (size_t)b * P.nK * P.v_stride + hh * kDh;
+    p.dk = K.dk + (size_t)b * P.nK * C + hh * kDh;
+    p.dv = K.dv + (size_t)b * P.nK * C + hh * kDh;
+    p.ostride = C;
+  } else {
+    p.b = prob; p.head = 0;
+    p.q = P.q + (size_t)prob * K.R * kDh;
+    p.dout = K.dout + (size_t)prob * K.R * kDh;
+    p.rstride = kDh;
+    p.v = P.v + (size_t)prob * P.nK * P.v_stride;
+    p.dk = K.dk + (size_t)prob * P.nK * kDh;
+    p.dv = K.dv + (size_t)prob * P.nK * kDh;
+    p.ostride = kDh;
+  }
+  p.score_off = (size_t)prob * K.R * P.nK;
+  p.row_off = (size_t)prob * K.R;
+  return p;
+}
+
+
+__device__ __forceinline__ f32x16 kv_mfma(bf16x8 a, bf16x8 b, f32x16 c) {
+  return __builtin_amdgcn_mfma_f32_32x32x16_bf16(a, b, c, 0, 0, 0);
+}
+__device__ __forceinline__ f32x16 kv_mfma3(bf16x8 ah, bf16x8 al, bf16x8 bh, bf16x8 bl, f32x16 c) {
+  c = kv_mfma(al, bh, c);
+  c = kv_mfma(ah, bl, c);
+  return kv_mfma(ah, bh, c);
+}
+
+template <bool PERHEAD>
+__device__ __forceinline__ void kv_pack_body(const KvParams& K, long gid, long stride) {
+  const AttnParams& P = K.A;
+  const int R = K.R, NT = K.NT;
+  const int nprob = PERHEAD ? P.B * P.H : P.B;
+  const long nunits = (long)nprob * NT * 12 * kWave;
+  for (long u = gid; u < nunits; u += stride) {
+    const int lane = (int)(u & 63);
+    long r = u >> 6;
+    const int sub = (int)(r & 3);
+    r >>= 2;
+    const int kind = (int)(r % 3);
+    const long bt = r / 3;
+    const int prob = (int)(bt / NT), tile = (int)(bt - (long)prob * NT), r0 = tile * 32;
+    const int l31 = lane & 31, g = lane >> 5;
+    const KvProblem pb = kv_problem<PERHEAD>(K, prob);
+    const float* src = kind == 2 ? pb.q : pb.dout;
+    float x[8];
+    if (kind == 0) {
+      const int row = r0 + l31;
+#pragma unroll
+      for (int e = 0; e < 8; ++e) x[e] = row < R ? src[(size_t)row * pb.rstride + 16 * sub + 8 * g + e] : 0.f;
+    } else {
+      const int d = 32 * (sub >> 1) + l31, t = sub & 1;
+#pragma unroll
+      for (int e = 0; e < 8; ++e) {
+        const int row = r0 + kv_row(8 * t + e, g);
+        x[e] = row < R ? src[(size_t)row * pb.rstride + d] : 0.f;
+      }
+    }
+    bf16x8 hi, lo;
+    kv_split8(x, hi, lo);
+    uint4* dst = K.pack + ((bt * 3 + kind) * 4 + sub) * kKvOperandUnits;
+    dst[lane] = __builtin_bit_cast(uint4, hi);
+    dst[kWave + lane] = __builtin_bit_cast(uint4, lo);
+  }
+  const long nz = (long)P.B * P.nK * (PERHEAD ? P.H : 1) * kDh / 4;
+  f32x4* zk = reinterpret_cast<f32x4*>(K.dk);
+  f32x4* zv = reinterpret_cast<f32x4*>(K.dv);
+  for (long i = gid; i < nz; i += stride) {
+    zk[i] = f32x4{0.f, 0.f, 0.f, 0.f};
+    zv[i] = f32x4{0.f, 0.f, 0.f, 0.f};
+  }
+}
+
+template <bool PERHEAD, int WAVES, int HALVES, bool SELF>
+__device__ __forceinline__ void kv_key_owner_body(const KvParams& K, float* smem, int kt, int hf, int prob) {
+  static_assert(!SELF || HALVES == 1, "plain stores need one workgroup per key tile");
+  constexpr int kKvWaves = WAVES, kKvThreads = WAVES * kWave, kKvSlots = HALVES * WAVES;
+  AttnParams P = K.A;
+  attn_load_rng(P);
+  const int tid = threadIdx.x, lane = tid & 63;
+  const int w = __builtin_amdgcn_readfirstlane(tid >> 6);
+  const int l31 = lane & 31, g = lane >> 5;
+  const KvProblem pb = kv_problem<PERHEAD>(K, prob);
+  const int b = pb.b;
+  const int R = K.R, NT = K.NT, nK = P.nK;
+  const int key = kt * 32 + l31;
+  const bool kvalid = SELF || key < nK;
+
+  uint4* vstrip = reinterpret_cast<uint4*>(smem) + w * (8 * kWave) + lane;
+  {
+    const float* vrow = pb.v + (size_t)(kvalid ? key : 0) * P.v_stride + 8 * g;
+#pragma unroll
+    for (int s = 0; s < 4; ++s) {
+      const f32x4 a = *reinterpret_cast<const f32x4*>(vrow + 16 * s), c = *reinterpret_cast<const f32x4*>(vrow + 16 * s + 4);
+      float x[8] = {a[0], a[1], a[2], a[3], c[0], c[1], c[2], c[3]};
+      if (!kvalid) {
+#pragma unroll
+        for (int e = 0; e < 8; ++e) x[e] = 0.f;
+      }
+      bf16x8 hi, lo;
+      kv_split8(x, hi, lo);
+      vstrip[(2 * s) * kWave] = __builtin_bit_cast(uint4, hi);
+      vstrip[(2 * s + 1) * kWave] = __builtin_bit_cast(uint4, lo);
+    }
+  }
+  f32x16 accV[2], accK[2];
+#pragma unroll
+  for (int i = 0; i < 16; ++i) { accV[0][i] = 0.f; accV[1][i] = 0.f; accK[0][i] = 0.f; accK[1][i] = 0.f; }
+
+  using rsrc_t = __amdgpu_buffer_rsrc_t;
+  const unsigned recs = (unsigned)((size_t)R * nK * 4);
+  const rsrc_t rs = __builtin_amdgcn_make_buffer_rsrc(P.scores + pb.score_off, 0, (int)recs, 0x00020000);
+  const rsrc_t rd = __builtin_amdgcn_make_buffer_rsrc(P.ds_out + pb.score_off, 0, (int)recs, 0x00020000);
+  const int rowbytes = nK * 4;
+  const unsigned lane_off = kvalid ? (unsigned)(4 * g * rowbytes + key * 4) : 0x80000000u;
+  const float* lse_b = P.lse + pb.row_off;
+  const float* delta_b = P.delta + pb.row_off;
+  const bool has_mask = P.mask_kind == VDETR_MASK_BOOL;
+  const unsigned char* mask_b = reinterpret_cast<const unsigned char*>(P.mask) + (size_t)b * P.nQ * nK + (kvalid ? key : 0);
+
+  auto load_scores = [&](int tile, float (&sv)[16]) {
+#pragma unroll
+    for (int a = 0; a < 4; ++a) {
+      const unsigned voff = lane_off + (unsigned)((tile * 32 + 8 * a) * rowbytes);
+#pragma unroll
+      for (int h = 0; h < 4; ++h)
+        sv[4 * a + h] = __builtin_bit_cast(float, __builtin_amdgcn_raw_buffer_load_b32(rs, (int)(voff + (unsigned)(h * rowbytes)), 0, kStreamAux));
+    }
+  };
+  const int first = hf * kKvWaves + w;
+  float sv[16], sn[16];
+  if (first < NT) load_scores(first, sn);
+
+  for (int tile = first; tile < NT; tile += kKvSlots) {
+    const int r0 = tile * 32;
+#pragma unroll
+    for (int i = 0; i < 16; ++i) sv[i] = sn[i];
+    const uint4* pk = K.pack + ((size_t)prob * NT + tile) * kKvTileUnits + lane;
+    auto operand = [&](int kind, int sub, int hl) { return pk[((kind * 4 + sub) * 2 + hl) * kWave]; };
+    auto row_consts = [&](int t, float (&lv)[8], float (&dv)[8]) {
+#pragma unroll
+      for (int a2 = 0; a2 < 2; ++a2) {
+        const int rb = r0 + 8 * (2 * t + a2) + 4 * g;
+        if (PERHEAD) {
+#pragma unroll
+          for (int h = 0; h < 4; ++h) {
+            const int row = SELF ? rb + h : min(rb + h, R - 1);
+            lv[4 * a2 + h] = lse_b[row];
+            dv[4 * a2 + h] = delta_b[row];
+          }
+        } else {
+          const f32x4 l4 = *reinterpret_cast<const f32x4*>(lse_b + min(rb, R - 4));
+          const f32x4 d4 = *reinterpret_cast<const f32x4*>(delta_b + min(rb, R - 4));
+#pragma unroll
+          for (int h = 0; h < 4; ++h) { lv[4 * a2 + h] = l4[h]; dv[4 * a2 + h] = d4[h]; }
+        }
+      }
+    };
+    uint4 opA[8], opB[8];
+#pragma unroll
+    for (int s = 0; s < 4; ++s) { opA[2 * s] = operand(0, s, 0); opA[2 * s + 1] = operand(0, s, 1); }
+#pragma unroll
+    for (int mt = 0; mt < 2; ++mt) {
+      opB[2 * mt] = operand(1, 2 * mt, 0); opB[2 * mt + 1] = operand(1, 2 * mt, 1);
+      opB[4 + 2 * mt] = operand(2, 2 * mt, 0); opB[4 + 2 * mt + 1] = operand(2, 2 * mt, 1);
+    }
+    float lv0[8], dv0[8];
+    row_consts(0, lv0, dv0);
+    __builtin_amdgcn_sched_barrier(0);
+    f32x16 dp;
+#pragma unroll
+    for (int i = 0; i < 16; ++i) dp[i] = 0.f;
+#pragma unroll
+    for (int s = 0; s < 4; ++s) {
+      const bf16x8 vh = __builtin_bit_cast(bf16x8, vstrip[(2 * s) * kWave]), vl = __builtin_bit_cast(bf16x8, vstrip[(2 * s + 1) * kWave]);
+      dp = kv_mfma3(__builtin_bit_cast(bf16x8, opA[2 * s]), __builtin_bit_cast(bf16x8, opA[2 * s + 1]), vh, vl, dp);
+    }
+    __builtin_amdgcn_sched_barrier(0);
+#pragma unroll
+    for (int mt = 0; mt < 2; ++mt) {
+      opA[2 * mt] = operand(1, 2 * mt + 1, 0); opA[2 * mt + 1] = operand(1, 2 * mt + 1, 1);
+      opA[4 + 2 * mt] = operand(2, 2 * mt + 1, 0); opA[4 + 2 * mt + 1] = operand(2, 2 * mt + 1, 1);
+    }
+    float lv1[8], dv1[8];
+    row_consts(1, lv1, dv1);
+    if (tile + kKvSlots < NT) load_scores(tile + kKvSlots, sn);
+    __builtin_amdgcn_sched_barrier(0);
+#pragma unroll
+    for (int t = 0; t < 2; ++t) {
+      float xp[8], xs[8];
+#pragma unroll
+      for (int a2 = 0; a2 < 2; ++a2) {
+        const int a = 2 * t + a2;
+        const int rb = r0 + 8 * a + 4 * g;
+        const unsigned voff = lane_off + (unsigned)((r0 + 8 * a) * rowbytes);
+        uint4 rnd = make_uint4(0xFFFFu, 0xFFFFu, 0xFFFFu, 0xFFFFu);
+        bool masked = false;
+        if (!PERHEAD) {
+          const int qi = min(rb, R - 4) >> 2;
+          if (P.drop_thresh) rnd = attn_rand4(P, b, qi, key, 0);
+          if (has_mask) masked = mask_b[(size_t)qi * nK] != 0;
+        }
+#pragma unroll
+        for (int h = 0; h < 4; ++h) {
+          const int v = 4 * a + h, e = 4 * a2 + h;
+          const bool ok = SELF || (rb + h < R && kvalid);
+          int pick = h;
+          if (PERHEAD) {
+            const int qi = SELF ? rb + h : min(rb + h, R - 1);
+            if (P.drop_thresh) rnd = attn_rand4(P, b, qi, key, pb.head >> 2);
+            if (has_mask) masked = mask_b[(size_t)qi * nK] != 0;
+            pick = pb.head & 3;
+          }
+          const bool keep = pick4(rnd, pick) >= P.drop_thresh;
+          const ScoreGrad gr = score_grad(sv[v], t ? lv1[e] : lv0[e], keep, P.drop_scale, true, dp[v], t ? dv1[e] : dv0[e], masked);
+          xp[e] = ok ? gr.p_drop : 0.f;
+          xs[e] = ok ? gr.ds : 0.f;
+          if (!SELF) __builtin_amdgcn_raw_buffer_store_b32(__float_as_int(gr.ds), rd, (int)(voff + (unsigned)(h * rowbytes)), 0, kStreamAux);
+        }
+      }
+      bf16x8 ph, pl, sh, sl;
+      kv_split8(xp, ph, pl);
+      kv_split8(xs, sh, sl);
+      const uint4* op = t ? opA : opB;
+#pragma unroll
+      for (int mt = 0; mt < 2; ++mt) {
+        accV[mt] = kv_mfma3(__builtin_bit_cast(bf16x8, op[2 * mt]), __builtin_bit_cast(bf16x8, op[2 * mt + 1]), ph, pl, accV[mt]);
+        accK[mt] = kv_mfma3(__builtin_bit_cast(bf16x8, op[4 + 2 * mt]), __builtin_bit_cast(bf16x8, op[4 + 2 * mt + 1]), sh, sl, accK[mt]);
+      }
+      __builtin_amdgcn_sched_barrier(0);
+    }
+  }
+  __syncthreads();
+
+  auto put = [&](int slot) {
+    float* dst = smem + (size_t)slot * 64 * kWave + lane;
+#pragma unroll
+    for (int i = 0; i < 16; ++i) {
+      dst[i * kWave] = accV[0][i]; dst[(16 + i) * kWave] = accV[1][i];
+      dst[(32 + i) * kWave] = accK[0][i]; dst[(48 + i) * kWave] = accK[1][i];
+    }
+  };
+  auto add = [&](int slot) {
+    const float* src = smem + (size_t)slot * 64 * kWave + lane;
+#pragma unroll
+    for (int i = 0; i < 16; ++i) {
+      accV[0][i] += src[i * kWave]; accV[1][i] += src[(16 + i) * kWave];
+      accK[0][i] += src[(32 + i) * kWave]; accK[1][i] += src[(48 + i) * kWave];
+    }
+  };
+#pragma unroll
+  for (int half = kKvWaves / 2; half >= 1; half >>= 1) {
+    if (w >= half && w < 2 * half) put(w - half);
+    __syncthreads();
+    if (w < half) add(w);
+    __syncthreads();
+  }
+  constexpr int kFinStride = kDh + 1;
+  if (w == 0) {
+#pragma unroll
+    for (int mt = 0; mt < 2; ++mt)
+#pragma unroll
+      for (int i = 0; i < 16; ++i) {
+        const int d = 32 * mt + kv_row(i, g);
+        smem[l31 * kFinStride + d] = accV[mt][i];
+        smem[(32 + l31) * kFinStride + d] = accK[mt][i] * P.scale;
+      }
+  }
+  __syncthreads();
+  for (int idx = tid; idx < 2 * 32 * kDh; idx += kKvThreads) {
+    const int which = idx >> 11, kl = (idx >> 6) & 31, d = idx & 63;
+    const int kg = kt * 32 + kl;
+    float* dst = (which ? pb.dk : pb.dv) + (size_t)kg * pb.ostride + d;
+    const float sum = smem[(which * 32 + kl) * kFinStride + d];
+    if (kg < nK) {
+      if (SELF) *dst = sum;
+      else unsafeAtomicAdd(dst, sum);
+    }
+  }
+}
+
+}
diff --git a/v-detr_amd/csrc/attn_bwd_self.hip b/v-detr_amd/csrc/attn_bwd_self.hip
--- /dev/null
+++ b/v-detr_amd/csrc/attn_bwd_self.hip
@@ -0,0 +1,198 @@
+#include "attn_bwd_kv_body.h"
+
+namespace vdetr {
+
+int attn_fill_params(const vdetr_attn_desc* d, AttnParams* P, const char* op);
+
+constexpr int kSelfWaves = 8;
+
+struct SelfParams {
+  KvParams K;
+  const uint4* img;
+  float* dq;
+  int NKT;
+};
+
+__device__ __forceinline__ void self_row_owner_body(const SelfParams& S, float* smem, int rt, int prob) {
+  const KvParams& K = S.K;
+  AttnParams P = K.A;
+  attn_load_rng(P);
+  const int tid = threadIdx.x, lane = tid & 63;
+  const int w = __builtin_amdgcn_readfirstlane(tid >> 6);
+  const int l31 = lane & 31, g = lane >> 5;
+  const KvProblem pb = kv_problem<true>(K, prob);
+  const int nK = P.nK, NKT = S.NKT, query = rt * 32 + l31;
+
+  uint4 opD[8];
+  {
+    const uint4* pk = K.pack + ((size_t)prob * K.NT + rt) * kKvTileUnits + lane;
+#pragma unroll
+    for (int i = 0; i < 8; ++i) opD[i] = pk[i * kWave];
+  }
+  const float lse_q = P.lse[pb.row_off + query], delta_q = P.delta[pb.row_off + query];
+
+  using rsrc_t = __amdgpu_buffer_rsrc_t;
+  const rsrc_t rs = __builtin_amdgcn_make_buffer_rsrc(P.scores + pb.score_off, 0, (int)((size_t)K.R * nK * 4), 0x00020000);
+  const unsigned lane_off = (unsigned)query * (unsigned)(nK * 4) + 16u * g;
+  auto load_scores = [&](int kt, float (&sv)[16]) {
+#pragma unroll
+    for (int a = 0; a < 4; ++a) {
+      const f32x4 x = __builtin_bit_cast(f32x4, __builtin_amdgcn_raw_buffer_load_b128(rs, (int)(lane_off + (unsigned)((kt * 32 + 8 * a) * 4)), 0, kStreamAux));
+#pragma unroll
+      for (int h = 0; h < 4; ++h) sv[4 * a + h] = x[h];
+    }
+  };
+  f32x16 accQ[2];
+#pragma unroll
+  for (int i = 0; i < 16; ++i) { accQ[0][i] = 0.f; accQ[1][i] = 0.f; }
+  float sv[16], sn[16];
+  if (w < NKT) load_scores(w, sn);
+
+  for (int kt = w; kt < NKT; kt += kSelfWaves) {
+#pragma unroll
+    for (int i = 0; i < 16; ++i) sv[i] = sn[i];
+    const uint4* im = S.img + ((size_t)prob * NKT + kt) * kKvSelfTileUnits + lane;
+    uint4 opV[8], opK0[4], opK1[4];
+#pragma unroll
+    for (int i = 0; i < 8; ++i) opV[i] = im[i * kWave];
+#pragma unroll
+    for (int mt = 0; mt < 2; ++mt) { opK0[2 * mt] = im[(8 + 4 * mt) * kWave]; opK0[2 * mt + 1] = im[(8 + 4 * mt + 1) * kWave]; }
+    __builtin_amdgcn_sched_barrier(0);
+    f32x16 dp;
+#pragma unroll
+    for (int i = 0; i < 16; ++i) dp[i] = 0.f;
+#pragma unroll
+    for (int s = 0; s < 4; ++s)
+      dp = kv_mfma3(__builtin_bit_cast(bf16x8, opV[2 * s]), __builtin_bit_cast(bf16x8, opV[2 * s + 1]),
+                    __builtin_bit_cast(bf16x8, opD[2 * s]), __builtin_bit_cast(bf16x8, opD[2 * s + 1]), dp);
+    __builtin_amdgcn_sched_barrier(0);
+#pragma unroll
+    for (int mt = 0; mt < 2; ++mt) { opK1[2 * mt] = im[(8 + 4 * mt + 2) * kWave]; opK1[2 * mt + 1] = im[(8 + 4 * mt + 3) * kWave]; }
+    if (kt + kSelfWaves < NKT) load_scores(kt + kSelfWaves, sn);
+    __builtin_amdgcn_sched_barrier(0);
+#pragma unroll
+    for (int t = 0; t < 2; ++t) {
+      float xs[8];
+#pragma unroll
+      for (int e = 0; e < 8; ++e) {
+        const int v = 8 * t + e, key = kt * 32 + kv_row(v, g);
+        bool keep = true;
+        if (P.drop_thresh) keep = pick4(attn_rand4(P, pb.b, query, key, pb.head >> 2), pb.head & 3) >= P.drop_thresh;
+        xs[e] = score_grad(sv[v], lse_q, keep, P.drop_scale, true, dp[v], delta_q, false).ds;
+      }
+      bf16x8 sh, sl;
+      kv_split8(xs, sh, sl);
+      const uint4* op = t ? opK1 : opK0;
+#pragma unroll
+      for (int mt = 0; mt < 2; ++mt)
+        accQ[mt] = kv_mfma3(__builtin_bit_cast(bf16x8, op[2 * mt]), __builtin_bit_cast(bf16x8, op[2 * mt + 1]), sh, sl, accQ[mt]);
+      __builtin_amdgcn_sched_barrier(0);
+    }
+  }
+
+#pragma unroll
+  for (int half = kSelfWaves / 2; half >= 1; half >>= 1) {
+    float* slot = smem + (size_t)(w & (half - 1)) * 32 * kWave + lane;
+    if (w >= half && w < 2 * half) {
+#pragma unroll
+      for (int i = 0; i < 16; ++i) { slot[i * kWave] = accQ[0][i]; slot[(16 + i) * kWave] = accQ[1][i]; }
+    }
+    __syncthreads();
+    if (w < half) {
+#pragma unroll
+      for (int i = 0; i < 16; ++i) { accQ[0][i] += slot[i * kWave]; accQ[1][i] += slot[(16 + i) * kWave]; }
+    }
+    __syncthreads();
+  }
+  if (w == 0) {
+    float* row = S.dq + ((size_t)pb.b * P.nQ + query) * (P.H * kDh) + pb.head * kDh + 4 * g;
+#pragma unroll
+    for (int mt = 0; mt < 2; ++mt)
+#pragma unroll
+      for (int a = 0; a < 4; ++a)
+        *reinterpret_cast<f32x4*>(row + 32 * mt + 8 * a) = f32x4{accQ[mt][4 * a] * P.scale, accQ[mt][4 * a + 1] * P.scale,
+                                                                  accQ[mt][4 * a + 2] * P.scale, accQ[mt][4 * a + 3] * P.scale};
+  }
+}
+
+__global__ __launch_bounds__(kSelfWaves * kWave) void attn_bwd_self_kernel(SelfParams S) {
+  extern __shared__ __attribute__((aligned(16))) float smem[];
+  const int nkt = S.NKT;
+  if ((int)blockIdx.x >= nkt) {
+    self_row_owner_body(S, smem, (int)blockIdx.x - nkt, blockIdx.y);
+    return;
+  }
+  kv_key_owner_body<true, kSelfWaves, 1, true>(S.K, smem, blockIdx.x, 0, blockIdx.y);
+}
+
+__global__ __launch_bounds__(256) void attn_bwd_self_pack_kernel(KvParams K, DeltaArgs D, int ndelta, uint4* img) {
+  if ((int)blockIdx.x < ndelta) {
+    __shared__ float wmax[4];
+    attn_delta_body(D, (int)blockIdx.x, wmax);
+    return;
+  }
+  const long gid = (long)((int)blockIdx.x - ndelta) * 256 + threadIdx.x, stride = (long)((int)gridDim.x - ndelta) * 256;
+  kv_pack_body<true>(K, gid, stride);
+  kv_self_images(img, K.A.k, K.A.v, K.A.k_stride, K.A.v_stride, K.A.B, K.A.H, K.A.nK, gid, stride);
+}
+
+}
+
+using namespace vdetr;
+
+static bool self_supported(const vdetr_attn_desc* d) {
+  return d && d->kind == VDETR_ATTN_PER_HEAD && d->H == 4 && d->B > 0 && d->nQ > 0 && d->nK > 0 && d->nQ % 32 == 0 && d->nK % 32 == 0 &&
+         !d->table && !d->mask && !d->bwd_aux;
+}
+
+extern "C" size_t vdetr_attn_bwd_self_workspace_bytes(const vdetr_attn_desc* d) {
+  if (!self_supported(d)) return 0;
+  return kv_self_image_offset(vdetr_attn_bwd_kv_workspace_bytes(d)) + (size_t)d->B * d->H * (d->nK / 32) * kKvSelfTileUnits * sizeof(uint4);
+}
+
+extern "C" int vdetr_attn_bwd_self_f32(const vdetr_attn_desc* d, const float* q, const float* k, const float* v, const float* dout,
+                                       const float* out, const float* scores, const float* lse, float* delta, float* dq, float* dk,
+                                       float* dv, void* workspace, size_t workspace_bytes, vdetr_stream_t stream) {
+  SelfParams S;
+  KvParams& K = S.K;
+  if (int e = attn_fill_params(d, &K.A, "attn_bwd_self")) return e;
+  VDETR_REQUIRE(self_supported(d), "attn_bwd_self: built for the per-head kind with 4 heads, no mask, no table, nQ and nK multiples of 32 "
+                "(kind %d, H %d, nQ %d, nK %d)", d->kind, d->H, d->nQ, d->nK);
+  VDETR_REQUIRE(q && k && v && dout && scores && lse && delta && dq && dk && dv, "attn_bwd_self: null pointer");
+  VDETR_REQUIRE((((uintptr_t)k | (uintptr_t)v | (uintptr_t)scores | (uintptr_t)dq | (uintptr_t)dk | (uintptr_t)dv) & 15) == 0,
+                "attn_bwd_self: k, v, scores, dq, dk and dv must be 16-B aligned");
+  const size_t nprob = (size_t)d->B * d->H;
+  VDETR_REQUIRE((size_t)d->nQ * d->nK * 4 < ((size_t)1 << 31), "attn_bwd_self: a score matrix (%d x %d) must stay below 2 GB", d->nQ, d->nK);
+  VDETR_REQUIRE(nprob <= 65535, "attn_bwd_self: %zu score matrices > 65535", nprob);
+  const size_t need = vdetr_attn_bwd_self_workspace_bytes(d);
+  if (!workspace || workspace_bytes < need) {
+    set_error("attn_bwd_self: workspace %zu B < required %zu B", workspace_bytes, need);
+    return VDETR_ERR_WORKSPACE;
+  }
+  VDETR_REQUIRE((((uintptr_t)workspace) & 255) == 0, "attn_bwd_self: the workspace (the operand images) must be 256-B aligned");
+  K.A.q = q; K.A.k = k; K.A.v = v;
+  K.A.scores = const_cast<float*>(scores); K.A.lse = const_cast<float*>(lse); K.A.delta = delta; K.A.ds_out = nullptr;
+  K.dout = dout; K.dk = dk; K.dv = dv;
+  K.pack = reinterpret_cast<uint4*>(workspace);
+  K.R = d->nQ;
+  K.NT = d->nQ / 32;
+  uint4* img = reinterpret_cast<uint4*>(reinterpret_cast<char*>(workspace) + kv_self_image_offset(vdetr_attn_bwd_kv_workspace_bytes(d)));
+  S.img = img; S.dq = dq; S.NKT = d->nK / 32;
+  hipStream_t st = (hipStream_t)stream;
+  if (out) {
+    DeltaArgs D{};
+    attn_delta_args(d, dout, out, v, delta, &D);
+    const int ndelta = D.qblocks + D.vblocks;
+    const long units = (long)nprob * K.NT * 12 * kWave, self_units = (long)nprob * S.NKT * 8 * kWave;
+    const long work = ((units > self_units ? units : self_units) + 255) / 256;
+    const unsigned blocks = (unsigned)(work < 2048 ? work : 2048);
+    hipLaunchKernelGGL(attn_bwd_self_pack_kernel, dim3(blocks + (unsigned)ndelta), dim3(256), 0, st, K, D, ndelta, img);
+    if (int e = check_launch("attn_bwd_self_pack")) return e;
+  }
+  const size_t strips = (size_t)kSelfWaves * 8 * kWave * sizeof(uint4), tree = (size_t)(kSelfWaves / 2) * 64 * kWave * sizeof(float);
+  const size_t fin = (size_t)2 * 32 * (kDh + 1) * sizeof(float);
+  const size_t lds = strips > tree ? (strips > fin ? strips : fin) : (tree > fin ? tree : fin);
+  if (int e = set_lds(attn_bwd_self_kernel, lds, "attn_bwd_self")) return e;
+  hipLaunchKernelGGL(attn_bwd_self_kernel, dim3(S.NKT + K.NT, (unsigned)nprob), dim3(kSelfWaves * kWave), lds, st, S);
+  return check_launch("attn_bwd_self");
+}
diff --git a/v-detr_amd/csrc/kv_pack.h b/v-detr_amd/csrc/kv_pack.h
--- a/v-detr_amd/csrc/kv_pack.h
+++ b/v-detr_amd/csrc/kv_pack.h
@@ -25,6 +25,36 @@
   uint4* dst = pack + ((tile * 3 + kind) * 4 + sub) * kKvOperandUnits;
   dst[lane] = __builtin_bit_cast(uint4, hi);
   dst[kWave + lane] = __builtin_bit_cast(uint4, lo);
+}
+
+constexpr int kKvSelfTileUnits = 2 * 4 * kKvOperandUnits;
+__host__ __device__ __forceinline__ constexpr size_t kv_self_image_offset(size_t kv_workspace_bytes) { return (kv_workspace_bytes + 255) & ~(size_t)255; }
+__device__ __forceinline__ void kv_self_images(uint4* img, const float* k, const float* v, int k_stride, int v_stride, int B, int H, int nK,
+                                               long gid, long stride) {
+  const int NKT = nK / 32;
+  const long nunits = (long)B * H * NKT * 8 * kWave;
+  for (long u = gid; u < nunits; u += stride) {
+    const int lane = (int)(u & 63), sub = (int)((u >> 6) & 3), which = (int)((u >> 8) & 1);
+    const long bt = u >> 9;
+    const int prob = (int)(bt / NKT), tile = (int)(bt - (long)prob * NKT), b = prob / H, hh = prob - b * H;
+    const int l31 = lane & 31, g = lane >> 5, k0 = tile * 32;
+    float x[8];
+    if (which == 0) {
+      const float* src = v + ((size_t)b * nK + k0 + l31) * v_stride + hh * kDh + 16 * sub + 8 * g;
+      const f32x4 a = *reinterpret_cast<const f32x4*>(src), c = *reinterpret_cast<const f32x4*>(src + 4);
+#pragma unroll
+      for (int e = 0; e < 4; ++e) { x[e] = a[e]; x[4 + e] = c[e]; }
+    } else {
+      const int d = 32 * (sub >> 1) + l31, t = sub & 1;
+#pragma unroll
+      for (int e = 0; e < 8; ++e) x[e] = k[((size_t)b * nK + k0 + kv_row(8 * t + e, g)) * k_stride + hh * kDh + d];
+    }
+    bf16x8 hi, lo;
+    kv_split8(x, hi, lo);
+    uint4* dst = img + ((bt * 2 + which) * 4 + sub) * kKvOperandUnits;
+    dst[lane] = __builtin_bit_cast(uint4, hi);
+    dst[kWave + lane] = __builtin_bit_cast(uint4, lo);
+  }
 }
 
 struct KvEmit {
```

Result: no change. 159.9, median of 6 (+0.6%).
